# AIRI-Institute/HairFastGAN

Hardware: AMD Instinct MI355X
Metric: stylegan2_generator_fwd_1024_images_per_sec (higher is better)
Workload: dtype f32 tensors + f32 accumulate; conv products as 3 fp16 MFMAs on (hi,lo)-split operands (fp32-class); 1 GPU; StyleGAN2 1024^2 generator forward (range 0->8), random W+, fresh noise per layer, HIP modulated-conv + upfirdn2d kernels (BASELINE.json configs[1]); batch_per_gpu=8, global_batch=8, parallelism=replica x1, weights=synthetic closed-form (oracle/synth.py), conv_precision=f16x3

## Files before the change

### hairfastgan_amd/_lib.py

```python
import ctypes
import os

_HERE = os.path.dirname(os.path.abspath(__file__))
LIB_PATH = os.environ.get("HAIRFAST_HIP_LIB") or os.path.join(_HERE, "csrc", "libhairfast_hip.so")

_f = ctypes.c_void_p
_i = ctypes.c_int
_ll = ctypes.c_longlong
_fl = ctypes.c_float
_d = ctypes.c_double
_st = ctypes.c_void_p

SIGNATURES = {
    "hf_upfirdn2d_f32": [_f, _f, _f, _i, _i, _i, _i, _i, _i, _i, _i, _i, _i, _i, _i, _i, _st],
    "hf_fused_bias_act_f32": [_f, _f, _f, _ll, _i, _i, _fl, _fl, _st],
    "hf_noise_bias_act_f32": [_f, _f, _f, _f, _f, _i, _i, _i, _ll, _fl, _fl, _st],
    "hf_modconv_prepare_f32": [_f, _f, _f, _i, _i, _i, _st],
    "hf_modulation_f32": [_f, _f, _ll, _f, _f, _i, _i, _i, _st],
    "hf_style_batch_f32": [_f, _f, _ll, _ll, _f, _i, _i, _i, _i, _i, _st],
    "hf_demod_f32": [_f, _f, _f, _i, _i, _i, _st],
    "hf_style_normalize_f32": [_f, _f, _i, _i, _i, _st],
    "hf_modconv3x3_f32": [_f, _f, _f, _f, _f, _f, _f, _ll, _f, _i, _i, _i, _i, _i, _fl, _fl, _f, _ll, _st],
    "hf_conv_split_weights_f16": [_f, _f, _f, _i, _i, _st],
    "hf_conv_split_weights_f16_taps": [_f, _f, _f, _i, _i, _i, _st],
    "hf_modconv3x3_small_f16_f32": [_f, _f, _f, _f, _i, _f, _f, _f, _f, _ll, _f, _i, _i, _i, _i, _i, _fl, _fl, _i, _i, _f, _ll, _st],
    "hf_modconv3x3_small_up_blur_f16_f32": [_f, _f, _f, _f, _f, _f, _i, _f, _f, _f, _f, _f, _ll, _f, _f, _i, _i, _i, _i, _i, _fl, _fl, _f, _ll, _st],
    "hf_conv1x1_f16_f32": [_f, _f, _f, _f, _f, _f, _i, _f, _f, _f, _f, _i, _f, _fl, _f, _i, _i, _i, _i, _i, _i, _i, _ll, _f, _ll, _st],
    "hf_modconv3x3_f16_f32": [_f, _f, _f, _f, _i, _f, _f, _f, _f, _ll, _f, _i, _i, _i, _i, _i, _fl, _fl, _st],
    "hf_modconv3x3_f16_rgb_f32": [_f, _f, _f, _f, _i, _f, _f, _f, _f, _ll, _f, _i, _i, _i, _i, _i, _fl, _fl, _f, _f, _f, _st],
    "hf_modconv3x3_f16_pre_image_f32": [_f, _f, _f, _f, _f, _i, _f, _f, _f, _ll, _f, _i, _i, _i, _i, _i, _fl, _fl, _f, _f, _f, _f, _f, _st],
    "hf_modconv3x3_f16_pre_f32": [_f, _f, _f, _f, _f, _i, _f, _f, _f, _ll, _f, _i, _i, _i, _i, _i, _fl, _fl, _f, _f, _f, _f, _f, _f, _st],
    "hf_modconv3x3_up_f16_pre_f32": [_f, _f, _f, _f, _f, _i, _f, _i, _i, _i, _i, _i, _i, _st],
    "hf_modconv3x3_up_f16_f32": [_f, _f, _f, _f, _i, _f, _f, _i, _i, _i, _i, _i, _i, _st],
    "hf_modconv3x3_up_blur_f16_f32": [_f, _f, _f, _f, _f, _f, _f, _f, _f, _f, ctypes.POINTER(ctypes.c_float),
                                      ctypes.POINTER(ctypes.c_float), _f, _f, _ll, _f, _f, _i, _i, _i, _i, _i, _fl, _fl, _st],
    "hf_modconv3x3_up_f32": [_f, _f, _f, _f, _f, _i, _i, _i, _i, _i, _i, _f, _ll, _st],
    "hf_modconv_up_pitch": [_i],
    "hf_blur_noise_bias_act_f32": [_f, _f, _f, _f, _f, _ll, _f, _i, _i, _i, _i, _i, _fl, _fl, _st],
    "hf_blur_noise_bias_act_split_f16": [_f, _f, _f, _f, _f, _f, _ll, _f, _f, _i, _i, _i, _i, _i, _fl, _fl, _st],
    "hf_torgb_f32": [_f, _f, _f, _f, _f, _f, _f, _i, _i, _i, _i, _st],
    "hf_conv_prepare_f32": [_f, _f, _i, _i, _i, _fl, _st],
    "hf_bn_fold_f32": [_f, _f, _f, _f, _f, _f, _f, _fl, _i, _st],
    "hf_conv2d_f32": [_f, _f, _f, _f, _f, _f, _f, _i, _f, _fl, _f, _i, _i, _i, _i, _i, _i, _i, _i, _ll, _f, _ll, _st],
    "hf_conv2d_f16_f32": [_f, _f, _f, _f, _f, _f, _i, _f, _f, _f, _f, _i, _f, _fl, _f, _i, _i, _i, _i, _i, _i, _i, _ll, _f, _ll, _st],
    "hf_split_activation_f16": [_f, _f, _f, _f, _f, _ll, _i, _i, _i, _st],
    "hf_split_activation_mod_f16": [_f, _f, _f, _f, _ll, _i, _i, _i, _st],
    "hf_plane_mean_f32": [_f, _f, _i, _i, _st],
    "hf_se_gate_f32": [_f, _f, _f, _f, _i, _i, _i, _st],
    "hf_scale_shortcut_add_f32": [_f, _f, _f, _f, _i, _i, _i, _i, _i, _i, _i, _st],
    "hf_upsample_bilinear_add_f32": [_f, _f, _f, _i, _i, _i, _i, _i, _st],
    "hf_adaptive_avgpool_f32": [_f, _f, _i, _i, _i, _i, _i, _i, _i, _i, _st],
    "hf_downscale2x_f32": [_f, _f, _i, _i, _i, _st],
    "hf_linear_f32": [_f, _f, _ll, _f, _f, _i, _i, _i, _fl, _st],
    "hf_equal_linear_f32": [_f, _f, _ll, _f, _f, _i, _i, _i, _fl, _i, _fl, _fl, _st],
    "hf_pixel_norm_f32": [_f, _f, _i, _i, _st],
    "hf_bicubic_down_f32": [_f, _f, _f, _ll, _i, _i, _i, _st],
    "hf_dilate_erode_f32": [_f, _f, _f, _ll, _i, _i, _i, _st],
    "hf_quantize_u8_f32": [_f, _f, _ll, _st],
    "hf_poisson_setup_u8": [_f, _f, _f, _f, _f, _i, _i, _i, _i, _st],
    "hf_poisson_jacobi_f32": [_f, _f, _f, _f, _i, _i, _i, _i, _i, _i, _st],
    "hf_poisson_finish_u8": [_f, _f, _f, _f, _i, _i, _i, _i, _st],
    "hf_resize_lanczos_u8": [_f, _f, _f, _i, _i, _i, _i, _i, _f, _f, _i, _f, _f, _i, _st],
    "hf_quad_bilinear_u8": [_f, _f, ctypes.POINTER(ctypes.c_double), _i, _i, _i, _i, _i, _st],
    "hf_quad_lanczos4_u8": [_f, _f, ctypes.POINTER(ctypes.c_double), _i, _i, _i, _i, _f, _f, _i, _st],
    "hf_quad_lanczos4_ratio": [],
    "hf_align_pad_blur_f32": [_f, _f, _f, _f, _i, _f, _f, _i, _i, _i, _i, _i, _i, _i, _st],
    "hf_align_pad_finish_u8": [_f, _f, _f, _f, _f, _f, _i, _i, _i, _st],
    "hf_u8_to_unit_f32": [_f, _f, _ll, _st],
    "hf_paste_quad_u8": [_f, _f, _f, ctypes.POINTER(ctypes.c_double), _i, _i, _i, _i, _i, _i, _i, _i, _st],
    "hf_multiply_u8": [_f, _f, _f, _ll, _st],
    "hf_image_to_bytes_f32": [_f, _f, _i, _i, _i, _fl, _fl, _i, _i, _st],
    "hf_labels_to_rgb_i64": [_f, _f, _ll, _f, _i, _i, _st],
    "hf_png_encode_u8": [_f, _ll, _f, _f, _i, _i, _i, _i, _i, _f, _ll, _st],
    "hf_jpeg_encode_u8": [_f, _ll, _f, _f, _i, _i, _i, _i, _i, _i, _f, _ll, _st],
    "hf_jpeg_decode_u8": [_f, _f, _f, _f, _ll, _f, _ll, _f, _i, _i, _i, _i, _i, _i, _i, _i, _i, _f, _ll, _st],
    "hf_png_decode_u8": [_f, _f, _f, _f, _ll, _f, _ll, _f, _i, _i, _i, _i, _i, _i, _f, _ll, _st],
    "hf_frechet_accumulate_f64": [_f, _f, _f, _i, _i, _st],
    "hf_frechet_accumulate_f16_f64": [_f, _f, _f, _i, _i, _st],
    "hf_frechet_stats_f64": [_f, _f, _f, _f, _ll, _i, _st],
    "hf_sym_eig_jacobi_f64": [_f, _f, _f, _f, _i, _i, ctypes.POINTER(ctypes.c_int), ctypes.POINTER(ctypes.c_double), _st],
    "hf_sym_eig_jacobi_work_doubles": (_ll, [_i, _i]),
    "hf_frechet_congruence_f64": [_f, _f, _f, _f, _f, _i, _st],
    "hf_frechet_finish_f64": [_f, _f, _f, _f, _f, _f, _i, _st],
    "hf_conv2d_direct_f32": [_f, _f, _f, _f, _f, _f, _i, _fl, _i, _i, _i, _i, _i, _i, _i, _i, _st],
    "hf_maxpool2d_f32": [_f, _f, _ll, _i, _i, _i, _i, _st],
    "hf_lpips_layer_f64": [_f, _f, _f, _f, _f, _i, _i, _i, _i, _i, _st],
    "hf_lpips_layer_work_doubles": (_ll, [_i, _i, _i]),
    "hf_sq_err_sum_f64": [_f, _f, _f, _f, _i, _ll, _i, _st],
    "hf_sq_err_sum_work_doubles": (_ll, [_i, _ll]),
    "hf_ssim_planes_f64": [_f, _f, _f, _f, _f, _f, _f, _f, _f, _f, _i, _i, _i, _i, _i, _i, _d, _d, _d, _st],
    "hf_ssim_work_doubles": (_ll, [_i, _i, _i, _i]),
    "hf_ssim_tile": [_i],
    "hf_crop_avgpool_f32": [_f, _f, _f, _f, _i, _i, _i, _i, _i, _i, _i, _i, _i, _i, _st],
    "hf_l2_normalize_rows_f32": [_f, _f, _f, _i, _i, _st],
    "hf_row_similarity_f64": [_f, _f, _f, _i, _i, _i, _i, _st],
    "hf_conv2d_rect_f16_f32": [_f, _f, _f, _f, _f, _i, _f, _f, _i, _i, _i, _i, _i, _i, _i, _i, _i, _i, _i, _i, _i, _i, _i, _i, _i, _st],
    "hf_pool3x3_f32": [_f, _f, _i, _i, _i, _i, _i, _i, _i, _i, _i, _i, _st],
    "hf_resize_bilinear_tf1_f32": [_f, _f, _i, _i, _i, _i, _i, _i, _i, _i, _fl, _fl, _st],
    "hf_maxpool3x3s2_f32":[_f, _f, _ll, _i, _i, _st],
    "hf_gate_f32": [_f, _f, _f, _f, _f, _fl, _ll, _i, _st],
    "hf_upsample_nearest_f32": [_f, _f, _ll, _i, _i, _i, _i, _st],
    "hf_parsing_mask_i64": [_f, _f, _f, _i, _i, _i, _i, _i, _i, _i, _i, _st],
    "hf_layernorm_f32": [_f, _f, _f, _f, _i, _i, _fl, _i, _fl, _st],
    "hf_layernorm_grouped_f32": [_f, _f, _f, _f, _i, _i, _i, _fl, _i, _fl, _st],
    "hf_modulate_f32": [_f, _f, _f, _f, _ll, _i, _fl, _st],
    "hf_sample_layernorm_f32": [_f, _f, _f, _f, _i, _i, _i, _ll, _fl, _fl, _f, _ll, _st],
    "hf_pixel_norm_dim1_f32": [_f, _f, _i, _i, _i, _st],
    "hf_axpby_bcast_f32": [_f, _f, _fl, _f, _fl, _ll, _ll, _st],
    "hf_add_bcast_f32": [_f, _f, _f, _ll, _ll, _st],
    "hf_label_conv3x3_f32": [_f, _f, _f, _f, _i, _i, _i, _i, _i, _i, _i, _i, _f, _st],
    "hf_ace_modulate_f32": [_f, _f, _f, _f, _f, _f, _f, _f, _f, _i, _i, _i, _i, _fl, _i, _st],
    "hf_conv2d_f16_split_f32": [_f, _f, _f, _f, _f, _f, _f, _f, _f, _f, _i, _f, _f, _f, _f, _i, _f, _fl, _f, _i, _i, _i, _i, _i, _i, _st],
    "hf_stem7x7s2_f16_f32": [_f, _f, _f, _f, _f, _f, _f, _fl, _i, _i, _i, _i, _i, _st],
    "hf_ace_modulate_table_f32": [_f, _f, _f, _f, _f, _f, _f, _f, _f, _f, _f, _i, _i, _i, _i, _i, _i, _i, _fl, _i, _i, _st],
    "hf_region_mean_f32": [_f, _f, _f, _i, _i, _i, _i, _i, _ll, _ll, _i, _i, _st],
    "hf_tanh_f32": [_f, _f, _ll, _st],
    "hf_channel_layernorm_f32": [_f, _f, _f, _f, _i, _ll, _fl, _st],
    "hf_mha_small_f32": [_f, _f, _i, _i, _i, _i, _st],
    "hf_quick_gelu_f32": [_f, _f, _ll, _st],
    "hf_debug_set_dispatch": [_i, _i],
    "hf_debug_last_path": [],
    "hf_debug_set_persistent_blocks": [_i],
    "hf_debug_set_tuning": [_i],
    "hf_set_batch_invariant": [_i],
    "hf_set_splitk_counters": [_f, _i],
    "hf_modconv3x3_f16_rgb_slabs": [_i],
    "hf_profile_marker": [_i, _st],
    "hf_conv2d_f16_split_output_ok": [_i, _i, _i, _i, _i, _i, _i, _i],
    "hf_scale_shortcut_add_split_f16": [_f, _f, _f, _f, _f, _f, _f, _f, _i, _i, _i, _i, _i, _i, _i, _st],
    "hf_strerror": (ctypes.c_char_p, [_i]),
    "hf_abi_version": [],
    "hf_modconv_workspace_floats": (_ll, [_i, _i, _i, _i, _i, _i]),
    "hf_conv2d_workspace_floats": (_ll, [_i, _i, _i, _i, _i, _i, _i, _i]),
    "hf_conv2d_f16_workspace_floats": (_ll, [_i, _i, _i, _i, _i, _i, _i]),
    "hf_modconv3x3_small_workspace_floats": (_ll, [_i, _i, _i, _i, _i]),
    "hf_conv1x1_f16_workspace_floats": (_ll, [_i, _i, _i, _i, _i, _i, _i]),
    "hf_sample_layernorm_workspace_floats": (_ll, [_i, _i, _i]),
    "hf_f16_overflow_count": (_ll, [_i]),
    "hf_png_bound": (_ll, [_i, _i, _i]),
    "hf_png_segment_rows": [_i, _i, _i],
    "hf_png_workspace_bytes": (_ll, [_i, _i, _i, _i]),
    "hf_jpeg_bound": (_ll, [_i, _i, _i, _i]),
    "hf_jpeg_chunk_mcus": [_i, _i],
    "hf_jpeg_workspace_bytes": (_ll, [_i, _i, _i, _i, _i]),
    "hf_jpeg_decode_workspace_bytes": (_ll, [_i, _i, _i, _i, _i, _i, _i, _ll]),
    "hf_png_decode_workspace_bytes": (_ll, [_i, _i, _i, _i, _ll]),
}


class HairfastLibError(RuntimeError):
    pass


def bind(cdll):
    for name, sig in SIGNATURES.items():
        try:
            fn = getattr(cdll, name)
        except AttributeError as e:
            raise HairfastLibError(f"{cdll._name}: missing symbol {name}") from e
        fn.restype, fn.argtypes = sig if isinstance(sig, tuple) else (ctypes.c_int, sig)
    return cdll


_LIB = None


def load():
    global _LIB
    if _LIB is None:
        if not os.path.exists(LIB_PATH):
            raise HairfastLibError(
                f"{LIB_PATH} not found: build it with `python -c 'import __graft_entry__ as g; g.build()'` "
                "or hairfastgan_amd/csrc/build.sh (hipcc --offload-arch=gfx950). "
                "hairfastgan_amd has no CPU / PyTorch fallback.")
        _LIB = bind(ctypes.CDLL(LIB_PATH))
    return _LIB


def check(lib, code, what):
    if code != 0:
        raise RuntimeError(f"{what}: {lib.hf_strerror(code).decode()} (code {code})")
```

### hairfastgan_amd/_marshal.py

```python
import functools
import os

import torch
import torch.nn.functional as F

from ._lib import check
from ._runtime import CANON_BATCH, plan_batch

SQRT2 = 2 ** 0.5

PROFILE = None


KERNEL_NAMES = {
    211: "conv_mfma_pipe<2,2,2,4>", 212: "conv_mfma_pipe<2,2,1,4>", 213: "conv_mfma_pipe<1,2,1,4>",
    214: "conv_mfma_pipe<2,2,2,2>", 215: "conv_mfma_pipe<1,1,2,2>", 216: "conv_mfma_pipe<1,4,1,4>",
    231: "conv_mfma_dma<2,2,2,4>", 232: "conv_mfma_dma<2,2,1,4>", 233: "conv_mfma_dma<1,2,1,4>", 234: "conv_mfma_dma<2,2,2,2>",
    244: "conv_mfma_pipe<2,2,2,2,stride2>", 245: "conv_mfma_pipe<1,1,2,2,stride2>",
    221: "conv_mfma_pipe<1,2,2,2,up>", 222: "conv_mfma_pipe<1,2,1,4,up>", 223: "conv_mfma_pipe<1,1,2,2,up>",
    224: "conv_mfma_pipe<1,2,2,4,up>", 225: "conv_mfma_pipe<1,1,1,4,up>", 300: "conv_mfma<1,1,2,2> split-K",
    581: "conv_mfma_h<1,2,2,4,up,pre>", 583: "conv_mfma_h<1,2,1,8,up,pre>",
    571: "conv_mfma_h<1,2,2,4,pre>", 572: "conv_mfma_h<2,2,1,8,pre>", 575: "conv_mfma_h<1,2,1,8,tw128,pre>",
    579: "conv_rows_h<32->32,strip64,pre>",
    551: "conv_mfma_h<1,2,2,4>", 552: "conv_mfma_h<2,2,1,8>", 553: "conv_mfma_h<1,2,1,8>", 555: "conv_mfma_h<1,2,1,8,tw128>",
    561: "conv_mfma_h<1,2,2,4,up>", 563: "conv_mfma_h<1,2,1,8,up>",
    573: "conv_mfma_h<1,2,1,8,up,fuse>", 593: "conv_mfma_h<1,2,1,8,up,pre,fuse>",
    601: "conv_enc_h<64x256>", 602: "conv_enc_h<64x128,stride2>", 603: "conv_enc_h<64x128>", 604: "conv_enc_h<64x512>",
    605: "conv_enc_h<64x128,stride2,x4 tiles>",
    606: "conv_enc_h<64x128,stride2,x2 tiles>",
}


def _launch_profiled(lib, flops, fn, label=None, nbytes=0.0, tag=""):
    if PROFILE is None:
        return fn()
    e0 = torch.cuda.Event(enable_timing=True)
    e1 = torch.cuda.Event(enable_timing=True)
    e0.record()
    r = fn()
    e1.record()
    if label is None:
        code = lib.hf_debug_last_path()
        label = KERNEL_NAMES.get(code, f"conv_mfma (general, code {code})")
        if tag and label.endswith(">"):
            label = label[:-1] + tag + ">"
    PROFILE.append((label, flops, e0, e1, nbytes))
    return r


def _p(t):
    return None if t is None else t.data_ptr()


def _c(t):
    if t is None:
        return None
    if t.dtype != torch.float32:
        raise TypeError(f"hairfastgan_amd kernels are fp32; got {t.dtype}")
    return t if t.is_contiguous() else t.contiguous()


class SplitActivation:

    def __init__(self, hi, lo, key):
        self.hi, self.lo, self.key = hi, lo, key
        b, cb, h, w, _ = hi.shape
        self.shape = (b, cb * 8, h, w)

    @classmethod
    def empty(cls, b, c, h, w, device, want_lo=True, key=None):
        hi = torch.empty((b, c // 8, h, w, 8), dtype=torch.float16, device=device)
        return cls(hi, torch.empty_like(hi) if want_lo else None, key)


def _hl(split):
    return (None, None) if split is None else (_p(split.hi), _p(split.lo))


def upfirdn2d(lib, st, x, kernel, up_x, up_y, down_x, down_y, pad_x0, pad_x1, pad_y0, pad_y1):
    x, kernel = _c(x), _c(kernel)
    n, c, h, w = x.shape
    kh, kw = kernel.shape
    out_h = (h * up_y + pad_y0 + pad_y1 - kh) // down_y + 1
    out_w = (w * up_x + pad_x0 + pad_x1 - kw) // down_x + 1
    out = x.new_empty((n, c, out_h, out_w))
    if out.numel():
        check(lib, lib.hf_upfirdn2d_f32(_p(out), _p(x), _p(kernel), n * c, h, w, kh, kw, up_x, up_y, down_x,
                                        down_y, pad_x0, pad_x1, pad_y0, pad_y1, st), "hf_upfirdn2d_f32")
    return out


def fused_bias_act(lib, st, x, bias, alpha, scale):
    x, bias = _c(x), _c(bias)
    out = torch.empty_like(x)
    n = x.numel()
    if n == 0:
        return out
    step_b = 1
    for d in x.shape[2:]:
        step_b *= d
    n_bias = bias.numel() if bias is not None else 0
    if bias is not None and x.ndim >= 2 and n_bias != x.shape[1]:
        raise ValueError("bias must have one entry per channel (dim 1)")
    check(lib, lib.hf_fused_bias_act_f32(_p(out), _p(x), _p(bias), n, max(n_bias, 1), step_b, alpha, scale, st),
          "hf_fused_bias_act_f32")
    return out


def _noise_args(noise, batch, hw):
    if noise is None:
        return None, 0
    noise = _c(noise)
    if noise.numel() == hw:
        return noise, 0
    if noise.numel() == batch * hw:
        return noise, hw
    raise ValueError(f"noise must be [1,1,H,W] or [B,1,H,W]; got {tuple(noise.shape)}")


def noise_bias_act(lib, st, x, noise, noise_w, bias, alpha=0.2, scale=SQRT2):
    x, bias, noise_w = _c(x), _c(bias), _c(noise_w)
    b, c, h, w = x.shape
    noise, nbs = _noise_args(noise, b, h * w)
    out = torch.empty_like(x)
    check(lib, lib.hf_noise_bias_act_f32(_p(out), _p(x), _p(noise), _p(noise_w), _p(bias), b, c, h * w, nbs,
                                         alpha, scale, st), "hf_noise_bias_act_f32")
    return out


def prepare_weights(lib, st, weight):
    weight = _c(weight)
    _, cout, cin, k, _ = weight.shape
    wt = weight.new_empty((k * k, cin, cout))
    wsq = weight.new_empty((cout, cin))
    check(lib, lib.hf_modconv_prepare_f32(_p(wt), _p(wsq), _p(weight), cout, cin, k, st), "hf_modconv_prepare_f32")
    return wt, wsq


def modulation(lib, st, style, mod_w, mod_b):
    if style.dtype != torch.float32:
        raise TypeError("style must be fp32")
    if style.stride(-1) != 1:
        style = style.contiguous()
    b, sd = style.shape
    mod_w, mod_b = _c(mod_w), _c(mod_b)
    cin = mod_w.shape[0]
    s = style.new_empty((b, cin))
    check(lib, lib.hf_modulation_f32(_p(s), _p(style), style.stride(0) if b > 1 else sd, _p(mod_w), _p(mod_b),
                                     b, cin, sd, st), "hf_modulation_f32")
    return s


def style_job_table(convs, rows, batch, device):
    recs, layout, ofs = [], [], 0
    for conv, row in zip(convs, rows):
        _, wsq = conv.prepared()
        cin, cout = conv.in_channel, conv.out_channel
        s_ofs = ofs
        ofs += batch * cin
        d_ofs = -1
        if conv.demodulate:
            d_ofs = ofs
            ofs += batch * cout
        mw, mb = conv.modulation.weight.detach(), conv.modulation.bias.detach()
        recs.append([mw.data_ptr(), mb.data_ptr(), wsq.data_ptr() if conv.demodulate else 0, cin | (cout << 32), row,
                     s_ofs, max(d_ofs, 0)])
        layout.append((s_ofs, cin, d_ofs, cout))
    table = torch.tensor(recs, dtype=torch.int64).to(device)
    return table, layout, ofs


def style_batch(lib, st, latent, table, layout, total, max_cin, max_cout):
    if latent.dtype != torch.float32 or latent.stride(-1) != 1:
        latent = latent.float().contiguous()
    b, _, sd = latent.shape
    out = latent.new_empty(total)
    check(lib, lib.hf_style_batch_f32(_p(out), _p(latent), latent.stride(0), latent.stride(1), _p(table), len(layout), b, sd,
                                      max_cin, max_cout, st), "hf_style_batch_f32")
    res = []
    for s_ofs, cin, d_ofs, cout in layout:
        s = out[s_ofs:s_ofs + b * cin].view(b, cin)
        d = out[d_ofs:d_ofs + b * cout].view(b, cout) if d_ofs >= 0 else None
        res.append((s, d))
    return res


def demod(lib, st, s, wsq):
    b, cin = s.shape
    cout = wsq.shape[0]
    d = s.new_empty((b, cout))
    check(lib, lib.hf_demod_f32(_p(d), _p(s), _p(wsq), b, cin, cout, st), "hf_demod_f32")
    return d


def style_normalize(lib, st, s, d):
    b, cin = s.shape
    check(lib, lib.hf_style_normalize_f32(_p(s), _p(d), b, cin, d.shape[1], st), "hf_style_normalize_f32")


def f16_overflow_count(lib, reset=False):
    return int(lib.hf_f16_overflow_count(1 if reset else 0))


def _workspace(lib, like, b, cin, cout, h, w, up):
    n = lib.hf_modconv_workspace_floats(b, cin, cout, h, w, 1 if up else 0)
    if n <= 0:
        return None, 0
    return like.new_empty((n,)), n


def modconv3x3(lib, st, x, wt, s, d, noise, noise_w, bias, alpha=0.2, scale=SQRT2):
    x = _c(x)
    b, cin, h, w = x.shape
    cout = wt.shape[2]
    noise, nbs = _noise_args(noise, b, h * w)
    out = x.new_empty((b, cout, h, w))
    noise_w, bias = _c(noise_w), _c(bias)
    ws, ws_n = _workspace(lib, x, b, cin, cout, h, w, False)
    code = _launch_profiled(
        lib, 2.0 * cin * cout * 9 * h * w * b,
        lambda: lib.hf_modconv3x3_f32(_p(out), _p(x), _p(wt), _p(s), _p(d), _p(noise), _p(noise_w), nbs, _p(bias),
                                      b, cin, cout, h, w, alpha, scale, _p(ws), ws_n, st))
    check(lib, code, "hf_modconv3x3_f32")
    return out


def split_weights_f16(lib, st, wt):
    wt = _c(wt)
    taps, cin, cout = wt.shape
    if taps != 9 or cin % 16:
        raise ValueError(f"f16 MFMA path needs 3x3 weights with cin % 16 == 0; got {tuple(wt.shape)}")
    n = 9 * cin * cout
    hi = torch.empty(n + 8, dtype=torch.float16, device=wt.device)[:n].view(cin // 16, 9, 2, cout, 8)
    lo = torch.empty((cin // 16, 9, 2, cout, 8), dtype=torch.float16, device=wt.device)
    check(lib, lib.hf_conv_split_weights_f16(_p(hi), _p(lo), _p(wt), cin, cout, st), "hf_conv_split_weights_f16")
    return hi, lo


def split_weights_unscale(wt_hi):
    n = wt_hi.numel()
    flat = torch.empty(0, dtype=torch.float16, device=wt_hi.device).set_(wt_hi.untyped_storage(), wt_hi.storage_offset(), (n + 8,))
    return float(flat[n:n + 2].view(torch.float32)[0])


def modconv3x3_f16_supported(cin, cout, h, w, batch=None):
    if batch is not None and plan_batch(batch) * h * w < 2048:
        return False
    return cin % 16 == 0 and w >= 32 and (h >= 8 if cout % 64 == 0 else (cout % 32 == 0 and h >= 16))


def torgb_fusable(cin, cout, h, w):
    if not (cout % 32 == 0 and modconv3x3_f16_supported(cin, cout, h, w)):
        return False
    return h * w >= (512 if cout in (32, 64) else 4096)


IMAGE_FUSE = os.environ.get("HAIRFAST_IMAGE_FUSE", "1") != "0"


def image_fusable(cin, cout, h, w):
    return cin == 32 and cout == 32 and w % 64 == 0 and h % 8 == 0 and IMAGE_FUSE


def modconv3x3_f16_pre_image(lib, st, act, wt_hi, wt_lo, nterms, d, noise, noise_w, bias, rgb, rgb_bias, skip, up_kernel,
                             alpha=0.2, scale=SQRT2):
    b, cin, h, w = act.shape
    cout = wt_hi.shape[3]
    skip = _c(skip)
    if tuple(skip.shape) != (b, 3, h // 2, w // 2):
        raise ValueError(f"skip must be [B,3,H/2,W/2]; got {tuple(skip.shape)} for a {h}x{w} layer")
    noise, nbs = _noise_args(noise, b, h * w)
    image = torch.empty((b, 3, h, w), dtype=torch.float32, device=act.hi.device)
    rgb_wt, rgb_s = _c(rgb[0]), _c(rgb[1])
    nparts = 2 if nterms == 3 else 1
    nb = float(b) * h * w * (2.0 * nparts * cin + 12.0 + 3.0) + 2.0 * nparts * 9 * cin * cout
    code = _launch_profiled(
        lib, 2.0 * cin * cout * 9 * h * w * b,
        lambda: lib.hf_modconv3x3_f16_pre_image_f32(_p(image), _p(act.hi), _p(act.lo), _p(wt_hi), _p(wt_lo), nterms, _p(d), _p(noise),
                                                    _p(_c(noise_w)), nbs, _p(_c(bias)), b, cin, cout, h, w, alpha, scale, _p(rgb_wt),
                                                    _p(rgb_s), _p(_c(rgb_bias)), _p(skip), _p(_c(up_kernel)), st), nbytes=nb)
    if code == -1:
        return None
    check(lib, code, "hf_modconv3x3_f16_pre_image_f32")
    return image


def torgb_slabs(cout):
    return cout // 64 if cout % 64 == 0 else cout // 32


def modconv3x3_f16(lib, st, x, wt_hi, wt_lo, nterms, s, d, noise, noise_w, bias, alpha=0.2, scale=SQRT2, rgb=None):
    x = _c(x)
    b, cin, h, w = x.shape
    cout = wt_hi.shape[3]
    noise, nbs = _noise_args(noise, b, h * w)
    out = x.new_empty((b, cout, h, w))
    noise_w, bias = _c(noise_w), _c(bias)
    if rgb is not None:
        rgb_wt, rgb_s = _c(rgb[0]), _c(rgb[1])
        raw = x.new_empty((b, 3 * torgb_slabs(cout), h, w))
        code = _launch_profiled(
            lib, 2.0 * cin * cout * 9 * h * w * b,
            lambda: lib.hf_modconv3x3_f16_rgb_f32(_p(out), _p(x), _p(wt_hi), _p(wt_lo), nterms, _p(s), _p(d), _p(noise),
                                                  _p(noise_w), nbs, _p(bias), b, cin, cout, h, w, alpha, scale,
                                                  _p(raw), _p(rgb_wt), _p(rgb_s), st))
        check(lib, code, "hf_modconv3x3_f16_rgb_f32")
        return out, raw
    code = _launch_profiled(
        lib, 2.0 * cin * cout * 9 * h * w * b,
        lambda: lib.hf_modconv3x3_f16_f32(_p(out), _p(x), _p(wt_hi), _p(wt_lo), nterms, _p(s), _p(d), _p(noise),
                                          _p(noise_w), nbs, _p(bias), b, cin, cout, h, w, alpha, scale, st))
    check(lib, code, "hf_modconv3x3_f16_f32")
    return out


def split_activation_reference(x, s):
    b, c, h, w = x.shape
    v = x if s is None else x * s[:, :, None, None]
    hi = v.half()
    lo = (v - hi.float()).half()
    blk = lambda t: t.reshape(b, c // 8, 8, h, w).permute(0, 1, 3, 4, 2).contiguous()
    return blk(hi), blk(lo)


def _modconv3x3_f16_pre(lib, st, act, wt_hi, wt_lo, nterms, d, noise, noise_w, bias, alpha=0.2, scale=SQRT2, rgb=None,
                        want_out=True, split_for=None):
    b, cin, h, w = act.shape
    cout = wt_hi.shape[3]
    dev = act.hi.device
    noise, nbs = _noise_args(noise, b, h * w)
    if not want_out and rgb is None and split_for is None:
        raise ValueError("want_out=False needs another consumer (rgb= or split_for=)")
    out = torch.empty((b, cout, h, w), dtype=torch.float32, device=dev) if want_out else None
    noise_w, bias = _c(noise_w), _c(bias)
    raw = rgb_wt = rgb_s = split = s_next = None
    if rgb is not None:
        rgb_wt, rgb_s = _c(rgb[0]), _c(rgb[1])
        raw = torch.empty((b, 3 * torgb_slabs(cout), h, w), dtype=torch.float32, device=dev)
    if split_for is not None:
        s_next = _c(split_for)
        split = SplitActivation.empty(b, cout, h, w, dev, want_lo=nterms == 3)
    nparts = 2 if nterms == 3 else 1
    nb = (float(b) * h * w * (2.0 * nparts * cin + (4.0 * cout if want_out else 0.0) + (2.0 * nparts * cout if split_for is not None else 0.0)
                              + (12.0 * torgb_slabs(cout) if rgb is not None else 0.0)) + 2.0 * nparts * 9 * cin * cout)
    code = _launch_profiled(
        lib, 2.0 * cin * cout * 9 * h * w * b,
        lambda: lib.hf_modconv3x3_f16_pre_f32(_p(out), _p(act.hi), _p(act.lo), _p(wt_hi), _p(wt_lo), nterms, _p(d), _p(noise),
                                              _p(noise_w), nbs, _p(bias), b, cin, cout, h, w, alpha, scale, _p(raw),
                                              _p(rgb_wt), _p(rgb_s), *_hl(split), _p(s_next), st), nbytes=nb)
    check(lib, code, "hf_modconv3x3_f16_pre_f32")
    return out, raw, split


def modconv3x3_f16_pre(lib, st, act, wt_hi, wt_lo, nterms, d, noise, noise_w, bias, alpha=0.2, scale=SQRT2, rgb=None,
                       want_out=True, split_for=None):
    out, raw, split = _modconv3x3_f16_pre(lib, st, act, wt_hi, wt_lo, nterms, d, noise, noise_w, bias, alpha, scale, rgb, want_out,
                                          split_for)
    res = (out,) + (() if rgb is None else (raw,)) + (() if split_for is None else (split,))
    return res[0] if len(res) == 1 else res


def split_weights_small(lib, st, wt):
    taps, cin, cout = wt.shape
    w1 = _c(wt).permute(1, 0, 2).reshape(1, cin, taps * cout).contiguous()
    return conv_split_weights_f16(lib, st, w1)


def modconv3x3_small_supported(cin, cout, h, w, batch, upsample=False):
    if cin % 32 or cout % 64 or h * w > 1024:
        return False
    n = plan_batch(batch) * h * w
    if upsample:
        return h * w <= 64 or (h * w <= 256 and n <= 1024)
    return 256 < n <= 2048 or (n == 256 and h * w <= 64) or (h * w == 64 and CANON_BATCH * 64 <= n <= 2048)


def conv3x3_small_supported(cin, cout, h, w, batch):
    return cin % 32 == 0 and cout % 64 == 0 and h * w <= 256 and plan_batch(batch) * h * w <= 4096 and cin * cout >= 512 * 512


def modconv3x3_small(lib, st, x, w9, nterms, s, d, noise, noise_w, bias, cout, alpha=0.2, scale=SQRT2, upsample=False):
    x = _c(x)
    b, cin, h, w = x.shape
    hi, lo = w9
    n = lib.hf_modconv3x3_small_workspace_floats(b, cin, cout, h, w)
    ws = x.new_empty((max(n, 1),))
    if upsample:
        pitch = lib.hf_modconv_up_pitch(w)
        out = x.new_empty((b, cout, 2 * h + 1, pitch))
        noise = bias = noise_w = None
        nbs = 0
    else:
        pitch = 0
        out = x.new_empty((b, cout, h, w))
        noise, nbs = _noise_args(noise, b, h * w)
    code = _launch_profiled(
        lib, 2.0 * cin * cout * 9 * h * w * b,
        lambda: lib.hf_modconv3x3_small_f16_f32(_p(out), _p(x), _p(hi), _p(lo), nterms, _p(_c(s)), _p(_c(d)), _p(noise),
                                                _p(_c(noise_w)), nbs, _p(_c(bias)), b, cin, cout, h, w, alpha, scale,
                                                1 if upsample else 0, pitch, _p(ws), n, st),
        label="gemm_h tap-GEMM (small planes)")
    check(lib, code, "hf_modconv3x3_small_f16_f32")
    return out


SMALL_UP_FUSED = os.environ.get("HAIRFAST_SMALL_UP_FUSED", "1") != "0"


def small_up_blur_supported(h, w):
    return (8 * (2 * h + 3) * (2 * w + 3) + 72 * h * w) * 4 <= 150 * 1024


def modconv3x3_small_up_blur(lib, st, x, w9, nterms, s, d, blur_kernel, noise, noise_w, bias, cout, alpha=0.2, scale=SQRT2,
                             split_for=None):
    x = _c(x)
    b, cin, h, w = x.shape
    hi, lo = w9
    n = lib.hf_modconv3x3_small_workspace_floats(b, cin, cout, h, w)
    ws = x.new_empty((max(n, 1),))
    noise, nbs = _noise_args(noise, b, 4 * h * w)
    out = split = s_next = None
    if split_for is not None:
        s_next = _c(split_for[1])
        split = SplitActivation.empty(b, cout, 2 * h, 2 * w, x.device, want_lo=split_for[2] if len(split_for) > 2 else True,
                                      key=split_for[0])
    else:
        out = x.new_empty((b, cout, 2 * h, 2 * w))
    code = _launch_profiled(
        lib, 2.0 * cin * cout * 9 * h * w * b,
        lambda: lib.hf_modconv3x3_small_up_blur_f16_f32(_p(out), *_hl(split), _p(x), _p(hi), _p(lo), nterms, _p(_c(s)), _p(_c(d)),
                                                        _p(_c(blur_kernel)), _p(noise), _p(_c(noise_w)), nbs, _p(_c(bias)),
                                                        _p(s_next), b, cin, cout, h, w, alpha, scale, _p(ws), n, st),
        label="gemm_h tap-GEMM (small planes)")
    check(lib, code, "hf_modconv3x3_small_up_blur_f16_f32")
    return out if split_for is None else split


def modconv3x3_up_f16_supported(cin, cout, h, w, batch=None):
    if batch is not None and plan_batch(batch) * h * w < 512:
        return False
    return cin % 16 == 0 and cout % 32 == 0 and h * w >= (256 if cout % 64 == 0 else 512) and min(h, w) >= 2


def modconv3x3_up(lib, st, x, wt, s, d, blur_kernel, noise, noise_w, bias, alpha=0.2, scale=SQRT2, f16=None,
                  split_for=None, small=None):
    pre = isinstance(x, SplitActivation)
    if not pre:
        x = _c(x)
    b, cin, h, w = x.shape
    cout = wt.shape[2]
    pitch = lib.hf_modconv_up_pitch(w)
    if pre or small is None:
        tmp = torch.empty((b, cout, 2 * h + 1, pitch), dtype=torch.float32, device=(x.hi if pre else x).device)
    if pre:
        hi, lo, nterms = f16
        code = _launch_profiled(
            lib, 2.0 * cin * cout * 9 * h * w * b,
            lambda: lib.hf_modconv3x3_up_f16_pre_f32(_p(tmp), _p(x.hi), _p(x.lo), _p(hi), _p(lo), nterms, _p(d), b, cin, cout,
                                                     h, w, pitch, st))
        check(lib, code, "hf_modconv3x3_up_f16_pre_f32")
    elif small is not None and SMALL_UP_FUSED and small_up_blur_supported(h, w):
        return modconv3x3_small_up_blur(lib, st, x, small[0], small[1], s, d, blur_kernel, noise, noise_w, bias, cout, alpha, scale,
                                        split_for=split_for)
    elif small is not None:
        tmp = modconv3x3_small(lib, st, x, small[0], small[1], s, d, None, None, None, cout, upsample=True)
    elif f16 is not None:
        hi, lo, nterms = f16
        code = _launch_profiled(
            lib, 2.0 * cin * cout * 9 * h * w * b,
            lambda: lib.hf_modconv3x3_up_f16_f32(_p(tmp), _p(x), _p(hi), _p(lo), nterms, _p(s), _p(d), b, cin, cout, h, w,
                                                 pitch, st))
        check(lib, code, "hf_modconv3x3_up_f16_f32")
    else:
        ws, ws_n = _workspace(lib, x, b, cin, cout, h, w, True)
        code = _launch_profiled(
            lib, 2.0 * cin * cout * 9 * h * w * b,
            lambda: lib.hf_modconv3x3_up_f32(_p(tmp), _p(x), _p(wt), _p(s), _p(d), b, cin, cout, h, w, pitch, _p(ws),
                                             ws_n, st))
        check(lib, code, "hf_modconv3x3_up_f32")
    noise, nbs = _noise_args(noise, b, 4 * h * w)
    if split_for is not None:
        s_next = split_for[1]
        want_lo = split_for[2] if len(split_for) > 2 else True
        split = SplitActivation.empty(b, cout, 2 * h, 2 * w, tmp.device, want_lo, key=split_for[0])
        nb = float(b * cout) * (4.0 * (2 * h + 1) * (2 * w + 1) + (4.0 if want_lo else 2.0) * 4 * h * w)
        code = _launch_profiled(
            lib, 0.0,
            lambda: lib.hf_blur_noise_bias_act_split_f16(*_hl(split), _p(tmp), _p(_c(blur_kernel)), _p(noise),
                                                         _p(_c(noise_w)), nbs, _p(_c(bias)), _p(_c(s_next)), b, cout,
                                                         2 * h + 1, 2 * w + 1, pitch, alpha, scale, st),
            label="blur4x4_split8", nbytes=nb)
        check(lib, code, "hf_blur_noise_bias_act_split_f16")
        return split
    out = tmp.new_empty((b, cout, 2 * h, 2 * w))
    nb = float(b * cout) * 4.0 * ((2 * h + 1) * (2 * w + 1) + 4 * h * w)
    code = _launch_profiled(
        lib, 0.0,
        lambda: lib.hf_blur_noise_bias_act_f32(_p(out), _p(tmp), _p(_c(blur_kernel)), _p(noise), _p(_c(noise_w)),
                                               nbs, _p(_c(bias)), b, cout, 2 * h + 1, 2 * w + 1, pitch, alpha, scale, st),
        label="blur4x4_noise_bias_act", nbytes=nb)
    check(lib, code, "hf_blur_noise_bias_act_f32")
    return out


def blur_factors(kernel4x4):
    import ctypes

    k = kernel4x4.detach().double().cpu()
    if tuple(k.shape) != (4, 4) or float(k[0, 0]) == 0.0:
        return None
    kx, ky = k[0, :].clone(), k[:, 0] / k[0, 0]
    if not torch.allclose(torch.outer(ky, kx), k, rtol=1e-6, atol=1e-12):
        return None
    arr = ctypes.c_float * 4
    return arr(*[float(v) for v in kx]), arr(*[float(v) for v in ky])


def modconv3x3_up_fused_supported(cin, cout, h, w):
    return cin % 16 == 0 and cout % 32 == 0 and h >= 16 and w >= 32


def modconv3x3_up_fused(lib, st, x, wt_hi, wt_lo, s, d, factors, noise, noise_w, bias, alpha=0.2, scale=SQRT2, split_for=None,
                        nterms=3):
    pre = isinstance(x, SplitActivation)
    if not pre:
        x = _c(x)
    b, cin, h, w = x.shape
    cout = wt_hi.shape[3]
    dev = x.hi.device if pre else x.device
    noise, nbs = _noise_args(noise, b, 4 * h * w)
    out = split = s_next = None
    if split_for is not None:
        s_next = _c(split_for)
        split = SplitActivation.empty(b, cout, 2 * h, 2 * w, dev, want_lo=nterms == 3)
    else:
        out = torch.empty((b, cout, 2 * h, 2 * w), dtype=torch.float32, device=dev)
    kx, ky = factors
    nb_alg = float(b) * (4.0 * cin * h * w + 4.0 * cout * 4 * h * w + 4.0 * 4 * h * w) + 4.0 * 9 * cin * cout
    code = _launch_profiled(
        lib, 2.0 * cin * cout * 9 * h * w * b,
        lambda: lib.hf_modconv3x3_up_blur_f16_f32(_p(out), *_hl(split), None if pre else _p(x), _p(x.hi) if pre else None,
                                                  _p(x.lo) if (pre and nterms == 3) else None, _p(wt_hi),
                                                  _p(wt_lo) if nterms == 3 else None, None if pre else _p(s), _p(d),
                                                  kx, ky, _p(noise), _p(_c(noise_w)), nbs, _p(_c(bias)), _p(s_next), b, cin, cout,
                                                  h, w, alpha, scale, st), nbytes=nb_alg)
    check(lib, code, "hf_modconv3x3_up_blur_f16_f32")
    return out if split_for is None else split


def torgb(lib, st, x, wt, s, bias, skip, up_kernel):
    x = _c(x)
    b, cin, h, w = x.shape
    skip = _c(skip)
    if skip is not None and tuple(skip.shape) != (b, 3, h // 2, w // 2):
        raise ValueError(f"skip must be [B,3,H/2,W/2]; got {tuple(skip.shape)} for x {tuple(x.shape)}")
    out = x.new_empty((b, 3, h, w))
    nb = float(b) * 4.0 * h * w * (cin + 3 + (0.75 if skip is not None else 0.0))
    code = _launch_profiled(
        lib, 0.0,
        lambda: lib.hf_torgb_f32(_p(out), _p(x), _p(wt), _p(s), _p(_c(bias)), _p(skip), _p(_c(up_kernel)), b, cin, h, w, st),
        label="torgb_kernel" if h * w > 4096 else "torgb_small_kernel", nbytes=nb)
    check(lib, code, "hf_torgb_f32")
    return out


ACT_NONE, ACT_LRELU, ACT_PRELU, ACT_QGELU = 0, 1, 2, 3
ACT_RESIDUAL_FIRST = 16


def conv_prepare(lib, st, weight, scale=1.0):
    weight = _c(weight)
    cout, cin, k, _ = weight.shape
    wt = weight.new_empty((k * k, cin, cout))
    check(lib, lib.hf_conv_prepare_f32(_p(wt), _p(weight), cout, cin, k, scale, st), "hf_conv_prepare_f32")
    return wt


def bn_fold(lib, st, gamma, beta, mean, var, eps, conv_bias=None):
    gamma, beta, mean, var, conv_bias = _c(gamma), _c(beta), _c(mean), _c(var), _c(conv_bias)
    n = gamma.numel()
    scale, shift = gamma.new_empty(n), gamma.new_empty(n)
    check(lib, lib.hf_bn_fold_f32(_p(scale), _p(shift), _p(gamma), _p(beta), _p(mean), _p(var), _p(conv_bias),
                                  float(eps), n, st), "hf_bn_fold_f32")
    return scale, shift


def _enc_conv_io(lib, x, cout, stride, in_scale, in_shift, residual, groups=1, x_shared=True, ws_floats=None, taps=9, nterms=3,
                 want_f32=True, split_out=False):
    pre = isinstance(x, SplitActivation)
    own = groups > 1 and not x_shared
    if pre:
        if in_scale is not None or in_shift is not None:
            raise ValueError("a pre-split input carries its affine already")
        n_img, cin, h, w = x.shape
        b = n_img // groups if own else n_img
        x_gstride = 1 if own else 0
        dev = x.hi.device
    else:
        x = _c(x)
        dev = x.device
        if own:
            g_, b, cin, h, w = x.shape
            if g_ != groups:
                raise ValueError("x must be [groups, B, cin, H, W]")
            x_gstride = b * cin * h * w
        else:
            b, cin, h, w = x.shape
            x_gstride = 0
    oh, ow = (h - 1) // stride + 1, (w - 1) // stride + 1
    shape = (groups, b, cout, oh, ow) if groups > 1 else (b, cout, oh, ow)
    out = torch.empty(shape, dtype=torch.float32, device=dev) if want_f32 else None
    if residual is not None:
        residual = _c(residual)
        if tuple(residual.shape) != shape:
            raise ValueError(f"residual {tuple(residual.shape)} != output {shape}")
    n = 0 if ws_floats is None else getattr(lib, ws_floats[0])(b, cin, cout, h, w, *ws_floats[1:], stride, groups)
    ws = torch.empty((n,), dtype=torch.float32, device=dev) if n > 0 else None
    nparts = 2 if nterms == 3 else 1
    nb = (float(b * (groups if own else 1)) * cin * (h * w if taps == 9 else oh * ow) * (2.0 * nparts if pre else 4.0)
          + float(b) * groups * cout * oh * ow * ((2.0 * nparts if split_out else 0.0) + (4.0 if want_f32 else 0.0)
                                                  + (4.0 if residual is not None else 0.0))
          + 2.0 * nparts * taps * cin * cout * groups)
    return x, (b, cin, h, w, oh, ow), x_gstride, out, residual, ws, max(n, 0), nb


def conv2d(lib, st, x, wt, k, stride=1, in_scale=None, in_shift=None, out_scale=None, bias=None, act=ACT_NONE,
           slope=None, alpha=0.0, residual=None, groups=1, x_shared=True):
    cout = wt.shape[-1]
    x, (b, cin, h, w, oh, ow), x_gstride, out, residual, ws, n, _ = _enc_conv_io(
        lib, x, cout, stride, None, None, residual, groups, x_shared, ("hf_conv2d_workspace_floats", k))
    code = _launch_profiled(
        lib, 2.0 * cin * cout * k * k * oh * ow * b * groups,
        lambda: lib.hf_conv2d_f32(_p(out), _p(x), _p(_c(wt)), _p(in_scale), _p(in_shift), _p(_c(out_scale)), _p(_c(bias)),
                                  act, _p(_c(slope)), float(alpha), _p(residual), b, cin, cout, h, w, k, stride, groups,
                                  x_gstride, _p(ws), n, st))
    check(lib, code, "hf_conv2d_f32")
    return out


def _pow2_ceil(v):
    p = 1
    while p < v:
        p <<= 1
    return p


@functools.lru_cache(maxsize=4096)
def conv2d_f16_supported(cin, cout, h, w, k, stride):
    if k != 3 or cin % 16 or cout % 64 or stride not in (1, 2):
        return False
    oh, ow = (h - 1) // stride + 1, (w - 1) // stride + 1
    tw = min(32, _pow2_ceil(ow))
    return tw >= 16 and _pow2_ceil(oh) >= 128 // tw


def conv_split_weights_f16(lib, st, wt):
    wt = _c(wt)
    w4 = wt if wt.ndim == 4 else wt.unsqueeze(0)
    g, taps, cin, cout = w4.shape
    if taps not in (9, 1) or cin % 16:
        raise ValueError(f"f16 MFMA path needs 3x3 or 1x1 weights with cin % 16 == 0; got {tuple(wt.shape)}")
    n = taps * cin * cout
    hi = torch.empty(g * (n + 8), dtype=torch.float16, device=wt.device)
    lo = torch.empty(g * n, dtype=torch.float16, device=wt.device)
    for i in range(g):
        check(lib, lib.hf_conv_split_weights_f16_taps(hi[i * (n + 8):].data_ptr(), lo[i * n:].data_ptr(), w4[i].data_ptr(), cin, cout,
                                                     taps, st), "hf_conv_split_weights_f16_taps")
    return hi, lo


def conv1x1_f16_supported(cin, cout):
    return cin % 32 == 0 and cout % 64 == 0


def conv1x1_f16(lib, st, x, wt_hi, wt_lo, nterms, cout, stride=1, in_scale=None, in_shift=None, out_scale=None, bias=None,
                act=ACT_NONE, slope=None, alpha=0.0, residual=None, groups=1, x_shared=True):
    pre = isinstance(x, SplitActivation)
    x, (b, cin, h, w, oh, ow), x_gstride, out, residual, ws, n, nb = _enc_conv_io(
        lib, x, cout, stride, in_scale, in_shift, residual, groups, x_shared, ("hf_conv1x1_f16_workspace_floats",), taps=1, nterms=nterms)
    code = _launch_profiled(
        lib, 2.0 * cin * cout * oh * ow * b * groups,
        lambda: lib.hf_conv1x1_f16_f32(_p(out), None if pre else _p(x), _p(x.hi) if pre else None, _p(x.lo) if pre else None,
                                       _p(wt_hi), _p(wt_lo), nterms, _p(_c(in_scale)), _p(_c(in_shift)),
                                       _p(_c(out_scale)), _p(_c(bias)), act, _p(_c(slope)), float(alpha), _p(residual), b, cin, cout,
                                       h, w, stride, groups, x_gstride, _p(ws), n, st),
        label="gemm_h", nbytes=nb)
    check(lib, code, "hf_conv1x1_f16_f32")
    return out


def split_activation_f16(lib, st, x, in_scale=None, in_shift=None, want_lo=True):
    x = _c(x)
    c, h, w = x.shape[-3:]
    images = x.numel() // (c * h * w)
    split = SplitActivation.empty(images, c, h, w, x.device, want_lo)
    check(lib, lib.hf_split_activation_f16(*_hl(split), _p(x), _p(_c(in_scale)), _p(_c(in_shift)), images, c, h, w, st),
          "hf_split_activation_f16")
    return split


def conv2d_f16(lib, st, x, wt_hi, wt_lo, nterms, cout, stride=1, in_scale=None, in_shift=None, out_scale=None, bias=None,
               act=ACT_NONE, slope=None, alpha=0.0, residual=None, groups=1, x_shared=True):
    pre = isinstance(x, SplitActivation)
    x, (b, cin, h, w, oh, ow), x_gstride, out, residual, ws, n, nb = _enc_conv_io(
        lib, x, cout, stride, in_scale, in_shift, residual, groups, x_shared, ("hf_conv2d_f16_workspace_floats",), nterms=nterms)
    code = _launch_profiled(
        lib, 2.0 * cin * cout * 9 * oh * ow * b * groups,
        lambda: lib.hf_conv2d_f16_f32(_p(out), None if pre else _p(x), _p(x.hi) if pre else None, _p(x.lo) if pre else None,
                                      _p(wt_hi), _p(wt_lo), nterms, _p(in_scale), _p(in_shift), _p(_c(out_scale)),
                                      _p(_c(bias)), act, _p(_c(slope)), float(alpha), _p(residual), b, cin, cout, h, w, stride,
                                      groups, x_gstride, _p(ws), n, st), tag=",pre" if pre else "", nbytes=nb)
    check(lib, code, "hf_conv2d_f16_f32")
    return out


def conv2d_f16_split_supported(lib, b, cin, cout, h, w, stride, nterms=3, pre=False):
    return cout % 8 == 0 and lib.hf_conv2d_f16_split_output_ok(b, cin, cout, h, w, stride, nterms, 1 if pre else 0) == 1


def conv2d_f16_split(lib, st, x, wt_hi, wt_lo, nterms, cout, stride=1, in_scale=None, in_shift=None, out_scale=None, bias=None,
                     act=ACT_NONE, slope=None, alpha=0.0, residual=None, next_scale=None, next_shift=None, want_f32=False):
    pre = isinstance(x, SplitActivation)
    x, (b, cin, h, w, oh, ow), _, out, residual, _, _, nb = _enc_conv_io(
        lib, x, cout, stride, in_scale, in_shift, residual, nterms=nterms, want_f32=want_f32, split_out=True)
    split = SplitActivation.empty(b, cout, oh, ow, (x.hi if pre else x).device, want_lo=nterms == 3)
    code = _launch_profiled(
        lib, 2.0 * cin * cout * 9 * oh * ow * b,
        lambda: lib.hf_conv2d_f16_split_f32(_p(out), *_hl(split), _p(_c(next_scale)), _p(_c(next_shift)), None if pre else _p(x),
                                            _p(x.hi) if pre else None, _p(x.lo) if pre else None, _p(wt_hi), _p(wt_lo), nterms,
                                            _p(in_scale), _p(in_shift), _p(_c(out_scale)), _p(_c(bias)), act, _p(_c(slope)),
                                            float(alpha), _p(residual), b, cin, cout, h, w, stride, st),
        tag=",pre,split-out" if pre else ",split-out", nbytes=nb)
    check(lib, code, "hf_conv2d_f16_split_f32")
    return split, out


def plane_mean(lib, st, x):
    x = _c(x)
# ... 916 lines not shown
```

### hairfastgan_amd/csrc/api.hip

```cpp
#include "hf_common.h"

extern "C" const char *hf_strerror(int code) {
  switch (code) {
    case HF_OK: return "ok";
    case HF_E_INVALID: return "invalid argument";
    case HF_E_LAUNCH: return "kernel launch failed";
    case HF_E_WORKSPACE: return "workspace too small";
    default: return "unknown error";
  }
}

extern "C" int hf_abi_version(void) { return 13; }

__global__ void hf_profile_marker_kernel() {}

extern "C" int hf_profile_marker(int id, void *stream) {
  if (id < 0 || id > 1023) return HF_E_INVALID;
  hipLaunchKernelGGL(hf_profile_marker_kernel, dim3(id + 1), dim3(64), 0, static_cast<hipStream_t>(stream));
  return hipGetLastError() == hipSuccess ? HF_OK : HF_E_LAUNCH;
}

extern "C" unsigned long long hf_f16_overflow_count_convh(int reset);
extern "C" unsigned long long hf_f16_overflow_count_blur(int reset);
extern "C" unsigned long long hf_f16_overflow_count_enc(int reset);
extern "C" unsigned long long hf_f16_overflow_count_gemm(int reset);
extern "C" unsigned long long hf_f16_overflow_count_stem(int reset);

extern "C" long long hf_f16_overflow_count(int reset) {
  return (long long)(hf_f16_overflow_count_convh(reset) + hf_f16_overflow_count_blur(reset) + hf_f16_overflow_count_enc(reset) +
                     hf_f16_overflow_count_gemm(reset) + hf_f16_overflow_count_stem(reset));
}
```

### hairfastgan_amd/csrc/convh.hip

```cpp
#define HF_WANT_F16_SPLIT
#include <type_traits>

#include "conv_common.h"

using namespace hf_detail;

#ifdef HF_H_TRACE
__device__ unsigned long long hf_trace_buf[8 * 512];
#define HF_TRACE_POINT(id)                                                                    \
  do {                                                                                         \
    if (blockIdx.x == 0 && blockIdx.y == 0 && lane == 0 && wave < 8 && trace_n < 510) {                    \
      hf_trace_buf[wave * 512 + trace_n++] = ((unsigned long long)(id) << 56) | (__builtin_readcyclecounter() & 0xffffffffffffffULL); \
    }                                                                                          \
  } while (0)
extern "C" int hf_debug_read_trace(unsigned long long *host, int n) {
  return (int)hipMemcpyFromSymbol(host, HIP_SYMBOL(hf_trace_buf), sizeof(unsigned long long) * n);
}
#else
#define HF_TRACE_POINT(id) ((void)0)
#endif

namespace {

template <int PT, bool UP, int TWMAX, bool FUSE = false>
// ... 743 lines not shown
      hf_barrier_keep_young<0>();
      HF_TRACE_POINT(3);
    }

    if (FUSE) {
      if (P.oh) epilogue_fused(std::true_type{}, cur, ep_slot, nzf, ((stage - 1) & 1));
      else epilogue_fused(std::false_type{}, cur, ep_slot, nzf, ((stage - 1) & 1));
    } else {
      bool done = false;
      if constexpr (!UP) {
        if (fast_ep) {
          epilogue_fast(G, cur, ep_slot, nzr);
          done = true;
        }
      }
      if (!done) epilogue(G, cur, ep_slot, nzr);
    }
    HF_TRACE_POINT(4);
    if (!has_next) break;
    zero_acc();
    if (nxt.b0 != cur.b0) ep_slot ^= 1;
    cur = nxt;
    t_cur = t_next;
  }
}

__global__ __launch_bounds__(256) void split_weights_absmax(unsigned int *__restrict__ trailer,
                                                            const float *__restrict__ wt, long long n) {
  float m = 0.0f;
  const long long stride = (long long)gridDim.x * blockDim.x;
  for (long long i = (long long)blockIdx.x * blockDim.x + threadIdx.x; i < n; i += stride) m = fmaxf(m, fabsf(wt[i]));
#pragma unroll
  for (int d = 32; d >= 1; d >>= 1) m = fmaxf(m, __shfl_xor(m, d, 64));
  if ((threadIdx.x & 63) == 0 && __float_as_uint(m) > trailer[1]) atomicMax(trailer + 1, __float_as_uint(m));
}
__global__ void split_weights_clear(unsigned int *trailer) {
  if (threadIdx.x < 4) trailer[threadIdx.x] = 0u;
}
__device__ __forceinline__ int weight_prescale_log2(unsigned int absmax_bits) {
  const int e = (int)((absmax_bits >> 23) & 255u) - 127;
  if (e <= -127 || e >= 128) return 0;
  int k = 13 - e;
  return k > 120 ? 120 : (k < -120 ? -120 : k);
}
__global__ __launch_bounds__(256) void split_weights(_Float16 *__restrict__ wth, _Float16 *__restrict__ wtl,
                                                     const float *__restrict__ wt, int cin, int cout, int taps) {
  const long long n = (long long)taps * cin * cout;
  unsigned int *trailer = reinterpret_cast<unsigned int *>(wth + n);
  const int k = weight_prescale_log2(trailer[1]);
  const float up = __uint_as_float((unsigned int)(127 + k) << 23);
  if (blockIdx.x == 0 && threadIdx.x == 0) reinterpret_cast<float *>(trailer)[0] = __uint_as_float((unsigned int)(127 - k) << 23);
  const long long stride = (long long)gridDim.x * blockDim.x;
  bool ovf = false;
  for (long long i = (long long)blockIdx.x * blockDim.x + threadIdx.x; i < n; i += stride) {
    const int co = (int)(i % cout);
    const long long r = i / cout;
    const int ci = (int)(r % cin), tap = (int)(r / cin);
    const long long dst = ((((long long)(ci / 16) * taps + tap) * 2 + (ci % 16) / 8) * cout + co) * 8 + (ci % 8);
    _Float16 h, l;
    hf_split_f16(wt[i] * up, h, l, ovf);
    wth[dst] = h;
    if (wtl) wtl[dst] = l;
  }
}

constexpr int RIM_DEPTH = 3;
template <int NTERMS>
__global__ __launch_bounds__(64) void conv_up_rim_h(const ConvParams P, const _Float16 *__restrict__ wth,
                                                    const _Float16 *__restrict__ wtl, int row_tiles, int pos_tiles) {
  constexpr int NPART = (NTERMS == 3) ? 2 : 1;
  const int lane = threadIdx.x & 63;
  const int li = lane & 31;
  const int lh = lane >> 5;
  const int co_tiles = P.cout / 32;
  int t = (int)blockIdx.x;
  const int co0 = (t % co_tiles) * 32;
  t /= co_tiles;
  const int pt = t % pos_tiles, b = t / pos_tiles;
  const bool is_row = pt < row_tiles;
  const int p = (is_row ? pt : pt - row_tiles) * 32 + li;
  const int h = P.h, w = P.w;
  const int plane = h * w;
  const bool store_ok = is_row ? p <= w : p < h;
  const bool near_ok = is_row ? p < w : p < h;
  const bool diag_ok = p >= 1 && (is_row ? p <= w : p < h);
  const int near_u = near_ok ? (is_row ? (h - 1) * w + p : p * w + (w - 1)) : 0;
  const int diag_u = diag_ok ? (is_row ? (h - 1) * w + p - 1 : (p - 1) * w + (w - 1)) : 0;
  const int tap0 = is_row ? 6 : 2, tap1 = is_row ? 7 : 5, tap2 = 8;

  const int nchunks = P.cin / KH;
  const long long x_lane = (((long long)b * (P.cin / 8) + lh) * plane) * 16;
  const long long x_chunk = 2LL * plane * 16;
  const char *xh = static_cast<const char *>(P.xh) + x_lane;
  const char *xl = NTERMS == 3 ? static_cast<const char *>(P.xl) + x_lane : nullptr;
  const long long w_lane = ((long long)lh * P.cout + co0 + li) * 16;
  const long long w_tap = 2LL * P.cout * 16, w_chunk = 9 * w_tap;
  const char *wh = reinterpret_cast<const char *>(wth) + w_lane;
  const char *wl = NTERMS == 3 ? reinterpret_cast<const char *>(wtl) + w_lane : nullptr;

  const float w_unscale = *reinterpret_cast<const float *>(wth + 9LL * P.cin * P.cout);
  float dmv[16];
#pragma unroll
  for (int r = 0; r < 16; ++r) dmv[r] = 1.0f;
  if (P.d) {
#pragma unroll
    for (int r = 0; r < 16; ++r) dmv[r] = P.d[(long long)b * P.d_bstride + co0 + (r & 3) + 8 * (r >> 2) + 4 * lh];
  }
#pragma unroll
  for (int r = 0; r < 16; ++r) dmv[r] *= w_unscale;

  half8 wa[RIM_DEPTH][3][NPART], xa[RIM_DEPTH][2][NPART];
  auto load = [&](int slot, int c) {
    const char *xc[2] = {xh + c * x_chunk, NTERMS == 3 ? xl + c * x_chunk : nullptr};
    const char *wc[2] = {wh + c * w_chunk, NTERMS == 3 ? wl + c * w_chunk : nullptr};
#pragma unroll
    for (int part = 0; part < NPART; ++part) {
      xa[slot][0][part] = *reinterpret_cast<const half8 *>(xc[part] + (long long)near_u * 16);
      xa[slot][1][part] = *reinterpret_cast<const half8 *>(xc[part] + (long long)diag_u * 16);
      wa[slot][0][part] = *reinterpret_cast<const half8 *>(wc[part] + tap0 * w_tap);
      wa[slot][1][part] = *reinterpret_cast<const half8 *>(wc[part] + tap1 * w_tap);
      wa[slot][2][part] = *reinterpret_cast<const half8 *>(wc[part] + tap2 * w_tap);
    }
  };
  f32x16 acc0, acc1;
#pragma unroll
  for (int r = 0; r < 16; ++r) acc0[r] = acc1[r] = 0.0f;
  auto mma = [&](f32x16 &acc, const half8 (&a)[NPART], const half8 (&bf)[NPART], bool ok) {
    const half8 zero = {};
    half8 bv[NPART];
#pragma unroll
    for (int part = 0; part < NPART; ++part) bv[part] = ok ? bf[part] : zero;
    mfma_f16x3<NTERMS, 1, 1>(&acc, &a[0], &a[NPART - 1], &bv[0], &bv[NPART - 1]);
  };

  auto chunk = [&](int s) {
    mma(acc0, wa[s][0], xa[s][0], near_ok);
    mma(acc1, wa[s][1], xa[s][0], near_ok);
    mma(acc0, wa[s][2], xa[s][1], diag_ok);
  };
#pragma unroll
  for (int s = 0; s < RIM_DEPTH; ++s) load(s, min(s, nchunks - 1));
  int c0 = 0;
  for (; c0 + RIM_DEPTH <= nchunks; c0 += RIM_DEPTH) {
#pragma unroll
    for (int s = 0; s < RIM_DEPTH; ++s) {
      chunk(s);
      load(s, min(c0 + s + RIM_DEPTH, nchunks - 1));
    }
  }
#pragma unroll
  for (int s = 0; s + 1 < RIM_DEPTH; ++s)
    if (c0 + s < nchunks) chunk(s);

  if (!store_ok) return;
  const long long oplane = (long long)P.out_h * P.out_w;
  float *ob = P.out + ((long long)b * P.cout + co0) * oplane +
              (is_row ? (long long)(2 * h) * P.out_w + 2 * p : (long long)(2 * p) * P.out_w + 2 * w);
  const long long second = is_row ? 1 : P.out_w;
  const bool has_second = !is_row || p < w;
#pragma unroll
  for (int r = 0; r < 16; ++r) {
    float *q = ob + (long long)((r & 3) + 8 * (r >> 2) + 4 * lh) * oplane;
    q[0] = acc0[r] * dmv[r];
    if (has_second) q[second] = acc1[r] * dmv[r];
  }
}

inline long long up_rim_blocks(const ConvParams &P) {
  return (long long)P.batch * (hf_cdiv(P.w + 1, 32) + hf_cdiv(P.h, 32)) * (P.cout / 32);
}
template <int NTERMS>
int launch_up_rim(const ConvParams &P, const _Float16 *wth, const _Float16 *wtl, hipStream_t st) {
  const int row_tiles = hf_cdiv(P.w + 1, 32), col_tiles = hf_cdiv(P.h, 32);
  hipLaunchKernelGGL((conv_up_rim_h<NTERMS>), dim3((unsigned)up_rim_blocks(P)), dim3(64), 0, st, P, wth, wtl, row_tiles,
                     row_tiles + col_tiles);
  return hf_launch_status();
}

template <int NTERMS, int CT_TILES, int PG, int WAVES_CO, int WAVES_PX, bool UP, int TWMAX = 32, bool PRE = false, bool FUSE = false>
int launch_h(ConvParams &P, const _Float16 *wth, const _Float16 *wtl, hipStream_t st) {
  using S = HShape<NTERMS, CT_TILES, PG, WAVES_CO, WAVES_PX, UP, TWMAX, FUSE>;
  constexpr int NT = S::NT, CT = S::CT, PT = S::PT, NPIX = S::Stage::NPIX;
  if (P.cin % KH || P.cout % CT || P.stride != 1 || P.t || P.groups > 1 || P.residual || P.act == ACT_PRELU)
    return HF_E_INVALID;
  if ((long long)P.cin * P.h * P.w >= (1LL << 31)) return HF_E_INVALID;
  if ((long long)CT * P.out_h * P.out_w * 4 >= (1LL << 32)) return HF_E_INVALID;
  P.splits = 1;
  P.n_geom = 1;
  P.g[0] = make_geom(0, 0, P.h, P.w, P.batch, PT, 0);
  if (TWMAX > 32 && P.w >= 64 && P.g[0].lg_nb == 0) {
    const int tw = min(TWMAX, pow2_floor(P.w)), th = PT / tw;
    if (th >= 1 && P.h >= th) {
      P.g[0].lg_tw = ilog2(tw); P.g[0].lg_th = ilog2(th);
      P.g[0].tiles_x = hf_cdiv(P.w, tw); P.g[0].tiles_y = hf_cdiv(P.h, th);
    }
  }
  if (FUSE) {
    constexpr int TH = PT / 32;
    P.g[0].lg_tw = 5; P.g[0].lg_th = ilog2(TH); P.g[0].lg_nb = 0;
    P.g[0].tiles_x = hf_cdiv(P.w, 30); P.g[0].tiles_y = hf_cdiv(P.h, TH - 2); P.g[0].tiles_b = P.batch;
  }
  int nblocks = geom_blocks(P.g[0]);
  const bool rim_kernel = UP && !FUSE && PRE && !(g_h_tune & 32);
  if (rim_kernel && up_rim_blocks(P) >= (1LL << 31)) return HF_E_INVALID;
  if (UP && !FUSE && !rim_kernel) {
    P.n_geom = 3;
    constexpr int RIM = PT >= 512 ? 4 : 2;
    P.g[1] = make_geom(P.h, 0, 1, P.w + 1, P.batch, PT, nblocks, true, RIM);
    nblocks += geom_blocks(P.g[1]);
    P.g[2] = make_geom(0, P.w, P.h, 1, P.batch, PT, nblocks, true, RIM);
    nblocks += geom_blocks(P.g[2]);
  }
  for (int i = 0; i < P.n_geom; ++i) {
    if (P.g[i].lg_nb != 0 || (1 << (P.g[i].lg_tw + P.g[i].lg_th)) != PT) return HF_E_INVALID;
    if (geom_xs(P.g[i], 1, UP ? 1 : 2) > NPIX) return HF_E_INVALID;
  }
  const size_t lds = S::lds_bytes(P.cin, P.rgb_out != nullptr);
  if (P.rgb_out && (UP || !P.rgb_w || !P.rgb_s || (!HF_STD_STYLED_TAIL(P) && (WAVES_CO != 1 || P.cout != CT)) ||
                    P.rgb_slabs != P.cout / (32 * CT_TILES)))
    return HF_E_INVALID;
  if (lds > 160 * 1024) return HF_E_INVALID;
  P.n_tiles = nblocks;
  const int co_tiles = P.cout / CT;
  const int per_cu = (2 * lds <= 160 * 1024) ? 2 : 1;
  int resident = (g_h_blocks > 0 ? g_h_blocks : 256 * per_cu) / co_tiles;
  if (resident < 1) resident = 1;
  const bool walk = P.cin / KH >= 2 && (P.cin / KH <= 8 || g_h_blocks > 0);
  const int gx = (walk && nblocks > resident) ? resident : nblocks;
  dim3 grid(gx, co_tiles);
  if (grid.y > 65535) return HF_E_INVALID;
  P.swap_xy = 0;
  if (co_tiles > 1 && gx <= 65535) {
    const double in_bytes = (double)P.batch * P.cin * P.h * P.w * 4.0, w_bytes = 9.0 * P.cin * P.cout * 4.0;
    if (columns_fastest(in_bytes, in_bytes, w_bytes, co_tiles, nblocks)) {
      P.swap_xy = 1;
      grid = dim3(co_tiles, gx);
    }
  }
  if (PRE) {
    if (!P.xh || (NTERMS == 3 && !P.xl) || P.s || (P.cin & 15)) return HF_E_INVALID;
    if ((long long)2 * P.h * P.w * 16 >= (1LL << 31)) return HF_E_INVALID;
    hipLaunchKernelGGL((conv_mfma_h<NTERMS, CT_TILES, PG, WAVES_CO, WAVES_PX, false, UP, TWMAX, PRE, FUSE>), grid, dim3(NT), lds, st,
                       P, wth, wtl);
  } else if (P.s) {
    hipLaunchKernelGGL((conv_mfma_h<NTERMS, CT_TILES, PG, WAVES_CO, WAVES_PX, true, UP, TWMAX, false, FUSE>), grid, dim3(NT), lds, st,
                       P, wth, wtl);
  } else {
    if (FUSE) return HF_E_INVALID;
    hipLaunchKernelGGL((conv_mfma_h<NTERMS, CT_TILES, PG, WAVES_CO, WAVES_PX, false, UP, TWMAX, false, false>), grid, dim3(NT), lds,
                       st, P, wth, wtl);
  }
  const int rc = hf_launch_status();
  if constexpr (UP && !FUSE && PRE) {
    if (rc == HF_OK && rim_kernel) return launch_up_rim<NTERMS>(P, wth, wtl, st);
  }
  return rc;
}

template <int CT_TILES_, int PG_, int WAVES_CO_, int WAVES_PX_, int TWMAX_ = 32>
struct HForm {
  static constexpr int CT_TILES = CT_TILES_, PG = PG_, WAVES_CO = WAVES_CO_, WAVES_PX = WAVES_PX_, TWMAX = TWMAX_;
};
using HForm63 = HForm<1, 2, 1, 8>;
template <bool UP, bool PRE, class F>
int with_h_form(int cfg, F &&f) {
  if constexpr (UP) {
    if (cfg == 63) return f(HForm63{});
    if (cfg == 61) return f(HForm<1, 2, 2, 4>{});
  } else {
    if (cfg == 55) return f(HForm<1, 2, 1, 8, 128>{});
    if constexpr (!PRE) {
      if (cfg == 56) return f(HForm<1, 2, 1, 8, 64>{});
      if (cfg == 54) return f(HForm<1, 2, 1, 4>{});
    }
    if (cfg == 53) return f(HForm<1, 2, 1, 8>{});
    if (cfg == 52) return f(HForm<2, 2, 1, 8>{});
    if (cfg == 51) return f(HForm<1, 2, 2, 4>{});
  }
  return HF_E_INVALID;
}
template <int NTERMS, bool UP, bool PRE, bool FUSE, class Form>
int launch_tile(Form, ConvParams &P, const _Float16 *h, const _Float16 *l, hipStream_t st) {
  return launch_h<NTERMS, Form::CT_TILES, Form::PG, Form::WAVES_CO, Form::WAVES_PX, UP, Form::TWMAX, PRE, FUSE>(P, h, l, st);
}
template <bool UP, bool PRE>
int launch_form(int cfg, int nterms, ConvParams &P, const _Float16 *h, const _Float16 *l, hipStream_t st) {
  return with_h_form<UP, PRE>(cfg, [&](auto form) {
    return with_nterms(nterms, [&](auto nt) { return launch_tile<decltype(nt)::value, UP, PRE, false>(form, P, h, l, st); });
  });
}

}

namespace hf_detail {

thread_local int g_force_h = 0;
thread_local int g_h_blocks = 0;
thread_local int g_h_tune = 0;
int g_batch_invariant = 0;

int launch_conv_h(ConvParams &P, int nterms, bool up, const void *wth, const void *wtl, hipStream_t st) {
  const _Float16 *h = static_cast<const _Float16 *>(wth), *l = static_cast<const _Float16 *>(wtl);
  if (!h || (nterms == 3 && !l)) return HF_E_INVALID;
  int cfg, rc;
  if (up) {
    cfg = (P.cout % 64) ? 63 : 61;
    rc = P.xh ? launch_form<true, true>(cfg, nterms, P, h, l, st) : launch_form<true, false>(cfg, nterms, P, h, l, st);
    if (rc == HF_OK) note_path(5, P.xh ? cfg + 20 : cfg);
    return rc;
  }
  cfg = g_force_h;
  if (cfg == 0) {
    const long long blocks52 = (long long)P.batch * hf_cdiv(P.h, 16) * hf_cdiv(P.w, 32) * (P.cout / 64);
    if (P.cout % 64) cfg = (P.w >= 128) ? 55 : 53;
    else cfg = (P.h * P.w >= 512 && blocks52 >= 256) ? 52 : 51;
  }
  if (P.rgb_out && cfg == 51) cfg = 52;
  if (P.xh) {
    if (!g_force_h && !(g_h_tune & 16) && P.cin == 32 && P.cout == 32) {
      rc = launch_conv_rows(P, nterms, wth, wtl, st);
      if (rc == HF_OK) {
        note_path(5, 79);
        return rc;
      }
    }
    if (P.rgb_skip) return HF_E_INVALID;
    rc = launch_form<false, true>(cfg, nterms, P, h, l, st);
    if (rc == HF_OK) note_path(5, cfg + 20);
    return rc;
  }
  rc = launch_form<false, false>((cfg >= 52 && cfg <= 56) ? cfg : 51, nterms, P, h, l, st);
  if (rc == HF_OK) note_path(5, cfg);
  return rc;
}

}

extern "C" int hf_conv_split_weights_f16(void *wt_hi, void *wt_lo, const float *wt, int cin, int cout, void *stream) {
  return hf_conv_split_weights_f16_taps(wt_hi, wt_lo, wt, cin, cout, 9, stream);
}

extern "C" int hf_conv_split_weights_f16_taps(void *wt_hi, void *wt_lo, const float *wt, int cin, int cout, int taps, void *stream) {
  if (!wt_hi || !wt || cin <= 0 || cout <= 0 || (cin % 16) || (taps != 9 && taps != 1)) return HF_E_INVALID;
  long long n = (long long)taps * cin * cout;
  long long g = (n + 255) / 256;
  if (g > 4096) g = 4096;
  unsigned int *trailer = reinterpret_cast<unsigned int *>(static_cast<_Float16 *>(wt_hi) + n);
  hipLaunchKernelGGL(split_weights_clear, dim3(1), dim3(64), 0, (hipStream_t)stream, trailer);
  hipLaunchKernelGGL(split_weights_absmax, dim3((int)(g > 512 ? 512 : g)), dim3(256), 0, (hipStream_t)stream, trailer, wt, n);
  hipLaunchKernelGGL(split_weights, dim3((int)g), dim3(256), 0, (hipStream_t)stream, static_cast<_Float16 *>(wt_hi),
                     static_cast<_Float16 *>(wt_lo), wt, cin, cout, taps);
  return hf_launch_status();
}

extern "C" unsigned long long hf_f16_overflow_count_convh(int reset) { return hf_f16_overflow_read_tu(reset); }

static int gen_fill(ConvParams &P, const float *x, const void *x_hi, const void *x_lo, const void *wt_hi, int nterms,
                    const float *s, const float *d, int batch, int cin, int cout, int h, int w, bool up = false, int tmp_pitch = 0) {
  if ((!x && !x_hi) || !wt_hi || batch <= 0 || cin <= 0 || cout <= 0 || h <= 0 || w <= 0 || (nterms != 1 && nterms != 3) ||
      (nterms == 3 && x_hi && !x_lo) || (up && tmp_pitch < 2 * w + 1))
    return HF_E_INVALID;
  P.x = x; P.xh = x_hi; P.xl = x_lo; P.s = s; P.d = d;
  P.s_bstride = cin; P.d_bstride = cout;
  P.groups = 1;
  P.batch = batch; P.cin = cin; P.cout = cout; P.h = h; P.w = w; P.out_h = h; P.out_w = w; P.out_wv = w;
  if (up) { P.out_h = 2 * h + 1; P.out_w = tmp_pitch; P.out_wv = 2 * w + 1; }
  P.stride = 1;
  return HF_OK;
}
static int gen_tail(ConvParams &P, const float *noise, const float *noise_w, long long noise_bstride, const float *bias,
                    float alpha, float scale) {
  if (noise && !noise_w) return HF_E_INVALID;
  P.noise = noise; P.noise_w = noise_w; P.bias = bias;
  P.noise_bstride = noise_bstride;
  P.act = bias ? ACT_LRELU : ACT_NONE;
  P.alpha = alpha; P.scale = scale;
  return HF_OK;
}

extern "C" int hf_modconv3x3_f16_f32(float *out, const float *x, const void *wt_hi, const void *wt_lo, int nterms,
                                     const float *s, const float *d, const float *noise, const float *noise_w,
                                     long long noise_bstride, const float *bias, int batch, int cin, int cout, int h,
                                     int w, float alpha, float scale, void *stream) {
  ConvParams P{};
  if (!out || !x || gen_fill(P, x, nullptr, nullptr, wt_hi, nterms, s, d, batch, cin, cout, h, w) != HF_OK ||
      gen_tail(P, noise, noise_w, noise_bstride, bias, alpha, scale) != HF_OK)
    return HF_E_INVALID;
  P.out = out;
  return launch_conv_h(P, nterms, false, wt_hi, wt_lo, (hipStream_t)stream);
}

extern "C" int hf_modconv3x3_up_f16_f32(float *tmp, const float *x, const void *wt_hi, const void *wt_lo, int nterms,
                                        const float *s, const float *d, int batch, int cin, int cout, int h, int w,
                                        int tmp_pitch, void *stream) {
  ConvParams P{};
  if (!tmp || !x || gen_fill(P, x, nullptr, nullptr, wt_hi, nterms, s, d, batch, cin, cout, h, w, true, tmp_pitch) != HF_OK)
    return HF_E_INVALID;
  P.out = tmp;
  return launch_conv_h(P, nterms, true, wt_hi, wt_lo, (hipStream_t)stream);
}

extern "C" int hf_modconv3x3_up_blur_f16_f32(float *out, void *split_hi, void *split_lo, const float *x, const void *x_hi,
                                             const void *x_lo, const void *wt_hi, const void *wt_lo, const float *s,
                                             const float *d, const float *blur_k1d_x, const float *blur_k1d_y, const float *noise, const float *noise_w,
                                             long long noise_bstride, const float *bias, const float *s_next, int batch, int cin,
                                             int cout, int h, int w, float alpha, float scale, void *stream) {
  const int nterms = wt_lo ? 3 : 1;
  ConvParams P{};
  if (gen_fill(P, x, x_hi, x_lo, wt_hi, nterms, x_hi ? nullptr : s, d, batch, cin, cout, h, w) != HF_OK ||
      gen_tail(P, noise, noise_w, noise_bstride, bias, alpha, scale) != HF_OK || (!out == !split_hi) || !blur_k1d_x ||
      !blur_k1d_y || h < 2 || w < 2 || (!x_hi && !s) || (cout % 32) || (cin % 16) ||
      (split_hi && ((nterms == 3 && !split_lo) || (cout & 7))) || !bias || !(alpha >= 0.0f && alpha <= 1.0f) || !(scale > 0.0f))
    return HF_E_INVALID;
  P.out = out;
  P.out_h = 2 * h; P.out_w = 2 * w; P.out_wv = 2 * w;
  P.oh = split_hi; P.ol = nterms == 3 ? split_lo : nullptr; P.s_next = s_next;
  for (int j = 0; j < 4; ++j) {
    P.blur_kx[j] = blur_k1d_x[3 - j];
    P.blur_ky[j] = blur_k1d_y[3 - j];
  }
  const _Float16 *hi = static_cast<const _Float16 *>(wt_hi), *lo = static_cast<const _Float16 *>(wt_lo);
  const int rc = with_nterms(nterms, [&](auto nt) {
    return x_hi ? launch_tile<decltype(nt)::value, true, true, true>(HForm63{}, P, hi, lo, (hipStream_t)stream)
                : launch_tile<decltype(nt)::value, true, false, true>(HForm63{}, P, hi, lo, (hipStream_t)stream);
  });
  if (rc == HF_OK) note_path(5, x_hi ? 93 : 73);
  return rc;
}

extern "C" int hf_set_batch_invariant(int on) {
  const int prev = hf_detail::g_batch_invariant;
  hf_detail::g_batch_invariant = on ? 1 : 0;
  return prev;
}

extern "C" int hf_debug_set_tuning(int bits) {
  hf_detail::g_h_tune = bits;
  return HF_OK;
}

extern "C" int hf_modconv3x3_f16_rgb_slabs(int cout) {
  return cout <= 0 || (cout % 32) ? 0 : ((cout % 64) ? cout / 32 : cout / 64);
}

extern "C" int hf_debug_set_persistent_blocks(int blocks) {
  hf_detail::g_h_blocks = blocks;
  return HF_OK;
}

extern "C" int hf_modconv3x3_f16_rgb_f32(float *out, const float *x, const void *wt_hi, const void *wt_lo, int nterms,
                                         const float *s, const float *d, const float *noise, const float *noise_w,
                                         long long noise_bstride, const float *bias, int batch, int cin, int cout,
                                         int h, int w, float alpha, float scale, float *rgb_raw, const float *rgb_wt,
                                         const float *rgb_s, void *stream) {
  ConvParams P{};
  if (!out || !x || gen_fill(P, x, nullptr, nullptr, wt_hi, nterms, s, d, batch, cin, cout, h, w) != HF_OK ||
      gen_tail(P, noise, noise_w, noise_bstride, bias, alpha, scale) != HF_OK || !rgb_raw || !rgb_wt || !rgb_s || (cout % 32))
    return HF_E_INVALID;
  P.out = out;
  P.rgb_out = rgb_raw; P.rgb_w = rgb_wt; P.rgb_s = rgb_s;
  P.rgb_slabs = hf_modconv3x3_f16_rgb_slabs(cout);
  return launch_conv_h(P, nterms, false, wt_hi, wt_lo, (hipStream_t)stream);
}

extern "C" int hf_modconv3x3_f16_pre_f32(float *out, const void *x_hi, const void *x_lo, const void *wt_hi,
                                         const void *wt_lo, int nterms, const float *d, const float *noise,
                                         const float *noise_w, long long noise_bstride, const float *bias, int batch,
                                         int cin, int cout, int h, int w, float alpha, float scale, float *rgb_raw,
                                         const float *rgb_wt, const float *rgb_s, void *split_hi, void *split_lo,
                                         const float *s_next, void *stream) {
  ConvParams P{};
  if ((!out && !rgb_raw && !split_hi) || !x_hi ||
      gen_fill(P, nullptr, x_hi, x_lo, wt_hi, nterms, nullptr, d, batch, cin, cout, h, w) != HF_OK ||
      gen_tail(P, noise, noise_w, noise_bstride, bias, alpha, scale) != HF_OK)
    return HF_E_INVALID;
  if ((rgb_raw && (!rgb_wt || !rgb_s || (cout % 32))) || (split_hi && ((cout & 7) || (nterms == 3 && !split_lo)))) return HF_E_INVALID;
  P.out = out;
  P.rgb_out = rgb_raw; P.rgb_w = rgb_wt; P.rgb_s = rgb_s;
  P.rgb_slabs = hf_modconv3x3_f16_rgb_slabs(cout);
  P.oh = split_hi; P.ol = split_lo; P.s_next = s_next;
  return launch_conv_h(P, nterms, false, wt_hi, wt_lo, (hipStream_t)stream);
}

extern "C" int hf_modconv3x3_f16_pre_image_f32(float *image, const void *x_hi, const void *x_lo, const void *wt_hi,
                                               const void *wt_lo, int nterms, const float *d, const float *noise,
                                               const float *noise_w, long long noise_bstride, const float *bias, int batch,
                                               int cin, int cout, int h, int w, float alpha, float scale, const float *rgb_wt,
                                               const float *rgb_s, const float *rgb_bias, const float *skip,
                                               const float *kernel4x4, void *stream) {
  ConvParams P{};
  if (!image || !x_hi || !rgb_wt || !rgb_s || !skip || !kernel4x4 || cin != 32 || cout != 32 || (h & 1) || (w & 1) || !bias ||
      gen_fill(P, nullptr, x_hi, x_lo, wt_hi, nterms, nullptr, d, batch, cin, cout, h, w) != HF_OK ||
      gen_tail(P, noise, noise_w, noise_bstride, bias, alpha, scale) != HF_OK)
    return HF_E_INVALID;
  if (g_force_h || (g_h_tune & 16)) return HF_E_INVALID;
  P.rgb_out = image; P.rgb_w = rgb_wt; P.rgb_s = rgb_s;
  P.rgb_slabs = 1;
  P.rgb_skip = skip; P.rgb_bias = rgb_bias; P.rgb_k4 = kernel4x4;
  return launch_conv_h(P, nterms, false, wt_hi, wt_lo, (hipStream_t)stream);
}

extern "C" int hf_modconv3x3_up_f16_pre_f32(float *tmp, const void *x_hi, const void *x_lo, const void *wt_hi,
                                            const void *wt_lo, int nterms, const float *d, int batch, int cin, int cout,
                                            int h, int w, int tmp_pitch, void *stream) {
  ConvParams P{};
  if (!tmp || !x_hi || gen_fill(P, nullptr, x_hi, x_lo, wt_hi, nterms, nullptr, d, batch, cin, cout, h, w, true, tmp_pitch) != HF_OK)
    return HF_E_INVALID;
  P.out = tmp;
  return launch_conv_h(P, nterms, true, wt_hi, wt_lo, (hipStream_t)stream);
}
```

### hairfastgan_amd/csrc/gemm_h.hip

```cpp
#define HF_WANT_F16_SPLIT
#include "conv_common.h"

using namespace hf_detail;

namespace {

constexpr int KS = 32;
inline int gemm_fill_blocks() { return ((hf_detail::g_h_tune >> 24) & 255) ? ((hf_detail::g_h_tune >> 24) & 255) : 256; }

template <int NTERMS, int PG, int CW>
struct GemmLayout {
  static constexpr int CT = 32 * CW, PT = 64 * PG;
  static constexpr int NPART = (NTERMS == 3) ? 2 : 1;
  static constexpr int W_UNITS = (KS / 8) * CT;
  static constexpr int X_UNITS = (KS / 8) * PT;
  static constexpr int BUF_UNITS = NPART * (W_UNITS + X_UNITS);
  static constexpr int OFF_WL = W_UNITS, OFF_XH = NPART * W_UNITS, OFF_XL = NPART * W_UNITS + X_UNITS;
  static constexpr size_t lds_bytes = (size_t)2 * BUF_UNITS * 16;
};

template <int NTERMS, int PG, bool PRE, bool VSPLIT = false, int CW = 2>
__global__ __launch_bounds__(128 * CW, 2) void gemm1x1_h(const ConvParams P, const _Float16 *__restrict__ wth_all,
                                                 const _Float16 *__restrict__ wtl_all) {
  using L = GemmLayout<NTERMS, PG, CW>;
// ... 23 lines not shown
  const int oplane = P.out_h * P.out_w;
  int t = blockIdx.x;
  const int tx = t % G.tiles_x;
  const int b0 = (t / G.tiles_x) << G.lg_nb;
  const int tx0 = tx << G.lg_tw;
  const long long iplane = (long long)P.h * P.w;
  const float *xb = PRE ? nullptr : P.x + go.x;

  long long e_src[XE];
  long long e_unit[XE];
  int e_sofs[XE];
#pragma unroll
  for (int e = 0; e < XE; ++e) {
    const int i = tid + e * NT;
    const int px = i % PT;
    const int pp = px & ((1 << G.lg_tw) - 1), im = px >> G.lg_tw;
    const int p = tx0 + pp, b = b0 + im;
    e_src[e] = -1;
    e_unit[e] = 0;
    e_sofs[e] = (b < P.batch ? b : 0) * P.s_bstride;
    if (p < oplane && b < P.batch) {
      const int oy = p / P.out_wv, ox = p - oy * P.out_wv;
      e_src[e] = (long long)b * P.cin * iplane + (long long)(oy * P.stride) * P.w + ox * P.stride;
      e_unit[e] = (long long)b * (P.cin >> 3) * iplane + p;
    }
  }

  const int nstages_all = P.cin / KS;
  const int s_begin = (P.splits > 1 && !VSPLIT) ? (int)blockIdx.z * P.chunks_per_split : 0;
  const int s_end = (P.splits > 1 && !VSPLIT) ? min(nstages_all, s_begin + P.chunks_per_split) : nstages_all;

  const unsigned lds_addr0 = hf_lds_addr(lds);
  auto dma_w = [&](int stage, int bufsel) {
#pragma unroll
    for (int j = 0; j < ND; ++j) {
      const int pc = wave + j * NW;
      const int part = pc / (W_UNITS / 64), q = pc % (W_UNITS / 64);
      const int row = q / (CT / 64), half = q % (CT / 64);
      const _Float16 *src = (part ? wtl : wth) + ((long long)(stage * (KS / KH) * 2 + row) * P.cout + co0 + half * 64) * 8;
      hf_glds16_raw_s(src, (unsigned)lane * 16u, lds_addr0 + (unsigned)(bufsel * BUF_UNITS + part * W_UNITS + q * 64) * 16u);
    }
  };
  auto dma_x = [&](int stage, int bufsel) {
#pragma unroll
    for (int e = 0; e < XE; ++e) {
      const int i = tid + e * NT;
      const int kb = i / PT;
      const bool inside = e_src[e] >= 0;
      const long long unit = e_unit[e] + (long long)(stage * (KS / 8) + kb) * iplane;
      const unsigned off = (unsigned)(unit * 16);
      const unsigned dst = lds_addr0 + (unsigned)(bufsel * BUF_UNITS + OFF_XH + (i - lane)) * 16u;
      hf_glds16_raw_s_if(inside, P.xh, off, dst);
      if (NTERMS == 3) hf_glds16_raw_s_if(inside, P.xl, off, dst + (unsigned)X_UNITS * 16u);
    }
  };
  float xr[PRE ? 1 : XE][8];
  auto load_x = [&](int stage) {
    if (PRE) return;
#pragma unroll
    for (int e = 0; e < XE; ++e) {
      const int kb = (tid + e * NT) / PT;
      const float *src = xb + (e_src[e] >= 0 ? e_src[e] : 0) + (long long)(stage * KS + kb * 8) * iplane;
#pragma unroll
      for (int k = 0; k < 8; ++k) xr[PRE ? 0 : e][k] = src[(long long)k * iplane];
    }
  };
  auto convert_x = [&](int stage, half8 *buf) {
    if (PRE) return;
    bool ovf = false;
#pragma unroll
    for (int e = 0; e < XE; ++e) {
      const int i = tid + e * NT;
      const int kb = i / PT;
      half8 hi, lo;
#pragma unroll
      for (int k = 0; k < 8; ++k) {
        const int ci = stage * KS + kb * 8 + k;
        float v = xr[PRE ? 0 : e][k];
        v = fmaf(v, P.s ? P.s[e_sofs[e] + ci] : 1.0f, P.t ? P.t[ci] : 0.0f);
        if (e_src[e] < 0) v = 0.0f;
        _Float16 hv, lv;
        hf_split_f16(v, hv, lv, ovf);
        hi[k] = hv;
        lo[k] = lv;
      }
      buf[OFF_XH + i] = hi;
      if (NTERMS == 3) buf[OFF_XL + i] = lo;
    }
    hf_note_overflow(ovf);
  };

  f32x16 acc[1][1][PG];
  f32x16 vsum[VSPLIT ? PG : 1];
  int slab_left = P.chunks_per_split;
#pragma unroll
  for (int g = 0; g < PG; ++g)
#pragma unroll
    for (int r = 0; r < 16; ++r) {
      acc[0][0][g][r] = 0.0f;
      if (VSPLIT) vsum[VSPLIT ? g : 0][r] = 0.0f;
    }

  if (PRE) {
    half8 z;
#pragma unroll
    for (int k = 0; k < 8; ++k) z[k] = (_Float16)0.0f;
#pragma unroll
    for (int e = 0; e < XE; ++e)
      if (e_src[e] < 0) {
        const int i = tid + e * NT;
#pragma unroll
        for (int bsel = 0; bsel < 2; ++bsel) {
          lds[bsel * BUF_UNITS + OFF_XH + i] = z;
          if (NTERMS == 3) lds[bsel * BUF_UNITS + OFF_XL + i] = z;
        }
      }
  }
  if (s_begin < s_end) {
    dma_w(s_begin, 0);
    if (PRE) dma_x(s_begin, 0);
    load_x(s_begin);
    convert_x(s_begin, lds);
  }
  hf_barrier_keep_young<0>();
  for (int s = s_begin; s < s_end; ++s) {
    const int cb = (s - s_begin) & 1;
    half8 *buf = lds + cb * BUF_UNITS, *nbuf = lds + (cb ^ 1) * BUF_UNITS;
    const bool more = s + 1 < s_end;
    if (more) {
      dma_w(s + 1, cb ^ 1);
      if (PRE) dma_x(s + 1, cb ^ 1);
      load_x(s + 1);
    }
#pragma unroll
    for (int cs = 0; cs < KS / KH; ++cs) {
      const half8 ah = buf[(cs * 2 + lh) * CT + wave_co + li];
      half8 al;
      if (NTERMS == 3) al = buf[OFF_WL + (cs * 2 + lh) * CT + wave_co + li];
#pragma unroll
      for (int g = 0; g < PG; ++g) {
        const int u = (cs * 2 + lh) * PT + (wave_pg + g) * 32 + li;
        const half8 bh = buf[OFF_XH + u];
        HF_MFMA_F16X3(NTERMS, 1, 1, &acc[0][0][g], &ah, &al, &bh, &buf[OFF_XL + u]);
      }
    }
    if (more) convert_x(s + 1, nbuf);
    if (VSPLIT && (--slab_left == 0 || !more)) {
      slab_left = P.chunks_per_split;
#pragma unroll
      for (int g = 0; g < PG; ++g) {
        vsum[VSPLIT ? g : 0] += acc[0][0][g] * w_unscale;
#pragma unroll
        for (int r = 0; r < 16; ++r) acc[0][0][g][r] = 0.0f;
      }
    }
    hf_barrier_keep_young<0>();
  }
#pragma unroll
  for (int g = 0; g < PG; ++g) {
    if (VSPLIT) acc[0][0][g] = vsum[VSPLIT ? g : 0];
    else
#pragma unroll
      for (int r = 0; r < 16; ++r) acc[0][0][g][r] *= w_unscale;
  }
  store_tile_rows<1, PG>(P, G, go, acc, co0 + wave_co, wave_pg, li, lh, 0, tx0, b0);
  if (!VSPLIT && P.splits > 1 && P.counters && splitk_arrive_last(P, reinterpret_cast<int *>(hf_dyn_lds)))
    reduce_tile_rows<1, PG>(P, G, go, co0 + wave_co, wave_pg, li, lh, 0, tx0, b0);
}

thread_local int g_gemm_wide_last = 0;

template <int NTERMS, int PG>
int launch_gemm(ConvParams &P, const _Float16 *wth, const _Float16 *wtl, hipStream_t st) {
  constexpr int PT = 64 * PG;
  const int oplane = P.out_h * P.out_w;
  TileGeom g{};
  g.y0 = 0; g.x0 = 0; g.dh = 1; g.dw = oplane;
  int tw = PT, nb = 1;
  if (oplane < PT && (oplane & (oplane - 1)) == 0) {
    tw = oplane;
    nb = PT / oplane;
    if (nb > pow2_ceil(P.batch)) nb = pow2_ceil(P.batch);
  }
  g.lg_tw = ilog2(tw); g.lg_th = 0; g.lg_nb = ilog2(nb);
  g.tiles_x = hf_cdiv(oplane, tw); g.tiles_y = 1; g.tiles_b = hf_cdiv(P.batch, nb);
  g.first_block = 0;
  P.g[0] = g;
  P.n_geom = 1;
  const int nblocks = g.tiles_x * g.tiles_b;
  const int groups_ = max(1, P.groups);
  const bool wide = PG == 4 && !(g_h_tune & 2) && (P.cout % 128) == 0 &&
                    (long long)nblocks * (P.cout / 128) * groups_ >= 2LL * gemm_fill_blocks();
  if (wide) P.co_tiles = P.cout / 128;
  g_gemm_wide_last = wide ? 1 : 0;
  const size_t lds = wide ? GemmLayout<NTERMS, PG, 4>::lds_bytes : GemmLayout<NTERMS, PG, 2>::lds_bytes;
  P.vsplit = (g_batch_invariant && P.splits > 1 && (long long)nblocks * P.co_tiles * max(1, P.groups) >= gemm_fill_blocks()) ? 1 : 0;
  dim3 grid(nblocks, P.co_tiles * max(1, P.groups), P.vsplit ? 1 : P.splits);
  if (grid.y > 65535 || grid.z > 65535) return HF_E_INVALID;
  P.counters = (P.splits > 1 && !P.vsplit && P.out != P.partial) ? splitk_counters_for((long long)grid.x * grid.y) : nullptr;
  if (P.xh && (P.stride != 1 || P.s || P.t || (NTERMS == 3 && !P.xl) || P.groups > 1 ||
               (long long)P.batch * P.cin * P.h * P.w * 2 >= (1LL << 32)))
    return HF_E_INVALID;
  with_bool(P.xh != nullptr, [&](auto pre) {
    with_bool(wide, [&](auto wd) {
      with_bool(P.vsplit != 0, [&](auto vs) {
        constexpr int CW = decltype(wd)::value ? 4 : 2;
        if constexpr (CW == 2 || PG == 4)
          hipLaunchKernelGGL((gemm1x1_h<NTERMS, PG, decltype(pre)::value, decltype(vs)::value, CW>), grid, dim3(128 * CW), lds, st, P,
                             wth, wtl);
      });
    });
  });
  return hf_launch_status();
}

int gemm_form(bool small, int nterms, ConvParams &P, const _Float16 *hi, const _Float16 *lo, hipStream_t st) {
  return with_bool(small, [&](auto sm) {
    return with_nterms(nterms, [&](auto nt) { return launch_gemm<decltype(nt)::value, decltype(sm)::value ? 2 : 4>(P, hi, lo, st); });
  });
}

}

static long long gemm_blocks(int batch, int cout, int oplane, int groups) {
  const int pt = oplane * (long long)batch <= 128 || oplane <= 128 ? 128 : 256;
  int tw = pt, nb = 1;
  if (oplane < pt && (oplane & (oplane - 1)) == 0) {
    tw = oplane;
    nb = pt / oplane;
    if (nb > pow2_ceil(batch)) nb = pow2_ceil(batch);
  }
  return (long long)hf_cdiv(oplane, tw) * hf_cdiv(batch, nb) * (cout / 64) * (groups > 1 ? groups : 1);
}

static int gemm_splits(int batch, int cin, int cout, int oplane, int groups) {
  const long long blocks = gemm_blocks(hf_detail::plan_batch(batch), cout, oplane, groups);
  const int stages = cin / KS;
  int sk = 1;
  if (blocks < 256 && stages >= 4) {
    sk = (int)((512 + blocks - 1) / blocks);
    if (sk > stages / 2) sk = stages / 2;
    if (sk < 1) sk = 1;
  }
  return sk;
}
static bool gemm_vsplit(int batch, int cout, int oplane, int groups, int sk) {
  return hf_detail::g_batch_invariant && sk > 1 && gemm_blocks(batch, cout, oplane, groups) >= gemm_fill_blocks();
}

extern "C" long long hf_conv1x1_f16_workspace_floats(int batch, int cin, int cout, int h, int w, int stride, int groups) {
  if (batch <= 0 || cin <= 0 || cout <= 0 || h <= 0 || w <= 0 || (stride != 1 && stride != 2) || (cin % KS) || (cout % 64)) return 0;
  const int oh = (h - 1) / stride + 1, ow = (w - 1) / stride + 1;
  const int sk = gemm_splits(batch, cin, cout, oh * ow, groups);
  if (gemm_vsplit(batch, cout, oh * ow, groups, sk)) return 0;
  return sk > 1 ? (long long)sk * (groups > 1 ? groups : 1) * batch * cout * oh * ow : 0;
}

extern "C" int hf_conv1x1_f16_f32(float *out, const float *x, const void *x_hi, const void *x_lo, const void *wt_hi,
                                  const void *wt_lo, int nterms, const float *in_scale, const float *in_shift, const float *out_scale, const float *bias,
                                  int act, const float *slope, float alpha, const float *residual, int batch, int cin,
                                  int cout, int h, int w, int stride, int groups, long long x_group_stride,
                                  float *workspace, long long workspace_floats, void *stream) {
  const int act_kind = act & ~HF_ACT_RESIDUAL_FIRST;
  if (!out || (!x && !x_hi) || !wt_hi || batch <= 0 || cin <= 0 || cout <= 0 || h <= 0 || w <= 0 || (nterms != 1 && nterms != 3) ||
      (nterms == 3 && !wt_lo) || (stride != 1 && stride != 2) || (cin % KS) || (cout % 64) || act_kind < 0 || act_kind > ACT_QGELU ||
      (act_kind == ACT_PRELU && !slope) || groups < 1 || (groups > 1 && (in_scale || in_shift)) ||
      (x_hi && (in_scale || in_shift || stride != 1 || groups > 1 || (nterms == 3 && !x_lo))))
    return HF_E_INVALID;
  ConvParams P{};
  P.out = out; P.x = x; P.xh = x_hi; P.xl = x_lo; P.s = in_scale; P.t = in_shift; P.d = out_scale; P.bias = bias; P.slope = slope;
  P.residual = residual; P.residual_pre = (act & HF_ACT_RESIDUAL_FIRST) ? 1 : 0;
  P.s_bstride = 0; P.d_bstride = 0;
  P.batch = batch; P.cin = cin; P.cout = cout; P.h = h; P.w = w;
  P.stride = stride;
  const int oh = (h - 1) / stride + 1, ow = (w - 1) / stride + 1;
  P.out_h = 1; P.out_w = oh * ow; P.out_wv = ow;
  P.act = act_kind; P.alpha = alpha; P.scale = 1.0f;
  P.groups = groups; P.co_tiles = cout / 64; P.x_gstride = x_group_stride; P.wt_gstride = 0;
  if ((long long)batch * cin * h * w >= (1LL << 40)) return HF_E_INVALID;
  const int oplane = oh * ow;
  const int sk = gemm_splits(batch, cin, cout, oplane, groups);
  P.splits = sk;
  if (sk > 1) {
    const long long slab = (long long)(groups > 1 ? groups : 1) * batch * cout * oplane;
    if (!gemm_vsplit(batch, cout, oplane, groups, sk) && (!workspace || workspace_floats < sk * slab)) return HF_E_WORKSPACE;
    const int stages = cin / KS;
    P.chunks_per_split = (stages + sk - 1) / sk;
    P.splits = (stages + P.chunks_per_split - 1) / P.chunks_per_split;
    P.partial = workspace;
    P.zslab = slab;
  }
  const _Float16 *hi = static_cast<const _Float16 *>(wt_hi), *lo = static_cast<const _Float16 *>(wt_lo);
  const bool small = (long long)oplane * batch <= 128 || oplane <= 128;
  const int rc = gemm_form(small, nterms, P, hi, lo, (hipStream_t)stream);
  if (rc != HF_OK) return rc;
  note_path(7, g_gemm_wide_last ? 6 : (small ? 1 : 2));
  if (P.splits > 1 && !P.vsplit && !P.counters) {
    P.out_h = 1; P.out_w = oplane;
    return launch_splitk_reduce(P, true, (hipStream_t)stream);
  }
  return HF_OK;
}

__global__ __launch_bounds__(256) void small_combine(float *__restrict__ out, const float *__restrict__ y, int splits,
                                                     long long zslab, const float *__restrict__ d,
                                                     const float *__restrict__ noise, const float *__restrict__ noise_w,
                                                     long long noise_bstride, const float *__restrict__ bias, int batch,
                                                     int cout, int h, int w, int up, int out_h, int out_pitch, int out_wv,
                                                     float alpha, float scale) {
#pragma clang fp contract(on)
  const long long oplane = (long long)out_h * out_pitch, iplane = (long long)h * w;
  const long long total = (long long)batch * cout * oplane;
  const long long stride = (long long)gridDim.x * 256;
  const float nw = noise ? noise_w[0] : 0.0f;
  for (long long i = (long long)blockIdx.x * 256 + threadIdx.x; i < total; i += stride) {
    const int ox = (int)(i % out_pitch);
    long long r = i / out_pitch;
    const int oy = (int)(r % out_h);
    r /= out_h;
    const int co = (int)(r % cout), b = (int)(r / cout);
    if (ox >= out_wv) continue;
    float acc = 0.0f;
    const float *yb = y + ((long long)b * 9 * cout + co) * iplane;
#pragma unroll
    for (int ky = 0; ky < 3; ++ky)
#pragma unroll
      for (int kx = 0; kx < 3; ++kx) {
        int sy, sx;
        bool ok;
        if (up) {
          const int ty = oy - ky, tx = ox - kx;
          ok = ty >= 0 && tx >= 0 && !(ty & 1) && !(tx & 1) && (ty >> 1) < h && (tx >> 1) < w;
          sy = ty >> 1;
          sx = tx >> 1;
        } else {
          sy = oy + ky - 1;
          sx = ox + kx - 1;
          ok = sy >= 0 && sy < h && sx >= 0 && sx < w;
        }
        if (ok) {
          const float *src = yb + (long long)(ky * 3 + kx) * cout * iplane + (long long)sy * w + sx;
          float v = 0.0f;
          for (int z = 0; z < splits; ++z) v += src[(long long)z * zslab];
          acc += v;
        }
      }
    float v = acc * (d ? d[(long long)b * cout + co] : 1.0f);
    if (!up) {
      if (noise) v = fmaf(nw, noise[(long long)b * noise_bstride + (long long)oy * out_pitch + ox], v);
      if (bias) v = hf_lrelu(v + bias[co], alpha, scale);
    }
    out[i] = v;
  }
}

extern "C" int hf_split_activation_mod_f16(void *out_hi, void *out_lo, const float *x, const float *scale, long long images,
                                           int channels, int h, int w, void *stream);

static int small_gemm(ConvParams &P, const void *w9_hi, const void *w9_lo, int nterms, const float *x, const float *s,
                      int batch, int cin, int cout, int h, int w, float *workspace, long long workspace_floats,
                      hipStream_t st) {
  P = ConvParams{};
  const long long split_floats = (long long)batch * cin * h * w / 2;
  {
    int sk0 = gemm_splits(batch, cin, 9 * cout, h * w, 1);
    if (gemm_vsplit(batch, 9 * cout, h * w, 1, sk0)) sk0 = 1;
    const long long need = (long long)sk0 * batch * 9 * cout * h * w + 2 * split_floats;
    if (!workspace || workspace_floats < need) return HF_E_WORKSPACE;
    float *xs_hi = workspace + (long long)sk0 * batch * 9 * cout * h * w, *xs_lo = xs_hi + split_floats;
    const int rc = hf_split_activation_mod_f16(xs_hi, nterms == 3 ? xs_lo : nullptr, x, s, batch, cin, h, w, st);
    if (rc != HF_OK) return rc;
    P.xh = xs_hi;
    P.xl = nterms == 3 ? xs_lo : nullptr;
  }
  P.x = x; P.s = nullptr; P.s_bstride = 0; P.d_bstride = 0;
  P.batch = batch; P.cin = cin; P.cout = 9 * cout; P.h = h; P.w = w; P.stride = 1;
  P.out_h = 1; P.out_w = h * w; P.out_wv = w;
  P.act = ACT_NONE; P.scale = 1.0f;
  P.groups = 1; P.co_tiles = 9 * cout / 64;
  const int oplane = h * w;
  int sk = gemm_splits(batch, cin, 9 * cout, oplane, 1);
  const int stages = cin / KS;
  P.chunks_per_split = (stages + sk - 1) / sk;
  sk = (stages + P.chunks_per_split - 1) / P.chunks_per_split;
  P.splits = sk;
  const long long slab = (long long)batch * 9 * cout * oplane;
  if (!workspace || workspace_floats < (long long)(gemm_vsplit(batch, 9 * cout, oplane, 1, sk) ? 1 : sk) * slab) return HF_E_WORKSPACE;
  P.partial = workspace;
  P.zslab = slab;
  P.out = workspace;
  if (sk == 1) P.splits = 1;
  const _Float16 *hi = static_cast<const _Float16 *>(w9_hi), *lo = static_cast<const _Float16 *>(w9_lo);
  bool small = (long long)oplane * batch <= 128 || oplane <= 128;
  if (!small && !(g_h_tune & 2)) {
    const long long n256 = (long long)hf_cdiv(oplane, 256) * batch * (9 * cout / 64) * (gemm_vsplit(batch, 9 * cout, oplane, 1, sk) ? 1 : sk);
    const long long slots = 2LL * gemm_fill_blocks(), tail = n256 % slots;
    small = n256 > slots && tail > 0 && 2 * tail <= slots;
  }
  return gemm_form(small, nterms, P, hi, lo, st);
}

extern "C" long long hf_modconv3x3_small_workspace_floats(int batch, int cin, int cout, int h, int w) {
  if (batch <= 0 || cin <= 0 || cout <= 0 || h <= 0 || w <= 0 || (cin % KS) || (cout % 64)) return 0;
  int sk = gemm_splits(batch, cin, 9 * cout, h * w, 1);
  if (gemm_vsplit(batch, 9 * cout, h * w, 1, sk)) sk = 1;
  return (long long)sk * batch * 9 * cout * h * w + (long long)batch * cin * h * w;
}

extern "C" int hf_modconv3x3_small_f16_f32(float *out, const float *x, const void *w9_hi, const void *w9_lo, int nterms,
                                           const float *s, const float *d, const float *noise, const float *noise_w,
                                           long long noise_bstride, const float *bias, int batch, int cin, int cout, int h,
                                           int w, float alpha, float scale, int upsample, int tmp_pitch, float *workspace,
                                           long long workspace_floats, void *stream) {
  if (!out || !x || !w9_hi || batch <= 0 || cin <= 0 || cout <= 0 || h <= 0 || w <= 0 || (nterms != 1 && nterms != 3) ||
      (nterms == 3 && !w9_lo) || (cin % KS) || (cout % 64) || (noise && !noise_w) || h * w > 1024 ||
      (upsample && (tmp_pitch < 2 * w + 1 || noise || bias)))
    return HF_E_INVALID;
  ConvParams P;
  const int rc = small_gemm(P, w9_hi, w9_lo, nterms, x, s, batch, cin, cout, h, w, workspace, workspace_floats, (hipStream_t)stream);
  if (rc != HF_OK) return rc;
  const int out_h = upsample ? 2 * h + 1 : h, pitch = upsample ? tmp_pitch : w, wv = upsample ? 2 * w + 1 : w;
  const long long total = (long long)batch * cout * out_h * pitch;
  long long g = (total + 255) / 256;
  if (g > 4096) g = 4096;
  hipLaunchKernelGGL(small_combine, dim3((int)g), dim3(256), 0, (hipStream_t)stream, out, workspace, P.vsplit ? 1 : P.splits, P.zslab, d, noise,
                     noise_w, noise_bstride, bias, batch, cout, h, w, upsample ? 1 : 0, out_h, pitch, wv, alpha, scale);
  note_path(7, upsample ? 4 : 3);
  return hf_launch_status();
}


template <bool SPLIT>
__global__ __launch_bounds__(1024) void small_up_blur(float *__restrict__ out, half8 *__restrict__ out_hi,
                                                      half8 *__restrict__ out_lo, const float *__restrict__ y, int splits,
                                                      long long zslab, const float *__restrict__ d,
                                                      const float *__restrict__ kernel4x4, const float *__restrict__ noise,
                                                      const float *__restrict__ noise_w, long long noise_bstride,
                                                      const float *__restrict__ bias, const float *__restrict__ s_next, int cout,
                                                      int h, int w, float alpha, float scale) {
#pragma clang fp contract(on)
  HF_DYN_LDS;
  const int th = 2 * h + 3, tw = 2 * w + 3, tplane = th * tw, iplane = h * w;
  float *T = reinterpret_cast<float *>(hf_dyn_lds);
  float *V = T + 8 * tplane;
  const int cblocks = cout >> 3;
  const int b = blockIdx.x / cblocks, cb = blockIdx.x - b * cblocks;
  constexpr int NT = 1024;
  {
    constexpr int U = 4;
    const int qs = NT / iplane, ps = NT - qs * iplane;
    int ct = threadIdx.x / iplane, p = threadIdx.x - ct * iplane;
    while (ct < 72) {
      const float *src[U];
      float t[U];
      int vi[U];
#pragma unroll
      for (int u = 0; u < U; ++u) {
        const int cc = min(ct, 71);
        const int c = cc / 9, tap = cc - c * 9;
        src[u] = y + ((long long)b * 9 * cout + (long long)tap * cout + cb * 8 + c) * iplane + p;
        vi[u] = ct < 72 ? ct * iplane + p : -1;
        t[u] = 0.0f;
        ct += qs;
        p += ps;
        if (p >= iplane) {
          p -= iplane;
          ++ct;
        }
      }
      for (int z = 0; z < splits; ++z) {
#pragma unroll
        for (int u = 0; u < U; ++u) t[u] += src[u][(long long)z * zslab];
      }
#pragma unroll
      for (int u = 0; u < U; ++u)
        if (vi[u] >= 0) V[vi[u]] = t[u];
    }
  }
  __syncthreads();
  {
    const int dy = NT / tw, dx = NT - dy * tw;
    int c = threadIdx.x / tplane, r = threadIdx.x - c * tplane;
    int ry = r / tw, rx = r - ry * tw;
    while (c < 8) {
      const int oy = ry - 1, ox = rx - 1;
      float v = 0.0f;
      if (oy >= 0 && oy <= 2 * h && ox >= 0 && ox <= 2 * w) {
        float acc = 0.0f;
        const float *vb = V + c * 9 * iplane;
#pragma unroll
        for (int ky = 0; ky < 3; ++ky)
#pragma unroll
          for (int kx = 0; kx < 3; ++kx) {
            const int ty = oy - ky, tx = ox - kx;
            const bool ok = ty >= 0 && tx >= 0 && !(ty & 1) && !(tx & 1) && (ty >> 1) < h && (tx >> 1) < w;
            if (ok) acc += vb[(ky * 3 + kx) * iplane + (ty >> 1) * w + (tx >> 1)];
          }
        v = acc * (d ? d[(long long)b * cout + cb * 8 + c] : 1.0f);
      }
      T[c * tplane + ry * tw + rx] = v;
      rx += dx;
      ry += dy;
      if (rx >= tw) {
        rx -= tw;
        ++ry;
      }
      while (ry >= th) {
        ry -= th;
        ++c;
      }
    }
  }
  __syncthreads();
  float kf[4][4];
#pragma unroll
  for (int ky = 0; ky < 4; ++ky)
#pragma unroll
    for (int kx = 0; kx < 4; ++kx) kf[ky][kx] = kernel4x4[(3 - ky) * 4 + (3 - kx)];
  const int out_h = 2 * h, out_w = 2 * w;
  const float nw = noise ? noise_w[0] : 0.0f;
  const float *nz = noise ? noise + (long long)b * noise_bstride : nullptr;
  bool ovf = false;
  for (int p = threadIdx.x; p < out_h * out_w; p += NT) {
    const int oy = p / out_w, ox = p - oy * out_w;
    const float nzr = nz ? nz[(long long)oy * out_w + ox] : 0.0f;
    float res[8];
#pragma unroll
    for (int c = 0; c < 8; ++c) {
      const float *win = T + c * tplane + oy * tw + ox;
      float acc = 0.0f;
#pragma unroll
      for (int r = 0; r < 4; ++r)
#pragma unroll
        for (int j = 0; j < 4; ++j) acc = fmaf(win[r * tw + j], kf[r][j], acc);
      if (nz) acc = fmaf(nw, nzr, acc);
      if (bias) acc = hf_lrelu(acc + bias[cb * 8 + c], alpha, scale);
      res[c] = acc;
    }
    if (!SPLIT) {
#pragma unroll
      for (int c = 0; c < 8; ++c) out[(((long long)b * cout + cb * 8 + c) * out_h + oy) * out_w + ox] = res[c];
    } else {
      half8 h8, l8;
#pragma unroll
      for (int c = 0; c < 8; ++c) {
        float v = res[c] * (s_next ? s_next[(long long)b * cout + cb * 8 + c] : 1.0f);
        _Float16 hv, lv;
        hf_split_f16(v, hv, lv, ovf);
        h8[c] = hv;
        l8[c] = lv;
      }
      const long long unit = (((long long)b * cblocks + cb) * out_h + oy) * out_w + ox;
      out_hi[unit] = h8;
      if (out_lo) out_lo[unit] = l8;
    }
  }
  if (SPLIT) hf_note_overflow(ovf);
}

extern "C" int hf_modconv3x3_small_up_blur_f16_f32(float *out, void *out_hi, void *out_lo, const float *x, const void *w9_hi,
                                                   const void *w9_lo, int nterms, const float *s, const float *d,
                                                   const float *blur_kernel4x4, const float *noise, const float *noise_w,
                                                   long long noise_bstride, const float *bias, const float *s_next, int batch,
                                                   int cin, int cout, int h, int w, float alpha, float scale, float *workspace,
                                                   long long workspace_floats, void *stream) {
  if ((!out == !out_hi) || !x || !w9_hi || !blur_kernel4x4 || batch <= 0 || cin <= 0 || cout <= 0 || h <= 0 || w <= 0 ||
      (nterms != 1 && nterms != 3) || (nterms == 3 && !w9_lo) || (cin % KS) || (cout % 64) || (noise && !noise_w) || h * w > 1024 ||
      (long long)batch * (cout >> 3) > 0x7fffffffLL)
    return HF_E_INVALID;
  const size_t lds = ((size_t)8 * (2 * h + 3) * (2 * w + 3) + (size_t)72 * h * w) * sizeof(float);
  if (lds > 150 * 1024) return HF_E_INVALID;
  ConvParams P;
  const int rc = small_gemm(P, w9_hi, w9_lo, nterms, x, s, batch, cin, cout, h, w, workspace, workspace_floats, (hipStream_t)stream);
  if (rc != HF_OK) return rc;
  const int splits = P.vsplit ? 1 : P.splits;
  const dim3 grid(batch * (cout >> 3));
  if (out_hi)
    hipLaunchKernelGGL(small_up_blur<true>, grid, dim3(1024), lds, (hipStream_t)stream, nullptr, static_cast<half8 *>(out_hi),
                       static_cast<half8 *>(out_lo), workspace, splits, P.zslab, d, blur_kernel4x4, noise, noise_w, noise_bstride,
                       bias, s_next, cout, h, w, alpha, scale);
  else
    hipLaunchKernelGGL(small_up_blur<false>, grid, dim3(1024), lds, (hipStream_t)stream, out, nullptr, nullptr, workspace, splits,
                       P.zslab, d, blur_kernel4x4, noise, noise_w, noise_bstride, bias, nullptr, cout, h, w, alpha, scale);
  note_path(7, 5);
  return hf_launch_status();
}

#include "conv_rect.h"

extern "C" unsigned long long hf_f16_overflow_count_gemm(int reset) { return hf_f16_overflow_read_tu(reset); }
```

### hairfastgan_amd/stylegan2/model.py

```python
import math
import os
import random

import torch
from torch import nn
from torch.nn import functional as F

from .. import _marshal as M
from .._runtime import conv_nterms, conv_precision, lib, reference_rng_walk, require_gpu, run_guarded, stream
from .op import FusedLeakyReLU, fused_leaky_relu, upfirdn2d


FUSE_BLUR_MIN_H = int(os.environ.get("HAIRFAST_FUSE_BLUR_MIN_H", "128"))


class PixelNorm(nn.Module):
    def forward(self, input):
        require_gpu(input)
        return M.pixel_norm(lib(), stream(), input)


def make_kernel(k):
    k = torch.tensor(k, dtype=torch.float32)
    if k.ndim == 1:
        k = k[None, :] * k[:, None]
    return k / k.sum()


class Upsample(nn.Module):
    def __init__(self, kernel, factor=2):
        super().__init__()
        self.factor = factor
        self.register_buffer("kernel", make_kernel(kernel) * (factor ** 2))
        p = self.kernel.shape[0] - factor
        self.pad = ((p + 1) // 2 + factor - 1, p // 2)

    def forward(self, input):
        return upfirdn2d(input, self.kernel, up=self.factor, down=1, pad=self.pad)


class Downsample(nn.Module):
    def __init__(self, kernel, factor=2):
        super().__init__()
        self.factor = factor
        self.register_buffer("kernel", make_kernel(kernel))
        p = self.kernel.shape[0] - factor
        self.pad = ((p + 1) // 2, p // 2)

    def forward(self, input):
        return upfirdn2d(input, self.kernel, up=1, down=self.factor, pad=self.pad)


class Blur(nn.Module):
    def __init__(self, kernel, pad, upsample_factor=1):
        super().__init__()
        kernel = make_kernel(kernel)
        if upsample_factor > 1:
            kernel = kernel * (upsample_factor ** 2)
        self.register_buffer("kernel", kernel)
        self.pad = pad

    def forward(self, input):
        return upfirdn2d(input, self.kernel, pad=self.pad)


class EqualLinear(nn.Module):
    def __init__(self, in_dim, out_dim, bias=True, bias_init=0, lr_mul=1, activation=None):
        super().__init__()
        self.weight = nn.Parameter(torch.randn(out_dim, in_dim).div_(lr_mul))
        self.bias = nn.Parameter(torch.zeros(out_dim).fill_(bias_init)) if bias else None
        self.activation = activation
        self.scale = (1 / math.sqrt(in_dim)) * lr_mul
        self.lr_mul = lr_mul

    def forward(self, input):
        require_gpu(input)
        return M.equal_linear(lib(), stream(), input, self.weight.detach(),
                              None if self.bias is None else self.bias.detach(), self.lr_mul, bool(self.activation))


class ModulatedConv2d(nn.Module):
    def __init__(self, in_channel, out_channel, kernel_size, style_dim, demodulate=True, upsample=False,
                 downsample=False, blur_kernel=[1, 3, 3, 1]):
        super().__init__()
        if downsample:
            raise NotImplementedError("downsample=True is Discriminator-only in the reference (out of scope)")
        if kernel_size not in (1, 3):
            raise NotImplementedError("kernel_size must be 1 (ToRGB) or 3 (StyledConv)")
        if upsample and kernel_size != 3:
            raise NotImplementedError("upsample needs kernel_size 3")
        if kernel_size == 1 and (out_channel != 3 or demodulate):
            raise NotImplementedError("the 1x1 modulated conv exists only as ToRGB (3 outputs, no demodulation)")
        self.eps = 1e-8
        self.kernel_size = kernel_size
        self.in_channel = in_channel
        self.out_channel = out_channel
        self.upsample = upsample
        self.downsample = downsample
        if upsample:
            factor = 2
            p = (len(blur_kernel) - factor) - (kernel_size - 1)
            self.blur = Blur(blur_kernel, pad=((p + 1) // 2 + factor - 1, p // 2 + 1), upsample_factor=factor)
        self.scale = 1 / math.sqrt(in_channel * kernel_size ** 2)
        self.padding = kernel_size // 2
        self.weight = nn.Parameter(torch.randn(1, out_channel, in_channel, kernel_size, kernel_size))
        self.modulation = EqualLinear(style_dim, in_channel, bias_init=1)
        self.demodulate = demodulate
        self._prep = None
        self._prep_f16 = None
        self._coeffs = None
        self.register_load_state_dict_post_hook(lambda m, _ik: m.invalidate())

    def invalidate(self):
        self._prep = self._prep_f16 = self._coeffs = None

    def __repr__(self):
        return (f"{self.__class__.__name__}({self.in_channel}, {self.out_channel}, {self.kernel_size}, "
                f"upsample={self.upsample}, downsample={self.downsample})")

    def prepared(self):
        w = self.weight
        key = (w.data_ptr(), None if w.is_inference() else w._version, w.device)
        if self._prep is None or self._prep[0] != key:
            require_gpu(w)
            wt, wsq = M.prepare_weights(lib(), stream(), w.detach())
            self._prep = (key, wt, wsq)
        return self._prep[1], self._prep[2]

    def prepared_f16(self):
        wt, _ = self.prepared()
        key = self._prep[0]
        if self._prep_f16 is None or self._prep_f16[0] != key:
            hi, lo = M.split_weights_f16(lib(), stream(), wt)
            self._prep_f16 = (key, hi, lo)
        return self._prep_f16[1], self._prep_f16[2]

    def prepared_small(self):
        wt, _ = self.prepared()
        key = self._prep[0]
        cached = self.__dict__.get("_prep_small")
        if cached is None or cached[0] != key:
            cached = self.__dict__["_prep_small"] = (key, M.split_weights_small(lib(), stream(), wt))
        return cached[1]

    def route_same_res(self, shape, plain=True):
        b, cin, h, w = shape
        cout = self.out_channel
        if conv_precision() == "f32":
            return "f32", False
        if plain and M.modconv3x3_small_supported(cin, cout, h, w, b):
            return "small", False
        if M.modconv3x3_f16_supported(cin, cout, h, w, batch=b):
            return "f16", not self.upsample and self.kernel_size == 3 and M.torgb_fusable(cin, cout, h, w)
        return "f32", False

    def route_up(self, shape, is_split=False, tail=True):
        b, cin, h, w = shape
        cout = self.out_channel
        if conv_precision() == "f32":
            return "f32"
        if h >= FUSE_BLUR_MIN_H and tail and M.modconv3x3_up_fused_supported(cin, cout, h, w) and self.blur_factors() is not None:
            return "fused"
        if not is_split and M.modconv3x3_small_supported(cin, cout, h, w, b, upsample=True):
            return "small"
        return "f16" if M.modconv3x3_up_f16_supported(cin, cout, h, w, batch=b) else "f32"

    def conv_same_res(self, input, wt, s, d, noise, noise_w, bias, alpha=0.2, scale=math.sqrt(2), rgb=None):
        kernel, _ = self.route_same_res(input.shape, plain=rgb is None)
        if kernel == "small":
            return M.modconv3x3_small(lib(), stream(), input, self.prepared_small(), conv_nterms(), s, d, noise, noise_w, bias,
                                      self.out_channel, alpha, scale)
        if kernel == "f16":
            hi, lo = self.prepared_f16()
            return M.modconv3x3_f16(lib(), stream(), input, hi, lo, conv_nterms(), s, d, noise, noise_w, bias, alpha, scale, rgb=rgb)
        assert rgb is None
        return M.modconv3x3(lib(), stream(), input, wt, s, d, noise, noise_w, bias, alpha, scale)

    def fuses_torgb(self, input):
        return self.route_same_res(input.shape, plain=False)[1]

    def blur_factors(self):
        k = self.blur.kernel
        key = (k.data_ptr(), k._version if not k.is_inference() else None)
        cached = self.__dict__.get("_blur_fac")
        if cached is None or cached[0] != key:
            if torch.cuda.is_current_stream_capturing():
                return None if cached is None else cached[1]
            cached = self.__dict__["_blur_fac"] = (key, M.blur_factors(k))
        return cached[1]

    def conv_up(self, input, wt, s, d, noise, noise_w, bias, alpha=0.2, scale=math.sqrt(2), split_for=None):
        route = self.route_up(input.shape, isinstance(input, M.SplitActivation),
                              tail=noise is not None and bias is not None and 0.0 <= alpha <= 1.0)
        if route == "fused":
            hi, lo = self.prepared_f16()
            return M.modconv3x3_up_fused(lib(), stream(), input, hi, lo, s, d, self.blur_factors(), noise, noise_w, bias, alpha, scale,
                                         split_for=None if split_for is None else split_for[1], nterms=conv_nterms())
        f16 = small = None
        if route == "small":
            small = (self.prepared_small(), conv_nterms())
        elif route == "f16":
            f16 = (*self.prepared_f16(), conv_nterms())
        return M.modconv3x3_up(lib(), stream(), input, wt, s, d, self.blur.kernel, noise, noise_w, bias, alpha, scale,
                               f16=f16, split_for=split_for, small=small)

    def style_coefficients(self, style):
        pre = self._coeffs
        if pre is not None and pre[0] == (style.data_ptr(), tuple(style.shape), tuple(style.stride())):
            return pre[1]
        wt, wsq = self.prepared()
        s = M.modulation(lib(), stream(), style, self.modulation.weight.detach(), self.modulation.bias.detach())
        d = None
        if self.demodulate:
            d = M.demod(lib(), stream(), s, wsq)
            M.style_normalize(lib(), stream(), s, d)
        return wt, s, d

    def forward(self, input, style):
        require_gpu(input, style)
        wt, s, d = self.style_coefficients(style)
        if self.kernel_size == 1:
            return M.torgb(lib(), stream(), input, wt, s, None, None, None)
        if self.upsample:
            if tuple(self.blur.pad) != (1, 1) or tuple(self.blur.kernel.shape) != (4, 4):
                raise NotImplementedError("fused upsampling path expects the [1,3,3,1] blur with pad (1,1)")
            return self.conv_up(input, wt, s, d, None, None, None)
        return self.conv_same_res(input, wt, s, d, None, None, None)


class NoiseInjection(nn.Module):
    def __init__(self):
        super().__init__()
        self.weight = nn.Parameter(torch.zeros(1))

    def forward(self, image, noise=None):
        require_gpu(image)
        if noise is None:
            batch, _, height, width = image.shape
            noise = image.new_empty(batch, 1, height, width).normal_()
        return M.noise_bias_act(lib(), stream(), image, noise, self.weight.detach(), None, 1.0, 1.0)


class ConstantInput(nn.Module):
    def __init__(self, channel, size=4):
        super().__init__()
        self.input = nn.Parameter(torch.randn(1, channel, size, size))

    def forward(self, input):
        return self.input.repeat(input.shape[0], 1, 1, 1)


class StyledConv(nn.Module):
    def __init__(self, in_channel, out_channel, kernel_size, style_dim, upsample=False,
                 blur_kernel=[1, 3, 3, 1], demodulate=True):
        super().__init__()
        self.conv = ModulatedConv2d(in_channel, out_channel, kernel_size, style_dim, upsample=upsample,
                                    blur_kernel=blur_kernel, demodulate=demodulate)
        self.noise = NoiseInjection()
        self.activate = FusedLeakyReLU(out_channel)

    def forward(self, input, style, noise=None):
        return self._run(input, style, noise, None)

    def forward_rgb(self, input, style, noise, rgb):
        return self._run(input, style, noise, rgb)

    def _run(self, input, style, noise, rgb):
        require_gpu(input, style, noise)
        conv = self.conv
        wt, s, d = conv.style_coefficients(style)
        b, _, h, w = input.shape
        oh, ow = (2 * h, 2 * w) if conv.upsample else (h, w)
        if noise is None:
            noise = input.new_empty(b, 1, oh, ow).normal_()
        act = self.activate
        if conv.upsample:
            assert rgb is None
            return conv.conv_up(input, wt, s, d, noise, self.noise.weight.detach(), act.bias.detach(),
                                act.negative_slope, act.scale)
        if rgb is None:
            return conv.conv_same_res(input, wt, s, d, noise, self.noise.weight.detach(), act.bias.detach(),
                                      act.negative_slope, act.scale)
        rgb_wt, rgb_s = rgb
        return conv.conv_same_res(input, wt, s, d, noise, self.noise.weight.detach(), act.bias.detach(),
                                  act.negative_slope, act.scale, rgb=(rgb_wt, rgb_s))

    def forward_split(self, input, style, noise, s_next, coeffs=None):
        pre = isinstance(input, M.SplitActivation)
        require_gpu(None if pre else input, style, noise)
        conv = self.conv
        assert conv.upsample
        wt, s, d = conv.style_coefficients(style) if coeffs is None else coeffs
        b, _, h, w = input.shape
        if noise is None:
            noise = style.new_empty(b, 1, 2 * h, 2 * w).normal_()
        act = self.activate
        return conv.conv_up(input, wt, s, d, noise, self.noise.weight.detach(), act.bias.detach(),
                            act.negative_slope, act.scale, split_for=(None, s_next, conv_precision() == "f16x3"))

    def forward_image(self, split, coeffs, noise, rgb, to_rgb, skip):
        conv, act = self.conv, self.activate
        _, s, d = coeffs
        b, _, h, w = split.shape
        if noise is None:
            noise = split.hi.new_empty(b, 1, h, w, dtype=torch.float32).normal_()
        require_gpu(noise, skip)
        hi, lo = conv.prepared_f16()
        return M.modconv3x3_f16_pre_image(lib(), stream(), split, hi, lo, conv_nterms(), d, noise, self.noise.weight.detach(),
                                          act.bias.detach(), rgb, to_rgb.bias.detach(), skip, to_rgb._skip_kernel(skip),
                                          act.negative_slope, act.scale)

    def forward_from_split(self, split, coeffs, noise=None, rgb=None, want_out=True, split_for=None):
        conv = self.conv
        assert not conv.upsample
        _, s, d = coeffs
        b, _, h, w = split.shape
        if noise is None:
            noise = split.hi.new_empty(b, 1, h, w, dtype=torch.float32).normal_()
        require_gpu(noise)
        act = self.activate
        hi, lo = conv.prepared_f16()
        return M._modconv3x3_f16_pre(lib(), stream(), split, hi, lo, conv_nterms(), d, noise, self.noise.weight.detach(),
                                     act.bias.detach(), act.negative_slope, act.scale, rgb=rgb, want_out=want_out,
                                     split_for=split_for)


def _observed(*modules):
    for m in modules:
        for sub in m.modules():
            if sub._forward_hooks or sub._forward_pre_hooks:
                return True
    return False


class ToRGB(nn.Module):
    def __init__(self, in_channel, style_dim, upsample=True, blur_kernel=[1, 3, 3, 1]):
        super().__init__()
        if upsample:
            self.upsample = Upsample(blur_kernel)
        self.conv = ModulatedConv2d(in_channel, 3, 1, style_dim, demodulate=False)
        self.bias = nn.Parameter(torch.zeros(1, 3, 1, 1))

    def _skip_kernel(self, skip):
        if skip is None:
            return None
        kern = self.upsample.kernel
        if tuple(kern.shape) != (4, 4) or self.upsample.factor != 2 or tuple(self.upsample.pad) != (2, 1):
            raise NotImplementedError("fused skip path expects the [1,3,3,1] x2 upsampler")
        return kern

    def forward(self, input, style, skip=None):
        require_gpu(input, style, skip)
        wt, s, _ = self.conv.style_coefficients(style)
        return M.torgb(lib(), stream(), input, wt, s, self.bias.detach(), skip, self._skip_kernel(skip))

    def coefficients(self, style):
        wt, s, _ = self.conv.style_coefficients(style)
        return wt, s

    def finish(self, raw, skip=None):
        require_gpu(raw, skip)
        slabs = raw.shape[1] // 3
        eye = getattr(self, "_eye", None)
        if eye is None or eye.device != raw.device or eye.shape[1] != 3 * slabs:
            eye = self._eye = torch.eye(3, device=raw.device, dtype=raw.dtype).repeat(slabs, 1).reshape(1, 3 * slabs, 3)
        return M.torgb(lib(), stream(), raw, eye, None, self.bias.detach(), skip, self._skip_kernel(skip))


class Generator(nn.Module):
    def __init__(self, size, style_dim, n_mlp, channel_multiplier=2, blur_kernel=[1, 3, 3, 1], lr_mlp=0.01):
        super().__init__()
        self.size = size
        self.style_dim = style_dim
        layers = [PixelNorm()]
        for _ in range(n_mlp):
            layers.append(EqualLinear(style_dim, style_dim, lr_mul=lr_mlp, activation="fused_lrelu"))
        self.style = nn.Sequential(*layers)
        self.channels = {4: 512, 8: 512, 16: 512, 32: 512, 64: 256 * channel_multiplier,
                         128: 128 * channel_multiplier, 256: 64 * channel_multiplier,
                         512: 32 * channel_multiplier, 1024: 16 * channel_multiplier}
        self.input = ConstantInput(self.channels[4])
        self.conv1 = StyledConv(self.channels[4], self.channels[4], 3, style_dim, blur_kernel=blur_kernel)
        self.to_rgb1 = ToRGB(self.channels[4], style_dim, upsample=False)
        self.log_size = int(math.log(size, 2))
        self.num_layers = (self.log_size - 2) * 2 + 1
        self.convs = nn.ModuleList()
        self.upsamples = nn.ModuleList()
        self.to_rgbs = nn.ModuleList()
        self.noises = nn.Module()
        for layer_idx in range(self.num_layers):
            res = (layer_idx + 5) // 2
            self.noises.register_buffer(f"noise_{layer_idx}", torch.randn(1, 1, 2 ** res, 2 ** res))
        in_channel = self.channels[4]
        for i in range(3, self.log_size + 1):
            out_channel = self.channels[2 ** i]
            self.convs.append(StyledConv(in_channel, out_channel, 3, style_dim, upsample=True,
                                         blur_kernel=blur_kernel))
            self.convs.append(StyledConv(out_channel, out_channel, 3, style_dim, blur_kernel=blur_kernel))
            self.to_rgbs.append(ToRGB(out_channel, style_dim))
            in_channel = out_channel
        self.n_latent = self.log_size * 2 - 2
        self.register_load_state_dict_post_hook(lambda m, _ik: m.__dict__.pop("_style_jobs", None) and None)

    def make_noise(self):
        device = self.input.input.device
        noises = [torch.randn(1, 1, 2 ** 2, 2 ** 2, device=device)]
        for i in range(3, self.log_size + 1):
            for _ in range(2):
                noises.append(torch.randn(1, 1, 2 ** i, 2 ** i, device=device))
        return noises

    def mean_latent(self, n_latent):
        latent_in = torch.randn(n_latent, self.style_dim, device=self.input.input.device)
        return self.style(latent_in).mean(0, keepdim=True)

    def get_latent(self, input):
        return self.style(input)

    def forward(self, styles, return_latents=False, inject_index=None, truncation=1, truncation_latent=None,
                input_is_latent=False, noise=None, randomize_noise=True, layer_in=None, skip=None,
                start_layer=0, end_layer=8, return_rgb=False):
        if not input_is_latent:
            styles = [self.style(s) for s in styles]
        if noise is None:
            if randomize_noise:
                noise = [None] * self.num_layers
            else:
                noise = [getattr(self.noises, f"noise_{i}") for i in range(self.num_layers)]
        if truncation < 1:
            styles = [truncation_latent + truncation * (s - truncation_latent) for s in styles]
        if len(styles) < 2:
            inject_index = self.n_latent
            latent = styles[0].unsqueeze(1).repeat(1, inject_index, 1) if styles[0].ndim < 3 else styles[0]
        else:
            if inject_index is None:
                inject_index = random.randint(1, self.n_latent - 1)
            latent = torch.cat([styles[0].unsqueeze(1).repeat(1, inject_index, 1),
                                styles[1].unsqueeze(1).repeat(1, self.n_latent - inject_index, 1)], 1)

        if layer_in is None or tuple(layer_in.shape[-2:]) == (2 ** (start_layer + 1),) * 2:
            noise = self._draw_noise(noise, latent, start_layer, end_layer)

        def run():
            styled = self._batch_styles(latent)
            try:
                return self._run_layers(latent, noise, layer_in, skip, start_layer, end_layer, return_latents)
            finally:
                for conv in styled:
                    conv._coeffs = None

        return run_guarded(run)

    def _draw_noise(self, noise, latent, start_layer, end_layer):
        if any(n is not None for n in noise) or not latent.is_cuda or reference_rng_walk():
            return noise
        b = latent.shape[0]
        run = [i for i in range(self.num_layers)
               if (i == 0 and start_layer == 0) or (i > 0 and max(start_layer, 1) <= (i + 1) // 2 and
                                                    ((i + 1) // 2 <= end_layer or (i + 1) // 2 == start_layer))]
        if not run:
            return noise
        sizes = [b * (2 ** ((i + 5) // 2)) ** 2 for i in run]
        flat = torch.empty(sum(sizes), device=latent.device, dtype=torch.float32).normal_()
        out, o = list(noise), 0
        for i, n in zip(run, sizes):
            r = 2 ** ((i + 5) // 2)
            out[i] = flat[o:o + n].view(b, 1, r, r)
            o += n
        return out

    def _batch_styles(self, latent):
        if latent.ndim != 3 or latent.shape[1] < self.n_latent or not latent.is_cuda:
            return []
        convs, rows = [self.conv1.conv, self.to_rgb1.conv], [0, 1]
        for block in range(1, self.log_size - 1):
            i = 2 * block - 1
            convs += [self.convs[2 * block - 2].conv, self.convs[2 * block - 1].conv, self.to_rgbs[block - 1].conv]
            rows += [i, i + 1, i + 2]
        b = latent.shape[0]
        for c in convs:
            c.prepared()
        key = (b, latent.device, tuple(c.modulation.weight.data_ptr() for c in convs), tuple(c._prep[1].data_ptr() for c in convs))
        cache = self.__dict__.setdefault("_style_jobs", {})
        if key not in cache:
            if torch.cuda.is_current_stream_capturing():
                return []
            if len(cache) > 16:
                cache.clear()
            table, layout, total = M.style_job_table(convs, rows, b, latent.device)
            cache[key] = (table, layout, total, max(c.in_channel for c in convs),
                          max(c.out_channel for c in convs if c.demodulate))
        table, layout, total, mci, mco = cache[key]
        lat = latent if (latent.dtype == torch.float32 and latent.stride(-1) == 1) else latent.float().contiguous()
        res = M.style_batch(lib(), stream(), lat, table, layout, total, mci, mco)
        for conv, row, (sv, dv) in zip(convs, rows, res):
            view = latent[:, row]
            conv._coeffs = ((view.data_ptr(), tuple(view.shape), tuple(view.stride())), (conv.prepared()[0], sv, dv))
        return convs

    def _fast_block(self, block, src, mid_shape, fuses, latent, noise, skip, up_coeffs, end_layer):
        conv_up, conv_same, to_rgb = self.convs[2 * block - 2], self.convs[2 * block - 1], self.to_rgbs[block - 1]
        i = 2 * block - 1
        coeffs = conv_same.conv.style_coefficients(latent[:, i + 1])
        split = conv_up.forward_split(src, latent[:, i], noise[2 * block - 1], coeffs[1],
                                      coeffs=up_coeffs if isinstance(src, M.SplitActivation) else None)
        rgb = to_rgb.coefficients(latent[:, i + 2]) if fuses else None
        is_last = block == self.log_size - 2
        s_up = None
        if not is_last and block + 1 <= end_layer:
            nup, nsame = self.convs[2 * block], self.convs[2 * block + 1]
            up_shape = (mid_shape[0], conv_same.conv.out_channel) + mid_shape[2:]
            next_mid = (mid_shape[0], nup.conv.out_channel, 2 * mid_shape[2], 2 * mid_shape[3])
            if (nup.conv.route_up(up_shape, is_split=True) != "f32" and nsame.conv.route_same_res(next_mid, plain=False)[0] == "f16"
                    and not _observed(nup, nsame)):
                up_coeffs = nup.conv.style_coefficients(latent[:, i + 2])
                s_up = up_coeffs[1]
        fused_rgb = rgb is not None and not _observed(to_rgb)
        want_out = not fused_rgb or (not is_last and s_up is None)
        if (fused_rgb and not want_out and s_up is None and skip is not None and M.image_fusable(mid_shape[1], conv_same.conv.out_channel, *mid_shape[2:])
                and conv_same.activate.bias is not None):
            image = conv_same.forward_image(split, coeffs, noise[2 * block], rgb, to_rgb, skip)
            if image is not None:
                return None, image, None, up_coeffs
        out, raw, split_in = conv_same.forward_from_split(split, coeffs, noise[2 * block], rgb=rgb if fused_rgb else None,
                                                          want_out=want_out, split_for=s_up)
        skip = to_rgb.finish(raw, skip) if raw is not None else to_rgb(out, latent[:, i + 2], skip)
        return out, skip, split_in, up_coeffs

    def _run_layers(self, latent, noise, layer_in, skip, start_layer, end_layer, return_latents):
        out = self.input(latent)
        if start_layer == 0:
            out = self.conv1(out, latent[:, 0], noise=noise[0])
            skip = self.to_rgb1(out, latent[:, 1])
        if end_layer == 0:
            return out, skip
        split_in = up_coeffs = None
        for block in range(1, self.log_size - 1):
            if block < start_layer:
                continue
            if block != start_layer and block > end_layer:
                return out, skip
            conv_up, conv_same, to_rgb = self.convs[2 * block - 2], self.convs[2 * block - 1], self.to_rgbs[block - 1]
            i = 2 * block - 1
            src = layer_in if block == start_layer else (split_in if split_in is not None else out)
            mid_shape = (src.shape[0], conv_up.conv.out_channel, 2 * src.shape[2], 2 * src.shape[3])
            kernel, fuses = conv_same.conv.route_same_res(mid_shape, plain=False)
            if kernel == "f16" and not _observed(conv_up, conv_same):
                out, skip, split_in, up_coeffs = self._fast_block(block, src, mid_shape, fuses, latent, noise, skip, up_coeffs, end_layer)
            else:
                assert not isinstance(src, M.SplitActivation)
                split_in = None
                out = conv_up(src, latent[:, i], noise=noise[2 * block - 1])
                if fuses and not _observed(conv_same, to_rgb):
                    out, raw = conv_same.forward_rgb(out, latent[:, i + 1], noise[2 * block], to_rgb.coefficients(latent[:, i + 2]))
                    skip = to_rgb.finish(raw, skip)
                else:
                    out = conv_same(out, latent[:, i + 1], noise=noise[2 * block])
                    skip = to_rgb(out, latent[:, i + 2], skip)
        image = skip
        return (image, latent) if return_latents else (image, None)
```

### include/hairfast_hip.h

```cpp
#ifndef HAIRFAST_HIP_H
#define HAIRFAST_HIP_H

#ifdef __cplusplus
extern "C" {
#endif

#define HF_OK 0
#define HF_E_INVALID (-1)
#define HF_E_LAUNCH (-2)
#define HF_E_WORKSPACE (-3)

#define HF_ACT_RESIDUAL_FIRST 16

const char *hf_strerror(int code);
int hf_abi_version(void);

int hf_upfirdn2d_f32(float *out, const float *in, const float *kernel, int major, int in_h, int in_w,
                     int kh, int kw, int up_x, int up_y, int down_x, int down_y, int pad_x0, int pad_x1,
                     int pad_y0, int pad_y1, void *stream);

int hf_fused_bias_act_f32(float *out, const float *x, const float *bias, long long n, int n_bias,
                          int step_b, float alpha, float scale, void *stream);

int hf_noise_bias_act_f32(float *out, const float *x, const float *noise, const float *noise_w,
                          const float *bias, int batch, int channels, int hw, long long noise_bstride,
                          float alpha, float scale, void *stream);

int hf_modconv_prepare_f32(float *wt, float *wsq, const float *weight, int cout, int cin, int k,
                           void *stream);

int hf_modulation_f32(float *s, const float *latent, long long lat_stride, const float *mod_w,
                      const float *mod_b, int batch, int cin, int style_dim, void *stream);

int hf_demod_f32(float *d, const float *s, const float *wsq, int batch, int cin, int cout, void *stream);

int hf_style_normalize_f32(float *s, float *d, int batch, int cin, int cout, void *stream);

int hf_modconv3x3_f32(float *out, const float *x, const float *wt, const float *s, const float *d,
                      const float *noise, const float *noise_w, long long noise_bstride,
                      const float *bias, int batch, int cin, int cout, int h, int w, float alpha,
                      float scale, float *workspace, long long workspace_floats, void *stream);

typedef struct hf_style_job {
  const float *mod_w;
  const float *mod_b;
  const float *wsq;
  int cin, cout;
  int style_row, reserved;
  long long s_ofs, d_ofs;
} hf_style_job;
int hf_style_batch_f32(float *out, const float *latent, long long lat_bstride, long long lat_rstride,
                       const hf_style_job *jobs, int n_jobs, int batch, int style_dim, int max_cin, int max_cout,
                       void *stream);

int hf_conv_split_weights_f16(void *wt_hi, void *wt_lo, const float *wt, int cin, int cout, void *stream);
int hf_conv_split_weights_f16_taps(void *wt_hi, void *wt_lo, const float *wt, int cin, int cout, int taps, void *stream);
long long hf_f16_overflow_count(int reset);
int hf_modconv3x3_f16_f32(float *out, const float *x, const void *wt_hi, const void *wt_lo, int nterms,
                          const float *s, const float *d, const float *noise, const float *noise_w,
                          long long noise_bstride, const float *bias, int batch, int cin, int cout, int h,
                          int w, float alpha, float scale, void *stream);
int hf_modconv3x3_f16_rgb_slabs(int cout);
int hf_modconv3x3_f16_rgb_f32(float *out, const float *x, const void *wt_hi, const void *wt_lo, int nterms,
                              const float *s, const float *d, const float *noise, const float *noise_w,
                              long long noise_bstride, const float *bias, int batch, int cin, int cout, int h,
                              int w, float alpha, float scale, float *rgb_raw, const float *rgb_wt,
                              const float *rgb_s, void *stream);
int hf_modconv3x3_f16_pre_f32(float *out, const void *x_hi, const void *x_lo, const void *wt_hi, const void *wt_lo,
                              int nterms, const float *d, const float *noise, const float *noise_w,
                              long long noise_bstride, const float *bias, int batch, int cin, int cout, int h, int w,
                              float alpha, float scale, float *rgb_raw, const float *rgb_wt, const float *rgb_s,
                              void *split_hi, void *split_lo, const float *s_next, void *stream);
int hf_modconv3x3_f16_pre_image_f32(float *image, const void *x_hi, const void *x_lo, const void *wt_hi, const void *wt_lo,
                                    int nterms, const float *d, const float *noise, const float *noise_w,
                                    long long noise_bstride, const float *bias, int batch, int cin, int cout, int h, int w,
                                    float alpha, float scale, const float *rgb_wt, const float *rgb_s, const float *rgb_bias,
                                    const float *skip, const float *kernel4x4, void *stream);
int hf_modconv3x3_up_f16_pre_f32(float *tmp, const void *x_hi, const void *x_lo, const void *wt_hi, const void *wt_lo,
                                 int nterms, const float *d, int batch, int cin, int cout, int h, int w, int tmp_pitch,
                                 void *stream);
int hf_modconv3x3_up_f16_f32(float *tmp, const float *x, const void *wt_hi, const void *wt_lo, int nterms,
                             const float *s, const float *d, int batch, int cin, int cout, int h, int w,
                             int tmp_pitch, void *stream);

int hf_modconv3x3_up_blur_f16_f32(float *out, void *split_hi, void *split_lo, const float *x, const void *x_hi,
                                  const void *x_lo, const void *wt_hi, const void *wt_lo, const float *s, const float *d,
                                  const float *blur_k1d_x, const float *blur_k1d_y, const float *noise, const float *noise_w,
                                  long long noise_bstride, const float *bias, const float *s_next, int batch, int cin, int cout,
                                  int h, int w, float alpha, float scale, void *stream);

long long hf_modconv_workspace_floats(int batch, int cin, int cout, int h, int w, int upsample);

int hf_modconv3x3_up_f32(float *tmp, const float *x, const float *wt, const float *s, const float *d,
                         int batch, int cin, int cout, int h, int w, int tmp_pitch, float *workspace,
                         long long workspace_floats, void *stream);
int hf_modconv_up_pitch(int w);

int hf_blur_noise_bias_act_f32(float *out, const float *in, const float *kernel4x4, const float *noise,
                               const float *noise_w, long long noise_bstride, const float *bias,
                               int batch, int channels, int in_h, int in_w, int in_pitch, float alpha,
                               float scale, void *stream);

int hf_blur_noise_bias_act_split_f16(void *out_hi, void *out_lo, const float *in, const float *kernel4x4,
                                     const float *noise, const float *noise_w, long long noise_bstride,
                                     const float *bias, const float *s_next, int batch, int channels, int in_h,
                                     int in_w, int in_pitch, float alpha, float scale, void *stream);

int hf_torgb_f32(float *out, const float *x, const float *wt, const float *s, const float *bias,
                 const float *skip, const float *kernel4x4, int batch, int cin, int h, int w,
                 void *stream);


int hf_conv_prepare_f32(float *wt, const float *weight, int cout, int cin, int k, float scale, void *stream);

int hf_bn_fold_f32(float *scale, float *shift, const float *gamma, const float *beta, const float *mean,
                   const float *var, const float *conv_bias, float eps, int n, void *stream);

int hf_conv2d_f32(float *out, const float *x, const float *wt, const float *in_scale, const float *in_shift,
                  const float *out_scale, const float *bias, int act, const float *slope, float alpha,
                  const float *residual, int batch, int cin, int cout, int h, int w, int k, int stride,
                  int groups, long long x_group_stride, float *workspace, long long workspace_floats,
                  void *stream);
long long hf_conv2d_workspace_floats(int batch, int cin, int cout, int h, int w, int k, int stride, int groups);

int hf_conv2d_f16_f32(float *out, const float *x, const void *x_hi, const void *x_lo, const void *wt_hi,
                      const void *wt_lo, int nterms, const float *in_scale, const float *in_shift,
                      const float *out_scale, const float *bias, int act, const float *slope, float alpha,
                      const float *residual, int batch, int cin, int cout, int h, int w, int stride, int groups,
                      long long x_group_stride, float *workspace, long long workspace_floats, void *stream);
long long hf_conv2d_f16_workspace_floats(int batch, int cin, int cout, int h, int w, int stride, int groups);
int hf_conv2d_f16_split_f32(float *out, void *out_hi, void *out_lo, const float *next_scale, const float *next_shift,
                            const float *x, const void *x_hi, const void *x_lo, const void *wt_hi, const void *wt_lo,
                            int nterms, const float *in_scale, const float *in_shift, const float *out_scale,
                            const float *bias, int act, const float *slope, float alpha, const float *residual, int batch,
                            int cin, int cout, int h, int w, int stride, void *stream);
int hf_scale_shortcut_add_split_f16(float *out, void *out_hi, void *out_lo, const float *next_scale, const float *next_shift,
                                    const float *r, const float *gate, const float *shortcut, int sc_stride, int batch, int channels,
                                    int oh, int ow, int sh, int sw, void *stream);
int hf_conv2d_f16_split_output_ok(int batch, int cin, int cout, int h, int w, int stride, int nterms, int presplit_input);
int hf_conv1x1_f16_f32(float *out, const float *x, const void *x_hi, const void *x_lo, const void *wt_hi,
                       const void *wt_lo, int nterms, const float *in_scale, const float *in_shift, const float *out_scale, const float *bias, int act,
                       const float *slope, float alpha, const float *residual, int batch, int cin, int cout, int h, int w,
                       int stride, int groups, long long x_group_stride, float *workspace, long long workspace_floats,
                       void *stream);
long long hf_conv1x1_f16_workspace_floats(int batch, int cin, int cout, int h, int w, int stride, int groups);
int hf_modconv3x3_small_f16_f32(float *out, const float *x, const void *w9_hi, const void *w9_lo, int nterms, const float *s,
                                const float *d, const float *noise, const float *noise_w, long long noise_bstride,
                                const float *bias, int batch, int cin, int cout, int h, int w, float alpha, float scale,
                                int upsample, int tmp_pitch, float *workspace, long long workspace_floats, void *stream);
long long hf_modconv3x3_small_workspace_floats(int batch, int cin, int cout, int h, int w);
int hf_modconv3x3_small_up_blur_f16_f32(float *out, void *out_hi, void *out_lo, const float *x, const void *w9_hi,
                                        const void *w9_lo, int nterms, const float *s, const float *d,
                                        const float *blur_kernel4x4, const float *noise, const float *noise_w,
                                        long long noise_bstride, const float *bias, const float *s_next, int batch, int cin,
                                        int cout, int h, int w, float alpha, float scale, float *workspace,
                                        long long workspace_floats, void *stream);
int hf_split_activation_f16(void *out_hi, void *out_lo, const float *x, const float *in_scale, const float *in_shift,
                            long long images, int channels, int h, int w, void *stream);

int hf_split_activation_mod_f16(void *out_hi, void *out_lo, const float *x, const float *scale, long long images,
                                int channels, int h, int w, void *stream);

int hf_plane_mean_f32(float *out, const float *x, int planes, int hw, void *stream);
int hf_se_gate_f32(float *gate, const float *pooled, const float *fc1, const float *fc2, int batch, int channels,
                   int reduced, void *stream);
int hf_scale_shortcut_add_f32(float *out, const float *r, const float *gate, const float *shortcut,
                              int sc_stride, int batch, int channels, int oh, int ow, int sh, int sw,
                              void *stream);
int hf_upsample_bilinear_add_f32(float *out, const float *x, const float *y, int planes, int h, int w, int oh,
                                 int ow, void *stream);
int hf_adaptive_avgpool_f32(float *out, const float *x, int batch, int channels, int h, int w, int oh, int ow,
                            int out_channels_total, int out_channel_offset, void *stream);
int hf_downscale2x_f32(float *out, const float *x, int planes, int h, int w, void *stream);
int hf_linear_f32(float *out, const float *x, long long x_stride, const float *w, const float *bias, int batch,
                  int in_features, int out_features, float scale, void *stream);
int hf_equal_linear_f32(float *out, const float *x, long long x_stride, const float *w, const float *bias, int batch,
                        int in_features, int out_features, float lr_mul, int fused_lrelu, float alpha, float act_scale,
                        void *stream);
int hf_pixel_norm_f32(float *out, const float *x, int rows, int dim, void *stream);
int hf_maxpool3x3s2_f32(float *out, const float *x, long long planes, int h, int w, void *stream);
int hf_gate_f32(float *out, const float *x, const float *logit, const float *add_plane, const float *add_bcast,
                float plus_one, long long planes, int hw, void *stream);
int hf_upsample_nearest_f32(float *out, const float *x, long long planes, int h, int w, int oh, int ow, void *stream);
int hf_parsing_mask_i64(long long *out, const float *logits, const int *remap, int images, int classes, int h, int w,
                        int full_h, int full_w, int out_h, int out_w, void *stream);

int hf_sample_layernorm_f32(float *out, const float *x, const float *gamma, const float *beta, int batch, int channels,
                            int hw, long long x_batch_stride, float eps, float slope, float *workspace,
                            long long workspace_floats, void *stream);
long long hf_sample_layernorm_workspace_floats(int batch, int channels, int hw);
int hf_bicubic_down_f32(float *out, const float *x, const float *k1d, long long planes, int h, int w, int factor,
                        void *stream);
int hf_dilate_erode_f32(float *dilated, float *eroded, const float *mask, long long planes, int h, int w, int radius,
                        void *stream);

int hf_quantize_u8_f32(unsigned char *out, const float *x, long long n, void *stream);
int hf_poisson_setup_u8(float *b, float *x0, const unsigned char *src, const unsigned char *tgt, const unsigned char *mask,
                        int images, int channels, int h, int w, void *stream);
int hf_poisson_jacobi_f32(float *x_out, const float *x_in, const float *b, const unsigned char *mask, int images, int channels,
                          int h, int w, int sweeps, int tblock, void *stream);
int hf_poisson_finish_u8(unsigned char *out, const float *x, const unsigned char *tgt, const unsigned char *mask, int images,
                         int channels, int h, int w, void *stream);

int hf_resize_lanczos_u8(unsigned char *out, unsigned char *mid, const unsigned char *in, int planes, int h_in, int w_in,
                         int h_out, int w_out, const int *bounds_x, const int *kk_x, int ksize_x, const int *bounds_y,
                         const int *kk_y, int ksize_y, void *stream);
int hf_quad_bilinear_u8(unsigned char *out, const unsigned char *src, const double *coef8, int planes, int h, int w, int oh,
                        int ow, void *stream);
int hf_quad_lanczos4_u8(unsigned char *out, const unsigned char *src, const double *coef8, int planes, int h, int w, int osize,
                        const int *bounds, const int *kk, int ksize, void *stream);
int hf_quad_lanczos4_ratio(void);
int hf_align_pad_blur_f32(float *out, float *tmp, const unsigned char *src, const double *weights, int radius,
                          const float *mask_x, const float *mask_y, int planes, int h, int w, int pad_left, int pad_top,
                          int pad_right, int pad_bottom, void *stream);
int hf_align_pad_finish_u8(unsigned char *out, float *pre, const float *img, const float *median, const float *mask_x,
                           const float *mask_y, int planes, int h, int w, void *stream);
int hf_u8_to_unit_f32(float *out, const unsigned char *in, long long n, void *stream);

int hf_paste_quad_u8(unsigned char *photo, const unsigned char *src, const unsigned char *mask, const double *coef8, int planes,
                     int h, int w, int n, int x0, int y0, int x1, int y1, void *stream);
int hf_multiply_u8(unsigned char *out, const unsigned char *a, const unsigned char *b, long long n, void *stream);

int hf_image_to_bytes_f32(unsigned char *out, const float *in, int batch, int h, int w, float lo, float hi, int round_half,
                          int interleaved, void *stream);
int hf_labels_to_rgb_i64(unsigned char *out, const long long *labels, long long n_pixels, const unsigned char *palette,
                         int n_colors, int unknown_label, void *stream);

long long hf_png_bound(int h, int w, int channels);
int hf_png_segment_rows(int h, int w, int channels);
long long hf_png_workspace_bytes(int batch, int h, int w, int channels);
int hf_png_encode_u8(unsigned char *out, long long out_stride, long long *sizes, const unsigned char *in, int batch, int h,
                     int w, int channels, int filter, void *workspace, long long workspace_bytes, void *stream);

long long hf_jpeg_bound(int h, int w, int channels, int subsampling);
int hf_jpeg_chunk_mcus(int channels, int subsampling);
long long hf_jpeg_workspace_bytes(int batch, int h, int w, int channels, int subsampling);
int hf_jpeg_encode_u8(unsigned char *out, long long out_stride, long long *sizes, const unsigned char *in, int batch, int h,
                      int w, int channels, int quality, int subsampling, void *workspace, long long workspace_bytes,
                      void *stream);

long long hf_jpeg_decode_workspace_bytes(int batch, int h, int w, int components, int hs, int vs, int restart_interval,
                                         long long max_scan_bytes);
int hf_jpeg_decode_u8(unsigned char *out, float *out_f32, int *status, const unsigned char *scans, long long scans_bytes,
                      const long long *scan_offsets, long long max_scan_bytes, const unsigned char *tables, int batch, int h, int w,
                      int components, int hs, int vs, int restart_interval, int out_channels, int sub_bytes, void *workspace,
                      long long workspace_bytes, void *stream);

long long hf_png_decode_workspace_bytes(int batch, int h, int w, int color_type, long long max_stream_bytes);
int hf_png_decode_u8(unsigned char *out, float *out_f32, int *status, const unsigned char *streams, long long streams_bytes,
                     const long long *stream_offsets, long long max_stream_bytes, const unsigned char *palettes, int batch, int h,
                     int w, int color_type, int out_channels, int token_cap, void *workspace, long long workspace_bytes,
                     void *stream);

int hf_layernorm_f32(float *out, const float *x, const float *gamma, const float *beta, int rows, int dim, float eps,
                     int lrelu, float alpha, void *stream);
int hf_layernorm_grouped_f32(float *out, const float *x, const float *gamma, const float *beta, int rows, int dim, int groups,
                             float eps, int lrelu, float alpha, void *stream);
int hf_modulate_f32(float *out, const float *x, const float *gamma, const float *beta, long long n, int lrelu, float alpha,
                    void *stream);
int hf_pixel_norm_dim1_f32(float *out, const float *x, int batch, int layers, int dim, void *stream);
int hf_axpby_bcast_f32(float *out, const float *a, float alpha, const float *b, float beta, long long n, long long b_period,
                       void *stream);
int hf_add_bcast_f32(float *out, const float *a, const float *b, long long n, long long b_period, void *stream);

int hf_label_conv3x3_f32(float *out, const int *labels, const float *table, const float *bias, int batch, int channels,
                         int h, int w, int table_cols, int cols_per_sample, int group, int relu, float *tap_sum_scratch,
                         void *stream);
int hf_ace_modulate_f32(float *out, const float *x, const float *noise, const float *noise_var, const float *bn_scale,
                        const float *bn_shift, const float *avg, const float *sp, const float *blend, int batch,
                        int channels, int hw, int group, float slope, int x_upsample_w, void *stream);
int hf_ace_modulate_table_f32(float *out, const float *x, const float *noise, const float *noise_var, const float *bn_scale,
                              const float *bn_shift, const int *labels, const float *table, const float *avg_bias,
                              const float *sp, const float *blend, int batch, int channels, int h, int w, int table_cols,
                              int n_labels, int group, float slope, int interior, int x_upsample, void *stream);
int hf_region_mean_f32(float *out, const float *x, const int *labels, int batch, int channels, int h, int w, int n_labels,
                       long long batch_stride, long long plane_stride, int pitch, int act, void *stream);
int hf_tanh_f32(float *out, const float *x, long long n, void *stream);

int hf_stem7x7s2_f16_f32(float *out, const float *x, const void *w_hi, const void *w_lo, const float *w_unscale,
                         const float *out_scale, const float *bias, float alpha, int batch, int h, int w, int cout, int pool,
                         void *stream);

int hf_channel_layernorm_f32(float *out, const float *x, const float *gamma, const float *beta, int channels,
                             long long tokens, float eps, void *stream);
int hf_mha_small_f32(float *out, const float *qkv, int images, int seq, int heads, int head_dim, void *stream);
int hf_quick_gelu_f32(float *out, const float *x, long long n, void *stream);

int hf_frechet_accumulate_f64(double *sum, double *cov_sum, const float *feats, int n, int d, void *stream);
int hf_frechet_accumulate_f16_f64(double *sum, double *cov_sum, const void *feats, int n, int d, void *stream);
int hf_frechet_stats_f64(double *mu, double *cov, const double *sum, const double *cov_sum, long long n, int d, void *stream);
int hf_sym_eig_jacobi_f64(double *w, double *v, const double *a, double *work, int d, int max_sweeps, int *sweeps, double *off_norm,
                          void *stream);
long long hf_sym_eig_jacobi_work_doubles(int d, int want_vectors);
int hf_frechet_congruence_f64(double *m_out, const double *w, const double *v, const double *s2, double *work, int d, void *stream);
int hf_frechet_finish_f64(double *out, const double *mu1, const double *mu2, const double *s1, const double *s2, const double *ev,
                          int d, void *stream);

int hf_conv2d_direct_f32(float *out, const float *x, const float *weight, const float *in_scale, const float *in_shift,
                         const float *bias, int act, float alpha, int n, int cin, int cout, int h, int w, int k, int stride, int pad,
                         void *stream);
int hf_maxpool2d_f32(float *out, const float *x, long long planes, int h, int w, int k, int stride, void *stream);
int hf_lpips_layer_f64(double *dist, const float *fx, const float *fy, const float *lin_w, double *work, int n, int c, int h, int w,
                       int accumulate, void *stream);
long long hf_lpips_layer_work_doubles(int n, int h, int w);
int hf_sq_err_sum_f64(double *out, const void *a, const void *b, double *work, int n, long long per_image, int is_u8, void *stream);
long long hf_sq_err_sum_work_doubles(int n, long long per_image);

int hf_ssim_planes_f64(double *sum_s, double *sum_aux, double *map, double *next_x, double *next_y, const void *x, const void *y,
                       const float *mask, const double *taps, double *work, int dtype, int planes, int channels, int h, int w,
                       int win, double c1, double c2, double cn, void *stream);
long long hf_ssim_work_doubles(int planes, int h, int w, int win);
int hf_ssim_tile(int axis);

int hf_crop_avgpool_f32(float *out, const float *x, const float *scale, const float *shift, int n, int c, int h, int w, int y0,
                        int x0, int ch, int cw, int oh, int ow, void *stream);
int hf_l2_normalize_rows_f32(float *out, float *norms, const float *x, int rows, int d, void *stream);
int hf_row_similarity_f64(double *out, const float *a, const float *b, int n, int m, int d, int paired, void *stream);

int hf_conv2d_rect_f16_f32(float *out, const float *x, const float *weight, const void *wt_hi, const void *wt_lo, int nterms,
                           const float *out_scale, const float *bias, int act, int batch, int cin, int cout, int h, int w, int kh,
                           int kw, int stride, int pad_top, int pad_left, int out_h, int out_w, int xc0, int x_ctotal, int oc0,
                           int o_ctotal, void *stream);
int hf_pool3x3_f32(float *out, const float *x, int mode, int n, int c, int h, int w, int stride, int xc0, int x_ctotal, int oc0,
                   int o_ctotal, void *stream);
int hf_resize_bilinear_tf1_f32(float *out, const void *x, int is_u8, int n, int c, int h, int w, int oh, int ow, int affine,
                               float mul, float add, void *stream);

int hf_debug_set_dispatch(int same_cfg, int up_cfg);
int hf_debug_last_path(void);
int hf_debug_set_persistent_blocks(int blocks);
int hf_debug_set_tuning(int bits);
int hf_set_batch_invariant(int on);
int hf_set_splitk_counters(void *zeroed_ints, int n_ints);
int hf_profile_marker(int id, void *stream);

#ifdef __cplusplus
}
#endif
#endif
```

Before: 1728 images/s.

## Fold constant-input head conv and chain split activations through small-plane blocks

```diff
diff --git a/hairfastgan_amd/_lib.py b/hairfastgan_amd/_lib.py
--- a/hairfastgan_amd/_lib.py
+++ b/hairfastgan_amd/_lib.py
@@ -25,6 +25,10 @@
     "hf_conv_split_weights_f16_taps": [_f, _f, _f, _i, _i, _i, _st],
     "hf_modconv3x3_small_f16_f32": [_f, _f, _f, _f, _i, _f, _f, _f, _f, _ll, _f, _i, _i, _i, _i, _i, _fl, _fl, _i, _i, _f, _ll, _st],
     "hf_modconv3x3_small_up_blur_f16_f32": [_f, _f, _f, _f, _f, _f, _i, _f, _f, _f, _f, _f, _ll, _f, _f, _i, _i, _i, _i, _i, _fl, _fl, _f, _ll, _st],
+    "hf_modconv3x3_small_split_f16_f32": [_f, _f, _f, _f, _f, _f, _f, _f, _i, _f, _f, _f, _f, _ll, _f, _f, _i, _i, _i, _i, _i, _fl, _fl, _f, _ll, _st],
+    "hf_modconv3x3_small_up_blur_pre_f16_f32": [_f, _f, _f, _f, _f, _f, _f, _f, _i, _f, _f, _f, _f, _f, _ll, _f, _f, _i, _i, _i, _i, _i, _fl, _fl, _f, _ll, _st],
+    "hf_head_fold_prepare_f32": [_f, _f, _f, _i, _i, _i, _i, _i, _st],
+    "hf_head_fold_forward_f32": [_f, _f, _f, _f, _f, _f, _f, _f, _ll, _f, _f, _i, _i, _i, _i, _fl, _fl, _st],
     "hf_conv1x1_f16_f32": [_f, _f, _f, _f, _f, _f, _i, _f, _f, _f, _f, _i, _f, _fl, _f, _i, _i, _i, _i, _i, _i, _i, _ll, _f, _ll, _st],
     "hf_modconv3x3_f16_f32": [_f, _f, _f, _f, _i, _f, _f, _f, _f, _ll, _f, _i, _i, _i, _i, _i, _fl, _fl, _st],
     "hf_modconv3x3_f16_rgb_f32": [_f, _f, _f, _f, _i, _f, _f, _f, _f, _ll, _f, _i, _i, _i, _i, _i, _fl, _fl, _f, _f, _f, _st],
diff --git a/hairfastgan_amd/_marshal.py b/hairfastgan_amd/_marshal.py
--- a/hairfastgan_amd/_marshal.py
+++ b/hairfastgan_amd/_marshal.py
@@ -8,6 +8,7 @@
 from ._runtime import CANON_BATCH, plan_batch
 
 SQRT2 = 2 ** 0.5
+HF_E_UNSUPPORTED = -4
 
 PROFILE = None
 
@@ -39,6 +40,8 @@
     e0.record()
     r = fn()
     e1.record()
+    if isinstance(r, int) and r != 0:
+        return r
     if label is None:
         code = lib.hf_debug_last_path()
         label = KERNEL_NAMES.get(code, f"conv_mfma (general, code {code})")
@@ -279,7 +282,7 @@
         lambda: lib.hf_modconv3x3_f16_pre_image_f32(_p(image), _p(act.hi), _p(act.lo), _p(wt_hi), _p(wt_lo), nterms, _p(d), _p(noise),
                                                     _p(_c(noise_w)), nbs, _p(_c(bias)), b, cin, cout, h, w, alpha, scale, _p(rgb_wt),
                                                     _p(rgb_s), _p(_c(rgb_bias)), _p(skip), _p(_c(up_kernel)), st), nbytes=nb)
-    if code == -1:
+    if code == HF_E_UNSUPPORTED:
         return None
     check(lib, code, "hf_modconv3x3_f16_pre_image_f32")
     return image
@@ -379,29 +382,52 @@
     return cin % 32 == 0 and cout % 64 == 0 and h * w <= 256 and plan_batch(batch) * h * w <= 4096 and cin * cout >= 512 * 512
 
 
-def modconv3x3_small(lib, st, x, w9, nterms, s, d, noise, noise_w, bias, cout, alpha=0.2, scale=SQRT2, upsample=False):
-    x = _c(x)
+def modconv3x3_small(lib, st, x, w9, nterms, s, d, noise, noise_w, bias, cout, alpha=0.2, scale=SQRT2, upsample=False,
+                     split_for=None):
+    pre = isinstance(x, SplitActivation)
+    if not pre:
+        x = _c(x)
     b, cin, h, w = x.shape
+    like = x.hi if pre else x
     hi, lo = w9
     n = lib.hf_modconv3x3_small_workspace_floats(b, cin, cout, h, w)
-    ws = x.new_empty((max(n, 1),))
+    ws = like.new_empty((max(n, 1),), dtype=torch.float32)
     if upsample:
+        if split_for is not None:
+            raise ValueError("split_for needs the same-resolution form")
         pitch = lib.hf_modconv_up_pitch(w)
-        out = x.new_empty((b, cout, 2 * h + 1, pitch))
+        out = like.new_empty((b, cout, 2 * h + 1, pitch), dtype=torch.float32)
         noise = bias = noise_w = None
         nbs = 0
     else:
         pitch = 0
-        out = x.new_empty((b, cout, h, w))
+        out = like.new_empty((b, cout, h, w), dtype=torch.float32)
         noise, nbs = _noise_args(noise, b, h * w)
+    if not pre and split_for is None:
+        code = _launch_profiled(
+            lib, 2.0 * cin * cout * 9 * h * w * b,
+            lambda: lib.hf_modconv3x3_small_f16_f32(_p(out), _p(x), _p(hi), _p(lo), nterms, _p(_c(s)), _p(_c(d)), _p(noise),
+                                                    _p(_c(noise_w)), nbs, _p(_c(bias)), b, cin, cout, h, w, alpha, scale,
+                                                    1 if upsample else 0, pitch, _p(ws), n, st),
+            label="gemm_h tap-GEMM (small planes)")
+        check(lib, code, "hf_modconv3x3_small_f16_f32")
+        return out
+    if upsample:
+        raise ValueError("a SplitActivation input needs the same-resolution or the fused upsampling form")
+    split = s_next = None
+    if split_for is not None:
+        s_next = _c(split_for[1])
+        split = SplitActivation.empty(b, cout, h, w, like.device, want_lo=split_for[2] if len(split_for) > 2 else True,
+                                      key=split_for[0])
     code = _launch_profiled(
         lib, 2.0 * cin * cout * 9 * h * w * b,
-        lambda: lib.hf_modconv3x3_small_f16_f32(_p(out), _p(x), _p(hi), _p(lo), nterms, _p(_c(s)), _p(_c(d)), _p(noise),
-                                                _p(_c(noise_w)), nbs, _p(_c(bias)), b, cin, cout, h, w, alpha, scale,
-                                                1 if upsample else 0, pitch, _p(ws), n, st),
+        lambda: lib.hf_modconv3x3_small_split_f16_f32(_p(out), *_hl(split), None if pre else _p(x), *_hl(x if pre else None), _p(hi),
+                                                      _p(lo), nterms, None if pre else _p(_c(s)), _p(_c(d)), _p(noise),
+                                                      _p(_c(noise_w)), nbs, _p(_c(bias)), _p(s_next), b, cin, cout, h, w, alpha,
+                                                      scale, _p(ws), n, st),
         label="gemm_h tap-GEMM (small planes)")
-    check(lib, code, "hf_modconv3x3_small_f16_f32")
-    return out
+    check(lib, code, "hf_modconv3x3_small_split_f16_f32")
+    return out if split_for is None else (out, split)
 
 
 SMALL_UP_FUSED = os.environ.get("HAIRFAST_SMALL_UP_FUSED", "1") != "0"
@@ -413,19 +439,32 @@
 
 def modconv3x3_small_up_blur(lib, st, x, w9, nterms, s, d, blur_kernel, noise, noise_w, bias, cout, alpha=0.2, scale=SQRT2,
                              split_for=None):
-    x = _c(x)
+    pre = isinstance(x, SplitActivation)
+    if not pre:
+        x = _c(x)
     b, cin, h, w = x.shape
+    like = x.hi if pre else x
     hi, lo = w9
     n = lib.hf_modconv3x3_small_workspace_floats(b, cin, cout, h, w)
-    ws = x.new_empty((max(n, 1),))
+    ws = like.new_empty((max(n, 1),), dtype=torch.float32)
     noise, nbs = _noise_args(noise, b, 4 * h * w)
     out = split = s_next = None
     if split_for is not None:
         s_next = _c(split_for[1])
-        split = SplitActivation.empty(b, cout, 2 * h, 2 * w, x.device, want_lo=split_for[2] if len(split_for) > 2 else True,
+        split = SplitActivation.empty(b, cout, 2 * h, 2 * w, like.device, want_lo=split_for[2] if len(split_for) > 2 else True,
                                       key=split_for[0])
     else:
-        out = x.new_empty((b, cout, 2 * h, 2 * w))
+        out = like.new_empty((b, cout, 2 * h, 2 * w), dtype=torch.float32)
+    if pre:
+        code = _launch_profiled(
+            lib, 2.0 * cin * cout * 9 * h * w * b,
+            lambda: lib.hf_modconv3x3_small_up_blur_pre_f16_f32(_p(out), *_hl(split), None, *_hl(x), _p(hi), _p(lo), nterms, None,
+                                                                _p(_c(d)), _p(_c(blur_kernel)), _p(noise), _p(_c(noise_w)), nbs,
+                                                                _p(_c(bias)), _p(s_next), b, cin, cout, h, w, alpha, scale, _p(ws), n,
+                                                                st),
+            label="gemm_h tap-GEMM (small planes)")
+        check(lib, code, "hf_modconv3x3_small_up_blur_pre_f16_f32")
+        return out if split_for is None else split
     code = _launch_profiled(
         lib, 2.0 * cin * cout * 9 * h * w * b,
         lambda: lib.hf_modconv3x3_small_up_blur_f16_f32(_p(out), *_hl(split), _p(x), _p(hi), _p(lo), nterms, _p(_c(s)), _p(_c(d)),
@@ -434,6 +473,44 @@
         label="gemm_h tap-GEMM (small planes)")
     check(lib, code, "hf_modconv3x3_small_up_blur_f16_f32")
     return out if split_for is None else split
+
+
+def head_fold_prepare(lib, st, wt, const):
+    wt, const = _c(wt), _c(const)
+    taps, cin, cout = wt.shape
+    k = int(round(taps ** 0.5))
+    _, cc, h, w = const.shape
+    if k * k != taps or cc != cin or const.shape[0] != 1:
+        raise ValueError(f"head_fold_prepare: weight {tuple(wt.shape)} does not fit the constant {tuple(const.shape)}")
+    a = wt.new_empty((cout, h * w, cin))
+    check(lib, lib.hf_head_fold_prepare_f32(_p(a), _p(wt), _p(const), cin, cout, h, w, k, st), "hf_head_fold_prepare_f32")
+    return a
+
+
+def head_fold_supported(cin, cout, plane):
+    return cin % 4 == 0 and cout % 4 == 0 and 16 * plane * (cin + 4) + 32 * cin + 128 * plane <= 160 * 1024
+
+
+def head_fold_forward(lib, st, a, hw, s, d, noise, noise_w, bias, alpha=0.2, scale=SQRT2, split_for=None):
+    cout, plane, cin = a.shape
+    s = _c(s)
+    b = s.shape[0]
+    noise, nbs = _noise_args(noise, b, plane)
+    out = a.new_empty((b, cout, hw[0], hw[1]))
+    split = s_next = None
+    if split_for is not None:
+        s_next = _c(split_for[1])
+        split = SplitActivation.empty(b, cout, hw[0], hw[1], a.device, want_lo=split_for[2] if len(split_for) > 2 else True,
+                                      key=split_for[0])
+    code = _launch_profiled(
+        lib, 2.0 * cin * cout * plane * b,
+        lambda: lib.hf_head_fold_forward_f32(_p(out), *_hl(split), _p(a), _p(s), _p(_c(d)), _p(noise), _p(_c(noise_w)), nbs,
+                                             _p(_c(bias)), _p(s_next), b, cin, cout, plane, alpha, scale, st),
+        label="head_fold_forward", nbytes=4.0 * a.numel() + 4.0 * out.numel())
+    if code == HF_E_UNSUPPORTED:
+        return None
+    check(lib, code, "hf_head_fold_forward_f32")
+    return out if split_for is None else (out, split)
 
 
 def modconv3x3_up_f16_supported(cin, cout, h, w, batch=None):
diff --git a/hairfastgan_amd/csrc/api.hip b/hairfastgan_amd/csrc/api.hip
--- a/hairfastgan_amd/csrc/api.hip
+++ b/hairfastgan_amd/csrc/api.hip
@@ -6,6 +6,7 @@
     case HF_E_INVALID: return "invalid argument";
     case HF_E_LAUNCH: return "kernel launch failed";
     case HF_E_WORKSPACE: return "workspace too small";
+    case HF_E_UNSUPPORTED: return "declined: another entry point takes this launch";
     default: return "unknown error";
   }
 }
diff --git a/hairfastgan_amd/csrc/convh.hip b/hairfastgan_amd/csrc/convh.hip
--- a/hairfastgan_amd/csrc/convh.hip
+++ b/hairfastgan_amd/csrc/convh.hip
@@ -1069,7 +1069,7 @@
 int launch_conv_h(ConvParams &P, int nterms, bool up, const void *wth, const void *wtl, hipStream_t st) {
   const _Float16 *h = static_cast<const _Float16 *>(wth), *l = static_cast<const _Float16 *>(wtl);
   if (!h || (nterms == 3 && !l)) return HF_E_INVALID;
-  int cfg, rc;
+  int cfg, rc = HF_OK;
   if (up) {
     cfg = (P.cout % 64) ? 63 : 61;
     rc = P.xh ? launch_form<true, true>(cfg, nterms, P, h, l, st) : launch_form<true, false>(cfg, nterms, P, h, l, st);
@@ -1091,7 +1091,7 @@
         return rc;
       }
     }
-    if (P.rgb_skip) return HF_E_INVALID;
+    if (P.rgb_skip) return rc == HF_E_LAUNCH ? rc : HF_E_UNSUPPORTED;
     rc = launch_form<false, true>(cfg, nterms, P, h, l, st);
     if (rc == HF_OK) note_path(5, cfg + 20);
     return rc;
@@ -1260,7 +1260,7 @@
       gen_fill(P, nullptr, x_hi, x_lo, wt_hi, nterms, nullptr, d, batch, cin, cout, h, w) != HF_OK ||
       gen_tail(P, noise, noise_w, noise_bstride, bias, alpha, scale) != HF_OK)
     return HF_E_INVALID;
-  if (g_force_h || (g_h_tune & 16)) return HF_E_INVALID;
+  if (g_force_h || (g_h_tune & 16)) return HF_E_UNSUPPORTED;
   P.rgb_out = image; P.rgb_w = rgb_wt; P.rgb_s = rgb_s;
   P.rgb_slabs = 1;
   P.rgb_skip = skip; P.rgb_bias = rgb_bias; P.rgb_k4 = kernel4x4;
diff --git a/hairfastgan_amd/csrc/gemm_h.hip b/hairfastgan_amd/csrc/gemm_h.hip
--- a/hairfastgan_amd/csrc/gemm_h.hip
+++ b/hairfastgan_amd/csrc/gemm_h.hip
@@ -349,6 +349,46 @@
   return HF_OK;
 }
 
+__device__ __forceinline__ float small_combine_value(const float *__restrict__ y, int splits, long long zslab,
+                                                     const float *__restrict__ d, const float *__restrict__ noise, float nw,
+                                                     long long noise_bstride, const float *__restrict__ bias, int b, int co,
+                                                     int oy, int ox, int cout, int h, int w, int up, int out_pitch, float alpha,
+                                                     float scale) {
+#pragma clang fp contract(on)
+  const long long iplane = (long long)h * w;
+  float acc = 0.0f;
+  const float *yb = y + ((long long)b * 9 * cout + co) * iplane;
+#pragma unroll
+  for (int ky = 0; ky < 3; ++ky)
+#pragma unroll
+    for (int kx = 0; kx < 3; ++kx) {
+      int sy, sx;
+      bool ok;
+      if (up) {
+        const int ty = oy - ky, tx = ox - kx;
+        ok = ty >= 0 && tx >= 0 && !(ty & 1) && !(tx & 1) && (ty >> 1) < h && (tx >> 1) < w;
+        sy = ty >> 1;
+        sx = tx >> 1;
+      } else {
+        sy = oy + ky - 1;
+        sx = ox + kx - 1;
+        ok = sy >= 0 && sy < h && sx >= 0 && sx < w;
+      }
+      if (ok) {
+        const float *src = yb + (long long)(ky * 3 + kx) * cout * iplane + (long long)sy * w + sx;
+        float v = 0.0f;
+        for (int z = 0; z < splits; ++z) v += src[(long long)z * zslab];
+        acc += v;
+      }
+    }
+  float v = acc * (d ? d[(long long)b * cout + co] : 1.0f);
+  if (!up) {
+    if (noise) v = fmaf(nw, noise[(long long)b * noise_bstride + (long long)oy * out_pitch + ox], v);
+    if (bias) v = hf_lrelu(v + bias[co], alpha, scale);
+  }
+  return v;
+}
+
 __global__ __launch_bounds__(256) void small_combine(float *__restrict__ out, const float *__restrict__ y, int splits,
                                                      long long zslab, const float *__restrict__ d,
                                                      const float *__restrict__ noise, const float *__restrict__ noise_w,
@@ -356,7 +396,7 @@
                                                      int cout, int h, int w, int up, int out_h, int out_pitch, int out_wv,
                                                      float alpha, float scale) {
 #pragma clang fp contract(on)
-  const long long oplane = (long long)out_h * out_pitch, iplane = (long long)h * w;
+  const long long oplane = (long long)out_h * out_pitch;
   const long long total = (long long)batch * cout * oplane;
   const long long stride = (long long)gridDim.x * 256;
   const float nw = noise ? noise_w[0] : 0.0f;
@@ -367,38 +407,46 @@
     r /= out_h;
     const int co = (int)(r % cout), b = (int)(r / cout);
     if (ox >= out_wv) continue;
-    float acc = 0.0f;
-    const float *yb = y + ((long long)b * 9 * cout + co) * iplane;
-#pragma unroll
-    for (int ky = 0; ky < 3; ++ky)
-#pragma unroll
-      for (int kx = 0; kx < 3; ++kx) {
-        int sy, sx;
-        bool ok;
-        if (up) {
-          const int ty = oy - ky, tx = ox - kx;
-          ok = ty >= 0 && tx >= 0 && !(ty & 1) && !(tx & 1) && (ty >> 1) < h && (tx >> 1) < w;
-          sy = ty >> 1;
-          sx = tx >> 1;
-        } else {
-          sy = oy + ky - 1;
-          sx = ox + kx - 1;
-          ok = sy >= 0 && sy < h && sx >= 0 && sx < w;
-        }
-        if (ok) {
-          const float *src = yb + (long long)(ky * 3 + kx) * cout * iplane + (long long)sy * w + sx;
-          float v = 0.0f;
-          for (int z = 0; z < splits; ++z) v += src[(long long)z * zslab];
-          acc += v;
-        }
-      }
-    float v = acc * (d ? d[(long long)b * cout + co] : 1.0f);
-    if (!up) {
-      if (noise) v = fmaf(nw, noise[(long long)b * noise_bstride + (long long)oy * out_pitch + ox], v);
-      if (bias) v = hf_lrelu(v + bias[co], alpha, scale);
-    }
-    out[i] = v;
-  }
+    out[i] = small_combine_value(y, splits, zslab, d, noise, nw, noise_bstride, bias, b, co, oy, ox, cout, h, w, up, out_pitch,
+                                 alpha, scale);
+  }
+}
+
+__global__ __launch_bounds__(256) void small_combine_split(float *__restrict__ out, half8 *__restrict__ out_hi,
+                                                           half8 *__restrict__ out_lo, const float *__restrict__ y, int splits,
+                                                           long long zslab, const float *__restrict__ d,
+                                                           const float *__restrict__ noise, const float *__restrict__ noise_w,
+                                                           long long noise_bstride, const float *__restrict__ bias,
+                                                           const float *__restrict__ s_next, int batch, int cout, int h, int w,
+                                                           float alpha, float scale) {
+#pragma clang fp contract(on)
+  const int plane = h * w, cblocks = cout >> 3;
+  const long long total = (long long)batch * cblocks * plane;
+  const long long stride = (long long)gridDim.x * 256;
+  const float nw = noise ? noise_w[0] : 0.0f;
+  bool ovf = false;
+  for (long long i = (long long)blockIdx.x * 256 + threadIdx.x; i < total; i += stride) {
+    const int pix = (int)(i % plane);
+    const long long r = i / plane;
+    const int cb = (int)(r % cblocks), b = (int)(r / cblocks);
+    const int oy = pix / w, ox = pix - oy * w;
+    half8 h8, l8;
+#pragma unroll
+    for (int k = 0; k < 8; ++k) {
+      const int co = cb * 8 + k;
+      const float v = small_combine_value(y, splits, zslab, d, noise, nw, noise_bstride, bias, b, co, oy, ox, cout, h, w, 0, w,
+                                          alpha, scale);
+      out[((long long)b * cout + co) * plane + pix] = v;
+      const float m = fmaf(v, s_next ? s_next[(long long)b * cout + co] : 1.0f, 0.0f);
+      _Float16 hv, lv;
+      hf_split_f16(m, hv, lv, ovf);
+      h8[k] = hv;
+      l8[k] = lv;
+    }
+    out_hi[i] = h8;
+    if (out_lo) out_lo[i] = l8;
+  }
+  hf_note_overflow(ovf);
 }
 
 extern "C" int hf_split_activation_mod_f16(void *out_hi, void *out_lo, const float *x, const float *scale, long long images,
@@ -406,10 +454,13 @@
 
 static int small_gemm(ConvParams &P, const void *w9_hi, const void *w9_lo, int nterms, const float *x, const float *s,
                       int batch, int cin, int cout, int h, int w, float *workspace, long long workspace_floats,
-                      hipStream_t st) {
+                      hipStream_t st, const void *x_hi = nullptr, const void *x_lo = nullptr) {
   P = ConvParams{};
   const long long split_floats = (long long)batch * cin * h * w / 2;
-  {
+  if (x_hi) {
+    P.xh = x_hi;
+    P.xl = nterms == 3 ? x_lo : nullptr;
+  } else {
     int sk0 = gemm_splits(batch, cin, 9 * cout, h * w, 1);
     if (gemm_vsplit(batch, 9 * cout, h * w, 1, sk0)) sk0 = 1;
     const long long need = (long long)sk0 * batch * 9 * cout * h * w + 2 * split_floats;
@@ -454,26 +505,52 @@
   return (long long)sk * batch * 9 * cout * h * w + (long long)batch * cin * h * w;
 }
 
+static int small_conv(float *out, void *out_hi, void *out_lo, const float *x, const void *x_hi, const void *x_lo,
+                      const void *w9_hi, const void *w9_lo, int nterms, const float *s, const float *d, const float *noise,
+                      const float *noise_w, long long noise_bstride, const float *bias, const float *s_next, int batch, int cin,
+                      int cout, int h, int w, float alpha, float scale, int upsample, int tmp_pitch, float *workspace,
+                      long long workspace_floats, void *stream) {
+  if (!out || (!x == !x_hi) || !w9_hi || batch <= 0 || cin <= 0 || cout <= 0 || h <= 0 || w <= 0 || (nterms != 1 && nterms != 3) ||
+      (nterms == 3 && (!w9_lo || (x_hi && !x_lo))) || (cin % KS) || (cout % 64) || (noise && !noise_w) || h * w > 1024 ||
+      (upsample && (tmp_pitch < 2 * w + 1 || noise || bias || out_hi)) || (out_lo && !out_hi))
+    return HF_E_INVALID;
+  ConvParams P;
+  const int rc = small_gemm(P, w9_hi, w9_lo, nterms, x, s, batch, cin, cout, h, w, workspace, workspace_floats, (hipStream_t)stream,
+                            x_hi, x_lo);
+  if (rc != HF_OK) return rc;
+  const int out_h = upsample ? 2 * h + 1 : h, pitch = upsample ? tmp_pitch : w, wv = upsample ? 2 * w + 1 : w;
+  const long long total = out_hi ? (long long)batch * (cout >> 3) * h * w : (long long)batch * cout * out_h * pitch;
+  long long g = (total + 255) / 256;
+  if (g > 4096) g = 4096;
+  if (out_hi)
+    hipLaunchKernelGGL(small_combine_split, dim3((int)g), dim3(256), 0, (hipStream_t)stream, out, static_cast<half8 *>(out_hi),
+                       static_cast<half8 *>(out_lo), workspace, P.vsplit ? 1 : P.splits, P.zslab, d, noise, noise_w, noise_bstride,
+                       bias, s_next, batch, cout, h, w, alpha, scale);
+  else
+    hipLaunchKernelGGL(small_combine, dim3((int)g), dim3(256), 0, (hipStream_t)stream, out, workspace, P.vsplit ? 1 : P.splits, P.zslab, d, noise,
+                       noise_w, noise_bstride, bias, batch, cout, h, w, upsample ? 1 : 0, out_h, pitch, wv, alpha, scale);
+  note_path(7, upsample ? 4 : 3);
+  return hf_launch_status();
+}
+
 extern "C" int hf_modconv3x3_small_f16_f32(float *out, const float *x, const void *w9_hi, const void *w9_lo, int nterms,
                                            const float *s, const float *d, const float *noise, const float *noise_w,
                                            long long noise_bstride, const float *bias, int batch, int cin, int cout, int h,
                                            int w, float alpha, float scale, int upsample, int tmp_pitch, float *workspace,
                                            long long workspace_floats, void *stream) {
-  if (!out || !x || !w9_hi || batch <= 0 || cin <= 0 || cout <= 0 || h <= 0 || w <= 0 || (nterms != 1 && nterms != 3) ||
-      (nterms == 3 && !w9_lo) || (cin % KS) || (cout % 64) || (noise && !noise_w) || h * w > 1024 ||
-      (upsample && (tmp_pitch < 2 * w + 1 || noise || bias)))
-    return HF_E_INVALID;
-  ConvParams P;
-  const int rc = small_gemm(P, w9_hi, w9_lo, nterms, x, s, batch, cin, cout, h, w, workspace, workspace_floats, (hipStream_t)stream);
-  if (rc != HF_OK) return rc;
-  const int out_h = upsample ? 2 * h + 1 : h, pitch = upsample ? tmp_pitch : w, wv = upsample ? 2 * w + 1 : w;
-  const long long total = (long long)batch * cout * out_h * pitch;
-  long long g = (total + 255) / 256;
-  if (g > 4096) g = 4096;
-  hipLaunchKernelGGL(small_combine, dim3((int)g), dim3(256), 0, (hipStream_t)stream, out, workspace, P.vsplit ? 1 : P.splits, P.zslab, d, noise,
-                     noise_w, noise_bstride, bias, batch, cout, h, w, upsample ? 1 : 0, out_h, pitch, wv, alpha, scale);
-  note_path(7, upsample ? 4 : 3);
-  return hf_launch_status();
+  if (!x) return HF_E_INVALID;
+  return small_conv(out, nullptr, nullptr, x, nullptr, nullptr, w9_hi, w9_lo, nterms, s, d, noise, noise_w, noise_bstride, bias,
+                    nullptr, batch, cin, cout, h, w, alpha, scale, upsample, tmp_pitch, workspace, workspace_floats, stream);
+}
+
+extern "C" int hf_modconv3x3_small_split_f16_f32(float *out, void *out_hi, void *out_lo, const float *x, const void *x_hi,
+                                                 const void *x_lo, const void *w9_hi, const void *w9_lo, int nterms,
+                                                 const float *s, const float *d, const float *noise, const float *noise_w,
+                                                 long long noise_bstride, const float *bias, const float *s_next, int batch,
+                                                 int cin, int cout, int h, int w, float alpha, float scale, float *workspace,
+                                                 long long workspace_floats, void *stream) {
+  return small_conv(out, out_hi, out_lo, x, x_hi, x_lo, w9_hi, w9_lo, nterms, s, d, noise, noise_w, noise_bstride, bias, s_next,
+                    batch, cin, cout, h, w, alpha, scale, 0, 0, workspace, workspace_floats, stream);
 }
 
 
@@ -605,20 +682,22 @@
   if (SPLIT) hf_note_overflow(ovf);
 }
 
-extern "C" int hf_modconv3x3_small_up_blur_f16_f32(float *out, void *out_hi, void *out_lo, const float *x, const void *w9_hi,
-                                                   const void *w9_lo, int nterms, const float *s, const float *d,
-                                                   const float *blur_kernel4x4, const float *noise, const float *noise_w,
-                                                   long long noise_bstride, const float *bias, const float *s_next, int batch,
-                                                   int cin, int cout, int h, int w, float alpha, float scale, float *workspace,
-                                                   long long workspace_floats, void *stream) {
-  if ((!out == !out_hi) || !x || !w9_hi || !blur_kernel4x4 || batch <= 0 || cin <= 0 || cout <= 0 || h <= 0 || w <= 0 ||
-      (nterms != 1 && nterms != 3) || (nterms == 3 && !w9_lo) || (cin % KS) || (cout % 64) || (noise && !noise_w) || h * w > 1024 ||
-      (long long)batch * (cout >> 3) > 0x7fffffffLL)
+extern "C" int hf_modconv3x3_small_up_blur_pre_f16_f32(float *out, void *out_hi, void *out_lo, const float *x, const void *x_hi,
+                                                       const void *x_lo, const void *w9_hi, const void *w9_lo, int nterms,
+                                                       const float *s, const float *d, const float *blur_kernel4x4,
+                                                       const float *noise, const float *noise_w, long long noise_bstride,
+                                                       const float *bias, const float *s_next, int batch, int cin, int cout,
+                                                       int h, int w, float alpha, float scale, float *workspace,
+                                                       long long workspace_floats, void *stream) {
+  if ((!out == !out_hi) || (!x == !x_hi) || !w9_hi || !blur_kernel4x4 || batch <= 0 || cin <= 0 || cout <= 0 || h <= 0 || w <= 0 ||
+      (nterms != 1 && nterms != 3) || (nterms == 3 && (!w9_lo || (x_hi && !x_lo))) || (cin % KS) || (cout % 64) ||
+      (noise && !noise_w) || h * w > 1024 || (long long)batch * (cout >> 3) > 0x7fffffffLL)
     return HF_E_INVALID;
   const size_t lds = ((size_t)8 * (2 * h + 3) * (2 * w + 3) + (size_t)72 * h * w) * sizeof(float);
   if (lds > 150 * 1024) return HF_E_INVALID;
   ConvParams P;
-  const int rc = small_gemm(P, w9_hi, w9_lo, nterms, x, s, batch, cin, cout, h, w, workspace, workspace_floats, (hipStream_t)stream);
+  const int rc = small_gemm(P, w9_hi, w9_lo, nterms, x, s, batch, cin, cout, h, w, workspace, workspace_floats, (hipStream_t)stream,
+                            x_hi, x_lo);
   if (rc != HF_OK) return rc;
   const int splits = P.vsplit ? 1 : P.splits;
   const dim3 grid(batch * (cout >> 3));
@@ -633,6 +712,19 @@
   return hf_launch_status();
 }
 
+extern "C" int hf_modconv3x3_small_up_blur_f16_f32(float *out, void *out_hi, void *out_lo, const float *x, const void *w9_hi,
+                                                   const void *w9_lo, int nterms, const float *s, const float *d,
+                                                   const float *blur_kernel4x4, const float *noise, const float *noise_w,
+                                                   long long noise_bstride, const float *bias, const float *s_next, int batch,
+                                                   int cin, int cout, int h, int w, float alpha, float scale, float *workspace,
+                                                   long long workspace_floats, void *stream) {
+  if (!x) return HF_E_INVALID;
+  return hf_modconv3x3_small_up_blur_pre_f16_f32(out, out_hi, out_lo, x, nullptr, nullptr, w9_hi, w9_lo, nterms, s, d, blur_kernel4x4,
+                                                 noise, noise_w, noise_bstride, bias, s_next, batch, cin, cout, h, w, alpha, scale,
+                                                 workspace, workspace_floats, stream);
+}
+
+#include "head.h"
 #include "conv_rect.h"
 
 extern "C" unsigned long long hf_f16_overflow_count_gemm(int reset) { return hf_f16_overflow_read_tu(reset); }
diff --git a/hairfastgan_amd/csrc/head.h b/hairfastgan_amd/csrc/head.h
--- /dev/null
+++ b/hairfastgan_amd/csrc/head.h
@@ -0,0 +1,148 @@
+
+__global__ __launch_bounds__(256) void head_fold_prepare(float *__restrict__ A, const float *__restrict__ wt,
+                                                         const float *__restrict__ c, int cin, int cout, int h, int w, int k) {
+  const long long total = (long long)cout * h * w * cin;
+  const long long i = (long long)blockIdx.x * 256 + threadIdx.x;
+  if (i >= total) return;
+  const int ci = (int)(i % cin);
+  long long r = i / cin;
+  const int p = (int)(r % (h * w)), co = (int)(r / (h * w));
+  const int y = p / w, x = p - y * w, pad = k / 2;
+  float acc = 0.0f;
+  for (int ky = 0; ky < k; ++ky)
+    for (int kx = 0; kx < k; ++kx) {
+      const int sy = y + ky - pad, sx = x + kx - pad;
+      if (sy < 0 || sy >= h || sx < 0 || sx >= w) continue;
+      acc = fmaf(wt[((long long)(ky * k + kx) * cin + ci) * cout + co], c[((long long)ci * h + sy) * w + sx], acc);
+    }
+  A[i] = acc;
+}
+
+constexpr int HEAD_CO = 4;
+constexpr int HEAD_NB = 8;
+constexpr int HEAD_NT = 512;
+constexpr int HEAD_PADF = 4;
+static inline size_t head_fold_lds(int cin, int plane) {
+  return ((size_t)HEAD_CO * plane * (cin + HEAD_PADF) + (size_t)HEAD_NB * cin + (size_t)HEAD_NB * plane * HEAD_CO) * sizeof(float);
+}
+
+__global__ __launch_bounds__(HEAD_NT) void head_fold_forward(float *__restrict__ out, _Float16 *__restrict__ out_hi,
+                                                             _Float16 *__restrict__ out_lo, const float *__restrict__ A,
+                                                             const float *__restrict__ s, const float *__restrict__ d,
+                                                             const float *__restrict__ noise, const float *__restrict__ noise_w,
+                                                             long long noise_bstride, const float *__restrict__ bias,
+                                                             const float *__restrict__ s_next, int batch, int cin, int cout,
+                                                             int plane, float alpha, float scale) {
+#pragma clang fp contract(on)
+  HF_DYN_LDS;
+  const int rowf = cin + HEAD_PADF;
+  float *Al = reinterpret_cast<float *>(hf_dyn_lds);
+  float *Sl = Al + (size_t)HEAD_CO * plane * rowf;
+  float *Rl = Sl + (size_t)HEAD_NB * cin;
+  const int co0 = blockIdx.x * HEAD_CO;
+  const int cin4 = cin >> 2;
+  {
+    const float4 *src = reinterpret_cast<const float4 *>(A + (long long)co0 * plane * cin);
+    const int n4 = HEAD_CO * plane * cin4;
+    constexpr int U = 8;
+    for (int i0 = threadIdx.x; i0 < n4; i0 += U * HEAD_NT) {
+      float4 t[U];
+#pragma unroll
+      for (int u = 0; u < U; ++u) {
+        const int i = i0 + u * HEAD_NT;
+        t[u] = i < n4 ? src[i] : make_float4(0.0f, 0.0f, 0.0f, 0.0f);
+      }
+#pragma unroll
+      for (int u = 0; u < U; ++u) {
+        const int i = i0 + u * HEAD_NT;
+        if (i < n4) {
+          const int row = i / cin4, q = i - row * cin4;
+          *reinterpret_cast<float4 *>(Al + (size_t)row * rowf + 4 * q) = t[u];
+        }
+      }
+    }
+  }
+  const float nw = noise ? noise_w[0] : 0.0f;
+  bool ovf = false;
+  for (int b0 = 0; b0 < batch; b0 += HEAD_NB) {
+    const int nb = min(HEAD_NB, batch - b0);
+    __syncthreads();
+    for (int i = threadIdx.x; i < nb * cin4; i += HEAD_NT)
+      reinterpret_cast<float4 *>(Sl)[i] = reinterpret_cast<const float4 *>(s + (long long)b0 * cin)[i];
+    __syncthreads();
+    const int items = HEAD_CO * nb * plane;
+    for (int it = threadIdx.x; it < items; it += HEAD_NT) {
+      const int p = it % plane, r = it / plane;
+      const int bi = r % nb, c = r / nb;
+      const float4 *ar = reinterpret_cast<const float4 *>(Al + (size_t)(c * plane + p) * rowf);
+      const float4 *sr = reinterpret_cast<const float4 *>(Sl + (size_t)bi * cin);
+      float acc = 0.0f;
+      for (int q = 0; q < cin4; ++q) {
+        const float4 a = ar[q], m = sr[q];
+        acc = fmaf(a.x, m.x, acc);
+        acc = fmaf(a.y, m.y, acc);
+        acc = fmaf(a.z, m.z, acc);
+        acc = fmaf(a.w, m.w, acc);
+      }
+      const long long b = b0 + bi;
+      const int co = co0 + c;
+      float v = acc;
+      if (d) v *= d[b * cout + co];
+      if (noise) v = fmaf(nw, noise[b * noise_bstride + p], v);
+      if (bias) v += bias[co];
+      v = hf_lrelu(v, alpha, scale);
+      Rl[(bi * plane + p) * HEAD_CO + c] = v;
+    }
+    __syncthreads();
+    const int pairs = nb * plane;
+    for (int base = (threadIdx.x >> 6) << 6; base < pairs; base += HEAD_NT) {
+      const int j = base + (threadIdx.x & 63);
+      const bool live = j < pairs;
+      const int bi = live ? j / plane : 0, p = live ? j - bi * plane : 0;
+      const long long b = b0 + bi;
+      float v[HEAD_CO], m[HEAD_CO];
+#pragma unroll
+      for (int c = 0; c < HEAD_CO; ++c) {
+        v[c] = live ? Rl[(bi * plane + p) * HEAD_CO + c] : 0.0f;
+        if (live) out[(b * cout + co0 + c) * plane + p] = v[c];
+        m[c] = v[c] * ((live && s_next) ? s_next[b * cout + co0 + c] : 1.0f);
+      }
+      if (out_hi) {
+        hf_half4 h4, l4;
+        hf_split4_f16(m, h4, l4, ovf);
+        if (live) {
+          const long long e = ((b * (cout >> 3) + (co0 >> 3)) * plane + p) * 8 + (co0 & 4);
+          *reinterpret_cast<hf_half4 *>(out_hi + e) = h4;
+          if (out_lo) *reinterpret_cast<hf_half4 *>(out_lo + e) = l4;
+        }
+      }
+    }
+  }
+  if (out_hi) hf_note_overflow(ovf);
+}
+
+extern "C" int hf_head_fold_prepare_f32(float *A, const float *wt, const float *c, int cin, int cout, int h, int w, int k,
+                                        void *stream) {
+  if (!A || !wt || !c || cin <= 0 || cout <= 0 || h <= 0 || w <= 0 || k <= 0 || !(k & 1) || (cin & 3) ||
+      (long long)cout * h * w * cin > (1LL << 31) * 256)
+    return HF_E_INVALID;
+  const long long total = (long long)cout * h * w * cin;
+  hipLaunchKernelGGL(head_fold_prepare, dim3((unsigned)((total + 255) / 256)), dim3(256), 0, (hipStream_t)stream, A, wt, c, cin,
+                     cout, h, w, k);
+  return hf_launch_status();
+}
+
+extern "C" int hf_head_fold_forward_f32(float *out, void *out_hi, void *out_lo, const float *A, const float *s, const float *d,
+                                        const float *noise, const float *noise_w, long long noise_bstride, const float *bias,
+                                        const float *s_next, int batch, int cin, int cout, int plane, float alpha, float scale,
+                                        void *stream) {
+  if (!out || !A || !s || batch <= 0 || cin <= 0 || cout <= 0 || plane <= 0 || (cin & 3) || (cout % HEAD_CO) ||
+      (noise && !noise_w) || (out_lo && !out_hi) || (out_hi && (cout & 7)))
+    return HF_E_INVALID;
+  const size_t lds = head_fold_lds(cin, plane);
+  if (lds > 160 * 1024) return HF_E_UNSUPPORTED;
+  hipLaunchKernelGGL(head_fold_forward, dim3(cout / HEAD_CO), dim3(HEAD_NT), lds, (hipStream_t)stream, out,
+                     static_cast<_Float16 *>(out_hi), static_cast<_Float16 *>(out_lo), A, s, d, noise, noise_w, noise_bstride, bias,
+                     s_next, batch, cin, cout, plane, alpha, scale);
+  return hf_launch_status();
+}
diff --git a/hairfastgan_amd/stylegan2/model.py b/hairfastgan_amd/stylegan2/model.py
--- a/hairfastgan_amd/stylegan2/model.py
+++ b/hairfastgan_amd/stylegan2/model.py
@@ -12,6 +12,9 @@
 
 
 FUSE_BLUR_MIN_H = int(os.environ.get("HAIRFAST_FUSE_BLUR_MIN_H", "128"))
+
+HEAD_FOLD = os.environ.get("HAIRFAST_HEAD_FOLD", "1") != "0"
+HEAD_SPLIT = os.environ.get("HAIRFAST_HEAD_SPLIT", "1") != "0"
 
 
 class PixelNorm(nn.Module):
@@ -113,6 +116,7 @@
 
     def invalidate(self):
         self._prep = self._prep_f16 = self._coeffs = None
+        self.__dict__.pop("_fold", None)
 
     def __repr__(self):
         return (f"{self.__class__.__name__}({self.in_channel}, {self.out_channel}, {self.kernel_size}, "
@@ -141,6 +145,20 @@
         cached = self.__dict__.get("_prep_small")
         if cached is None or cached[0] != key:
             cached = self.__dict__["_prep_small"] = (key, M.split_weights_small(lib(), stream(), wt))
+        return cached[1]
+
+    def folded(self, const):
+        w = self.weight
+        ver = lambda t: None if t.is_inference() else t._version
+        key = (w.data_ptr(), ver(w), const.data_ptr(), ver(const), w.device, tuple(const.shape))
+        cached = self.__dict__.get("_fold")
+        if cached is None or cached[0] != key:
+            if (self.upsample or const.ndim != 4 or const.shape[0] != 1 or const.shape[1] != self.in_channel or const.device != w.device
+                    or not M.head_fold_supported(self.in_channel, self.out_channel, const.shape[2] * const.shape[3])
+                    or torch.cuda.is_current_stream_capturing()):
+                return None
+            wt, _ = self.prepared()
+            cached = self.__dict__["_fold"] = (key, M.head_fold_prepare(lib(), stream(), wt, const.detach()))
         return cached[1]
 
     def route_same_res(self, shape, plain=True):
@@ -161,7 +179,8 @@
             return "f32"
         if h >= FUSE_BLUR_MIN_H and tail and M.modconv3x3_up_fused_supported(cin, cout, h, w) and self.blur_factors() is not None:
             return "fused"
-        if not is_split and M.modconv3x3_small_supported(cin, cout, h, w, b, upsample=True):
+        if ((not is_split or (HEAD_SPLIT and M.SMALL_UP_FUSED and M.small_up_blur_supported(h, w)))
+                and M.modconv3x3_small_supported(cin, cout, h, w, b, upsample=True)):
             return "small"
         return "f16" if M.modconv3x3_up_f16_supported(cin, cout, h, w, batch=b) else "f32"
 
@@ -197,6 +216,9 @@
             return M.modconv3x3_up_fused(lib(), stream(), input, hi, lo, s, d, self.blur_factors(), noise, noise_w, bias, alpha, scale,
                                          split_for=None if split_for is None else split_for[1], nterms=conv_nterms())
         f16 = small = None
+        if route == "small" and isinstance(input, M.SplitActivation):
+            return M.modconv3x3_small_up_blur(lib(), stream(), input, self.prepared_small(), conv_nterms(), s, d, self.blur.kernel, noise,
+                                              noise_w, bias, self.out_channel, alpha, scale, split_for=split_for)
         if route == "small":
             small = (self.prepared_small(), conv_nterms())
         elif route == "f16":
@@ -297,6 +319,33 @@
         act = self.activate
         return conv.conv_up(input, wt, s, d, noise, self.noise.weight.detach(), act.bias.detach(),
                             act.negative_slope, act.scale, split_for=(None, s_next, conv_precision() == "f16x3"))
+
+    def forward_folded(self, const, style, noise, split_for=None):
+        conv, act = self.conv, self.activate
+        a = conv.folded(const)
+        if a is None or act.bias is None:
+            return None
+        require_gpu(style, noise)
+        _, s, d = conv.style_coefficients(style)
+        h, w = const.shape[2:]
+        if noise is None:
+            noise = s.new_empty(s.shape[0], 1, h, w).normal_()
+        return M.head_fold_forward(lib(), stream(), a, (h, w), s, d, noise, self.noise.weight.detach(), act.bias.detach(),
+                                   act.negative_slope, act.scale,
+                                   split_for=None if split_for is None else (None, split_for, conv_precision() == "f16x3"))
+
+    def forward_small_from_split(self, split, coeffs, noise=None, split_for=None):
+        conv, act = self.conv, self.activate
+        assert not conv.upsample
+        _, s, d = coeffs
+        b, _, h, w = split.shape
+        if noise is None:
+            noise = split.hi.new_empty(b, 1, h, w, dtype=torch.float32).normal_()
+        require_gpu(noise)
+        res = M.modconv3x3_small(lib(), stream(), split, conv.prepared_small(), conv_nterms(), s, d, noise, self.noise.weight.detach(),
+                                 act.bias.detach(), conv.out_channel, act.negative_slope, act.scale,
+                                 split_for=None if split_for is None else (None, split_for, conv_precision() == "f16x3"))
+        return res if split_for is not None else (res, None)
 
     def forward_image(self, split, coeffs, noise, rgb, to_rgb, skip):
         conv, act = self.conv, self.activate
@@ -527,14 +576,57 @@
         skip = to_rgb.finish(raw, skip) if raw is not None else to_rgb(out, latent[:, i + 2], skip)
         return out, skip, split_in, up_coeffs
 
+    def _block_kind(self, block, src_shape, is_split):
+        conv_up, conv_same = self.convs[2 * block - 2], self.convs[2 * block - 1]
+        if _observed(conv_up, conv_same):
+            return "plain"
+        mid_shape = (src_shape[0], conv_up.conv.out_channel, 2 * src_shape[2], 2 * src_shape[3])
+        if conv_same.conv.route_same_res(mid_shape, plain=False)[0] == "f16":
+            return "fast"
+        if (HEAD_SPLIT and M.SMALL_UP_FUSED and M.small_up_blur_supported(*src_shape[2:]) and conv_same.activate.bias is not None
+                and conv_up.conv.route_up(src_shape, is_split=is_split) == "small"
+                and conv_same.conv.route_same_res(mid_shape, plain=True)[0] == "small"):
+            return "head"
+        return "plain"
+
+    def _next_takes_split(self, block, out_shape, latent, end_layer):
+        if not HEAD_SPLIT or block >= self.log_size - 2 or block + 1 > end_layer:
+            return None, None
+        nup = self.convs[2 * block]
+        if self._block_kind(block + 1, out_shape, True) == "plain" or nup.conv.route_up(out_shape, is_split=True) != "small":
+            return None, None
+        up_coeffs = nup.conv.style_coefficients(latent[:, 2 * block + 1])
+        return up_coeffs[1], up_coeffs
+
+    def _head_block(self, block, src, latent, noise, skip, up_coeffs, end_layer):
+        conv_up, conv_same, to_rgb = self.convs[2 * block - 2], self.convs[2 * block - 1], self.to_rgbs[block - 1]
+        i = 2 * block - 1
+        coeffs = conv_same.conv.style_coefficients(latent[:, i + 1])
+        split = conv_up.forward_split(src, latent[:, i], noise[2 * block - 1], coeffs[1],
+                                      coeffs=up_coeffs if isinstance(src, M.SplitActivation) else None)
+        s_up, up_coeffs = self._next_takes_split(block, (src.shape[0], conv_same.conv.out_channel) + tuple(split.shape[2:]), latent, end_layer)
+        out, split_in = conv_same.forward_small_from_split(split, coeffs, noise[2 * block], split_for=s_up)
+        skip = to_rgb(out, latent[:, i + 2], skip)
+        return out, skip, split_in, up_coeffs
+
     def _run_layers(self, latent, noise, layer_in, skip, start_layer, end_layer, return_latents):
-        out = self.input(latent)
+        split_in = up_coeffs = None
+        out = None
+        if (start_layer == 0 and HEAD_FOLD and latent.is_cuda and type(self.input) is ConstantInput
+                and not _observed(self.input, self.conv1)):
+            const = self.input.input
+            s_up, coeffs = self._next_takes_split(0, (latent.shape[0], self.conv1.conv.out_channel) + tuple(const.shape[2:]), latent, end_layer)
+            out = self.conv1.forward_folded(const, latent[:, 0], noise[0], split_for=s_up)
+            if out is not None and s_up is not None:
+                (out, split_in), up_coeffs = out, coeffs
+        if out is None:
+            out = self.input(latent)
+            if start_layer == 0:
+                out = self.conv1(out, latent[:, 0], noise=noise[0])
         if start_layer == 0:
-            out = self.conv1(out, latent[:, 0], noise=noise[0])
             skip = self.to_rgb1(out, latent[:, 1])
         if end_layer == 0:
             return out, skip
-        split_in = up_coeffs = None
         for block in range(1, self.log_size - 1):
             if block < start_layer:
                 continue
@@ -544,9 +636,12 @@
             i = 2 * block - 1
             src = layer_in if block == start_layer else (split_in if split_in is not None else out)
             mid_shape = (src.shape[0], conv_up.conv.out_channel, 2 * src.shape[2], 2 * src.shape[3])
-            kernel, fuses = conv_same.conv.route_same_res(mid_shape, plain=False)
-            if kernel == "f16" and not _observed(conv_up, conv_same):
+            kind = self._block_kind(block, tuple(src.shape), isinstance(src, M.SplitActivation))
+            fuses = conv_same.conv.route_same_res(mid_shape, plain=False)[1]
+            if kind == "fast":
                 out, skip, split_in, up_coeffs = self._fast_block(block, src, mid_shape, fuses, latent, noise, skip, up_coeffs, end_layer)
+            elif kind == "head":
+                out, skip, split_in, up_coeffs = self._head_block(block, src, latent, noise, skip, up_coeffs, end_layer)
             else:
                 assert not isinstance(src, M.SplitActivation)
                 split_in = None
diff --git a/include/hairfast_hip.h b/include/hairfast_hip.h
--- a/include/hairfast_hip.h
+++ b/include/hairfast_hip.h
@@ -9,6 +9,7 @@
 #define HF_E_INVALID (-1)
 #define HF_E_LAUNCH (-2)
 #define HF_E_WORKSPACE (-3)
+#define HF_E_UNSUPPORTED (-4)
 
 #define HF_ACT_RESIDUAL_FIRST 16
 
@@ -155,6 +156,22 @@
                                         long long noise_bstride, const float *bias, const float *s_next, int batch, int cin,
                                         int cout, int h, int w, float alpha, float scale, float *workspace,
                                         long long workspace_floats, void *stream);
+int hf_modconv3x3_small_split_f16_f32(float *out, void *out_hi, void *out_lo, const float *x, const void *x_hi, const void *x_lo,
+                                      const void *w9_hi, const void *w9_lo, int nterms, const float *s, const float *d,
+                                      const float *noise, const float *noise_w, long long noise_bstride, const float *bias,
+                                      const float *s_next, int batch, int cin, int cout, int h, int w, float alpha, float scale,
+                                      float *workspace, long long workspace_floats, void *stream);
+int hf_modconv3x3_small_up_blur_pre_f16_f32(float *out, void *out_hi, void *out_lo, const float *x, const void *x_hi,
+                                            const void *x_lo, const void *w9_hi, const void *w9_lo, int nterms, const float *s,
+                                            const float *d, const float *blur_kernel4x4, const float *noise,
+                                            const float *noise_w, long long noise_bstride, const float *bias,
+                                            const float *s_next, int batch, int cin, int cout, int h, int w, float alpha,
+                                            float scale, float *workspace, long long workspace_floats, void *stream);
+int hf_head_fold_prepare_f32(float *A, const float *wt, const float *c, int cin, int cout, int h, int w, int k, void *stream);
+int hf_head_fold_forward_f32(float *out, void *out_hi, void *out_lo, const float *A, const float *s, const float *d,
+                             const float *noise, const float *noise_w, long long noise_bstride, const float *bias,
+                             const float *s_next, int batch, int cin, int cout, int plane, float alpha, float scale,
+                             void *stream);
 int hf_split_activation_f16(void *out_hi, void *out_lo, const float *x, const float *in_scale, const float *in_shift,
                             long long images, int channels, int h, int w, void *stream);
 
```

Result: no change. 1732 images/s (median of 6 runs) (+0.2%).
